# sjtuytc/betapose

Hardware: AMD Instinct MI355X
Metric: frames/sec (640x480, 50-kp KPD) (higher is better)
Workload: dtype f32 as an exact 3-way bf16 operand split (6 bf16 MFMA products), f32 accumulate and activations

## Files before the change

### betapose_amd/_lib.py

```python
from __future__ import annotations

import ctypes as C
import os
import threading

_HERE = os.path.dirname(os.path.abspath(__file__))
LIB_PATH = os.environ.get("BP_LIB") or os.path.join(_HERE, "libbetapose_hip.so")
_lock = threading.Lock()
_lib = None

c_float_p = C.POINTER(C.c_float)
c_double_p = C.POINTER(C.c_double)
c_int_p = C.POINTER(C.c_int)
vp = C.c_void_p

PROTOTYPES = {
    "bp_last_error": (C.c_char_p, []),
    "bp_version": (C.c_int, []),
    "bp_device_count": (C.c_int, []),
    "bp_device_name": (C.c_int, [C.c_int, C.c_char_p, C.c_int]),
    "bp_yolo_create": (C.c_int, [C.c_char_p, C.c_char_p, C.c_int, C.c_int, C.c_int, C.POINTER(vp)]),
    "bp_yolo_create_from_memory": (C.c_int, [C.c_char_p, vp, C.c_size_t, C.c_int, C.c_int, C.c_int, C.POINTER(vp)]),
    "bp_yolo_clone": (C.c_int, [vp, C.POINTER(vp)]),
    "bp_kpd_clone": (C.c_int, [vp, C.POINTER(vp)]),
    "bp_yolo_destroy": (None, [vp]),
    "bp_yolo_rows": (C.c_int, [vp]),
    "bp_yolo_attrs": (C.c_int, [vp]),
    "bp_yolo_forward": (C.c_int, [vp, vp, C.c_int, vp, vp]),
    "bp_yolo_forward_select": (C.c_int, [vp, vp, C.c_int, C.c_float, C.c_int, vp, vp, vp]),
    "bp_yolo_forward_select_classes": (C.c_int, [vp, vp, C.c_int, C.c_float, C.c_int, vp, C.c_int, vp, vp, vp]),
    "bp_yolo_select": (C.c_int, [vp, C.c_int, C.c_int, C.c_int, C.c_float, C.c_int, vp, vp]),
    "bp_yolo_tap_count": (C.c_int, [vp]),
    "bp_yolo_tap_info": (C.c_int, [vp, C.c_int, C.c_char_p, C.c_int, c_int_p, c_int_p, c_int_p]),
    "bp_yolo_tap_copy": (C.c_int, [vp, C.c_int, C.c_int, vp, vp]),
    "bp_kpd_create": (C.c_int, [vp, C.c_size_t, C.c_int, C.c_int, C.c_int, C.POINTER(vp)]),
    "bp_kpd_destroy": (None, [vp]),
    "bp_kpd_forward": (C.c_int, [vp, vp, C.c_int, vp, vp]),
    "bp_kpd_forward_argmax": (C.c_int, [vp, vp, C.c_int, vp, vp, vp]),
    "bp_kpd_launch_count": (C.c_int, [vp, C.c_int]),
    "bp_kpd_tap_count": (C.c_int, [vp]),
    "bp_kpd_tap_info": (C.c_int, [vp, C.c_int, C.c_char_p, C.c_int, c_int_p, c_int_p, c_int_p]),
    "bp_kpd_tap_copy": (C.c_int, [vp, C.c_int, C.c_int, vp, vp]),
    "bp_yolo_set_policy": (C.c_int, [vp, C.c_int, C.c_int, C.c_int, C.c_int]),
    "bp_kpd_set_policy": (C.c_int, [vp, C.c_int, C.c_int, C.c_int, C.c_int]),
    "bp_yolo_set_precision": (C.c_int, [vp, C.c_int]),
    "bp_kpd_set_precision": (C.c_int, [vp, C.c_int]),
    "bp_calibrate_ticks": (C.c_int, [C.c_longlong, c_float_p, vp]),
    "bp_yolo_set_prefetch": (C.c_int, [vp, C.c_int]),
    "bp_kpd_set_prefetch": (C.c_int, [vp, C.c_int]),
    "bp_yolo_set_fusion": (C.c_int, [vp, C.c_int]),
    "bp_kpd_set_fusion": (C.c_int, [vp, C.c_int]),
    "bp_yolo_fused_launches": (C.c_int, [vp, C.c_int, C.POINTER(C.c_int)]),
    "bp_kpd_fused_launches": (C.c_int, [vp, C.c_int, C.POINTER(C.c_int)]),
    "bp_yolo_xcd_errors": (C.c_int, [vp, C.POINTER(C.c_int), vp]),
    "bp_kpd_xcd_errors": (C.c_int, [vp, C.POINTER(C.c_int), vp]),
    "bp_yolo_set_stamps": (C.c_int, [vp, vp, C.c_int]),
    "bp_kpd_set_stamps": (C.c_int, [vp, vp, C.c_int]),
    "bp_yolo_op_name": (C.c_int, [vp, C.c_int, C.c_char_p, C.c_int]),
    "bp_kpd_op_name": (C.c_int, [vp, C.c_int, C.c_char_p, C.c_int]),
    "bp_yolo_op_stats": (C.c_int, [vp, c_double_p, c_double_p, C.c_int]),
    "bp_kpd_op_stats": (C.c_int, [vp, c_double_p, c_double_p, C.c_int]),
    "bp_yolo_device_bytes": (C.c_size_t, [vp]),
    "bp_kpd_device_bytes": (C.c_size_t, [vp]),
    "bp_crop": (C.c_int, [vp, C.c_int, C.c_int, C.c_int, vp, C.c_int, vp, vp, vp, vp, C.c_int, C.c_int, vp]),
    "bp_resize_bicubic": (C.c_int, [vp, C.c_int, C.c_int, C.c_int, C.c_int, C.c_int, C.c_int, vp, vp, vp]),
    "bp_conv2d": (C.c_int, [vp, C.c_int, C.c_int, C.c_int, C.c_int, vp, vp, C.c_int, C.c_int, C.c_int, C.c_int,
                            C.c_int, C.c_int, vp, C.c_int, C.c_int, C.c_int, vp, C.c_int, c_float_p, vp]),
    "bp_conv2d_planes": (C.c_int, [vp, C.c_int, C.c_int, C.c_int, C.c_int, vp, vp, C.c_int, C.c_int, C.c_int, C.c_int,
                                   C.c_int, C.c_int, vp, C.c_int, C.c_int, C.c_int, vp, vp, C.c_int, c_float_p, vp]),
    "bp_pipeline_create": (C.c_int, [vp, vp, C.c_int, C.c_int, C.c_int, C.c_float, C.c_int, vp, vp, vp, C.POINTER(vp)]),
    "bp_pipeline_kernel_count": (C.c_int, [vp]),
    "bp_yolo_profile": (C.c_int, [vp, C.c_int, C.c_int, c_float_p, c_int_p, C.c_int, vp]),
    "bp_kpd_profile": (C.c_int, [vp, C.c_int, C.c_int, c_float_p, c_int_p, C.c_int, vp]),
    "bp_pipeline_destroy": (None, [vp]),
    "bp_pipeline_frames": (vp, [vp]),
    "bp_pipeline_results": (vp, [vp]),
    "bp_pipeline_heatmaps": (vp, [vp]),
    "bp_pipeline_set_fixed_box": (C.c_int, [vp, vp]),
    "bp_pipeline_run": (C.c_int, [vp, C.c_int, vp]),
    "bp_pipeline_prepare": (C.c_int, [vp]),
    "bp_pipeline_latency_faults": (C.c_int, [vp]),
    "bp_scene_create": (C.c_int, [vp, vp, vp, C.c_int, C.c_int, C.c_int, C.c_float, C.c_int, vp, vp, C.POINTER(vp)]),
    "bp_scene_destroy": (None, [vp]),
    "bp_scene_results": (vp, [vp]),
    "bp_scene_poses": (vp, [vp]),
    "bp_scene_set_pose_solver": (C.c_int, [vp, C.c_int, vp, C.c_int, vp, C.c_int, vp]),
    "bp_scene_set_pose_ransac": (C.c_int, [vp, C.c_int, C.c_double, C.c_int, C.c_double]),
    "bp_scene_prepare": (C.c_int, [vp]),
    "bp_scene_run": (C.c_int, [vp, C.c_int, vp]),
    "bp_scene_kernel_count": (C.c_int, [vp]),
    "bp_yolo_select_nms": (C.c_int, [vp, C.c_int, C.c_int, C.c_int, C.c_float, C.c_int, C.c_int, C.c_float, C.c_int, vp, vp, vp]),
    "bp_yolo_forward_select_nms": (C.c_int, [vp, vp, C.c_int, C.c_float, C.c_int, C.c_int, C.c_float, C.c_int, vp, vp, vp, vp]),
    "bp_crop_candidates": (C.c_int, [vp, C.c_int, C.c_int, C.c_int, C.c_int, vp, C.c_int, vp, vp, vp, vp, C.c_int, C.c_int, vp]),
    "bp_cands_create": (C.c_int, [vp, vp, C.c_int, C.c_int, C.c_int, C.c_float, C.c_int, C.c_int, C.c_float, vp, vp, C.POINTER(vp)]),
    "bp_cands_destroy": (None, [vp]),
    "bp_cands_results": (vp, [vp]),
    "bp_cands_counts": (vp, [vp]),
    "bp_cands_prepare": (C.c_int, [vp]),
    "bp_cands_run": (C.c_int, [vp, C.c_int, vp]),
    "bp_cands_kernel_count": (C.c_int, [vp]),
    "bp_cands_set_pose_solver": (C.c_int, [vp, vp, C.c_int, vp, C.c_int, vp]),
    "bp_cands_pose": (vp, [vp]),
    "bp_cands_merged": (vp, [vp]),
    "bp_cands_info": (vp, [vp]),
    "bp_pose_from_candidate_records": (C.c_int, [vp, vp, C.c_int, C.c_int, vp, C.c_int, vp, C.c_int, vp, vp, vp, vp]),
    "bp_cands_set_instance_poses": (C.c_int, [vp, C.c_int, vp]),
    "bp_cands_instance_poses": (vp, [vp]),
    "bp_pose_instances_from_merged": (C.c_int, [vp, vp, vp, C.c_int, C.c_int, vp, C.c_int, vp, C.c_int, vp, vp]),
    "bp_heatmap_argmax": (C.c_int, [vp, C.c_int, C.c_int, C.c_int, C.c_int, vp, vp]),
    "bp_pose_errors": (C.c_int, [vp, C.c_int, vp, vp, C.c_int, vp, C.c_int, vp, vp]),
    "bp_pose_errors_sym": (C.c_int, [vp, C.c_int, vp, vp, C.c_int, vp, C.c_int, vp, C.c_int, vp, vp]),
    "bp_render_depth": (C.c_int, [vp, C.c_int, vp, C.c_int, vp, C.c_int, vp, C.c_int, C.c_int, C.c_double, C.c_double, vp, vp,
                                  vp]),
    "bp_render_depth_host": (C.c_int, [vp, C.c_int, vp, C.c_int, vp, C.c_int, vp, C.c_int, C.c_int, C.c_double, C.c_double, vp,
                                       vp]),
    "bp_vsd_errors": (C.c_int, [vp, C.c_int, vp, C.c_int, vp, vp, C.c_int, vp, vp, C.c_int, C.c_int, C.c_int, C.c_double, vp,
                                C.c_double, vp, C.c_int, C.c_double, C.c_double, C.c_double, C.c_int, vp, vp, vp]),
    "bp_icp_normal_equations": (C.c_int, [vp, C.c_int, vp, C.c_int, vp, C.c_int, vp, vp, C.c_int, C.c_int, C.c_int, C.c_double, vp,
                                          C.c_double, C.c_double, C.c_double, C.c_double, C.c_int, vp, vp]),
    "bp_icp_normal_equations_host": (C.c_int, [vp, C.c_int, vp, C.c_int, vp, C.c_int, vp, vp, C.c_int, C.c_int, C.c_int,
                                               C.c_double, vp, C.c_double, C.c_double, C.c_double, C.c_double, vp]),
    "bp_refine_depth": (C.c_int, [vp, C.c_int, vp, C.c_int, vp, C.c_int, vp, vp, C.c_int, C.c_int, C.c_int, C.c_double, vp,
                                  C.c_int, C.c_double, C.c_double, C.c_int, C.c_double, C.c_double, C.c_int, vp, vp, vp]),
    "bp_refine_depth_host": (C.c_int, [vp, C.c_int, vp, C.c_int, vp, C.c_int, vp, vp, C.c_int, C.c_int, C.c_int, C.c_double, vp,
                                       C.c_int, C.c_double, C.c_double, C.c_int, C.c_double, C.c_double, vp, vp]),
    "bp_pipeline_set_pose_solver": (C.c_int, [vp, vp, C.c_int, vp, C.c_int, vp]),
    "bp_pipeline_poses": (vp, [vp]),
    "bp_pose_from_records": (C.c_int, [vp, C.c_int, vp, C.c_int, vp, C.c_int, vp, vp]),
    "bp_solve_pnp_batch": (C.c_int, [vp, C.c_int, vp, C.c_int, C.c_int, vp, vp, vp, vp]),
    "bp_pnp_ransac_samples": (C.c_int, [C.c_int, C.c_int, vp]),
    "bp_pnp_ransac_trials_needed": (C.c_int, [C.c_int, C.c_double, vp]),
    "bp_pnp_ransac_workspace_bytes": (C.c_size_t, [C.c_int, C.c_int]),
    "bp_solve_pnp_ransac_batch": (C.c_int, [vp, C.c_int, vp, C.c_int, C.c_int, vp, C.c_double, C.c_int, C.c_double, vp, vp, vp,
                                            vp, C.c_size_t, vp]),
    "bp_pipeline_set_pose_ransac": (C.c_int, [vp, C.c_double, C.c_int, C.c_double]),
    "bp_pose_ransac_workspace_bytes": (C.c_size_t, [C.c_int, C.c_int]),
    "bp_pose_from_records_ransac": (C.c_int, [vp, C.c_int, vp, C.c_int, vp, C.c_int, C.c_double, C.c_int, C.c_double, vp, vp,
                                              C.c_size_t, vp]),
    "bp_solve_pnp": (C.c_int, [vp, vp, C.c_int, vp, vp, vp]),
    "bp_solve_pnp_status": (C.c_int, [vp, vp, C.c_int, vp, vp, vp, vp]),
    "bp_solve_pnp_refined": (C.c_int, [vp, vp, C.c_int, vp, vp, vp]),
    "bp_solve_pnp_ransac": (C.c_int, [vp, vp, C.c_int, vp, C.c_double, C.c_int, C.c_double, vp, vp, vp]),
    "bp_pose_nms": (C.c_int, [vp, vp, vp, vp, C.c_int, C.c_int, vp, vp, vp, vp]),
    "bp_darknet_last_error": (C.c_char_p, []),
    "bp_darknet_create": (C.c_int, [C.c_char_p, C.c_char_p, C.c_int, C.POINTER(vp)]),
    "bp_darknet_destroy": (None, [vp]),
    "bp_darknet_width": (C.c_int, [vp]),
    "bp_darknet_height": (C.c_int, [vp]),
    "bp_darknet_classes": (C.c_int, [vp]),
    "bp_darknet_detect_rgb": (C.c_int, [vp, vp, C.c_int, C.c_int, C.c_float, C.c_float, vp, C.c_int]),
    "bp_darknet_detect_png": (C.c_int, [vp, vp, C.c_size_t, C.c_float, C.c_float, vp, C.c_int]),
    "bp_darknet_detect_image": (C.c_int, [vp, vp, C.c_size_t, C.c_float, C.c_float, vp, C.c_int]),
    "bp_image_decode_rgb": (C.c_int, [vp, C.c_size_t, vp, C.c_size_t, C.POINTER(C.c_int), C.POINTER(C.c_int)]),
    "bp_darknet_detect_file": (C.c_int, [vp, C.c_char_p, C.c_float, C.c_float, vp, C.c_int]),
    "bp_yolo_create_darknet": (C.c_int, [C.c_char_p, C.c_char_p, C.c_int, C.c_int, C.c_int, C.POINTER(vp)]),
    "bp_stream_create_masked": (C.c_int, [vp, C.c_int, C.POINTER(vp)]),
    "bp_stream_destroy": (C.c_int, [vp]),
    "bp_probe_placement": (C.c_int, [C.c_int, vp, vp, vp]),
    "bp_png_info": (C.c_int, [vp, C.c_size_t, C.POINTER(C.c_int), C.POINTER(C.c_int), C.POINTER(C.c_int)]),
    "bp_png_decode_bgr": (C.c_int, [vp, C.c_size_t, vp, C.c_size_t, C.POINTER(C.c_int), C.POINTER(C.c_int)]),
    "bp_loader_create": (C.c_int, [C.POINTER(C.c_char_p), C.c_int, C.c_int, C.c_int, C.c_int, C.c_int, C.c_int,
                                   C.POINTER(vp)]),
    "bp_loader_destroy": (None, [vp]),
    "bp_loader_next": (C.c_int, [vp, C.POINTER(C.c_longlong), C.POINTER(vp)]),
    "bp_loader_release": (C.c_int, [vp, C.c_longlong]),
    "bp_upload": (C.c_int, [vp, vp, C.c_size_t, vp]),
}

RESULT_FLOATS = 316
POSE_DOUBLES = 166
PNP_MAX_POINTS = 64
MAX_SCENE_CLASSES = 16
MAX_CANDIDATES = 8
MERGED_FLOATS = 152


class BetaposeHipError(RuntimeError):
    pass


def lib():
    global _lib
    with _lock:
        if _lib is not None:
            return _lib
        import torch
        if not os.path.exists(LIB_PATH):
            from .build import build
            build(verbose=False)
        try:
            L = C.CDLL(LIB_PATH)
        except OSError as e:
            raise BetaposeHipError("cannot load %s: %s (run `python -m betapose_amd.build`)" % (LIB_PATH, e))
        for name, (res, args) in PROTOTYPES.items():
            fn = getattr(L, name)
            fn.restype = res
            fn.argtypes = args
        _lib = L
        return L


def check(rc: int) -> None:
    if rc != 0:
        msg = lib().bp_last_error()
        raise BetaposeHipError(msg.decode() if msg else "libbetapose_hip error %d" % rc)


def require_gpu() -> None:
    import torch
    if not torch.cuda.is_available():
        raise BetaposeHipError("betapose_amd needs an AMD GPU (gfx950): torch.cuda.is_available() is False; "
                               "there is no CPU fallback on the product path")
    if lib().bp_device_count() <= 0:
        raise BetaposeHipError("libbetapose_hip.so sees no HIP device")


def ptr(t) -> int:
    if t is None:
        return None
    if hasattr(t, "data_ptr"):
        if not t.is_contiguous():
            raise ValueError("tensor must be contiguous")
# ... 8 lines not shown
```

### betapose_amd/build.py

```python
from __future__ import annotations

import os
import shutil
import subprocess
import sys

HERE = os.path.dirname(os.path.abspath(__file__))
CSRC = os.path.join(HERE, "csrc")
LIB = os.path.join(HERE, "libbetapose_hip.so")
SOURCES = ["conv_igemm.hip", "conv_halo.hip", "conv_fused.hip", "conv_pl.hip", "conv_s1.hip", "conv_p3.hip", "aux_kernels.hip", "pose_metrics.hip", "pose_metrics_sym.hip", "raster.hip", "vsd.hip", "icp.hip", "pose_tail.hip", "pose_tail_cands.hip", "pose_tail_inst.hip", "pnp_ransac.hip", "engine.cpp", "host_post.cpp", "raster_host.cpp", "icp_host.cpp", "frame_io.cpp", "jpeg_bmp.cpp", "c_api.cpp", "darknet_compat.cpp"]
HEADERS = ["bp_common.h", "engine.h", "frame_chain.h", "frame_io.h", "conv_tail.inc", "pnp_wave.inc", "pnp_math.inc", "pose_decode.inc", "pose_tail.h", "raster.h", "raster_math.inc", "icp.h", "icp_math.inc", "conv_dev.h", os.path.join("..", "..", "include", "betapose_hip.h"),
           os.path.join("..", "..", "include", "yolo_v2_class_compat.h")]
EXP = "experimental"
EXP_SOURCES = [os.path.join(EXP, s_) for s_ in ("conv_w64.hip", "conv_kg.hip", "conv_rd.hip")]
EXP_HEADERS = [os.path.join(EXP, s_) for s_ in ("mega.inc", "kernels_unity.hip")]
ARCH = "gfx950"
LAST_ACTION = None
MIN_STUBS = {"conv_s1.hip": 1, "conv_p3.hip": 39, "conv_igemm.hip": 14, "conv_halo.hip": 13, "conv_fused.hip": 12, "conv_pl.hip": 12, "aux_kernels.hip": 21, "pose_metrics.hip": 2, "pose_metrics_sym.hip": 4, "raster.hip": 3, "vsd.hip": 2, "icp.hip": 4, "pose_tail.hip": 3, "pose_tail_cands.hip": 1, "pose_tail_inst.hip": 1, "pnp_ransac.hip": 2}
MIN_STUBS_EXP = {"conv_s1.hip": 1, "conv_p3.hip": 39, "experimental/kernels_unity.hip": 26, "conv_fused.hip": 12, "conv_pl.hip": 12, "experimental/conv_w64.hip": 8,
                 "experimental/conv_kg.hip": 3, "experimental/conv_rd.hip": 2, "aux_kernels.hip": 24, "pose_metrics.hip": 2, "pose_metrics_sym.hip": 4, "raster.hip": 3, "vsd.hip": 2, "icp.hip": 4, "pose_tail.hip": 3, "pose_tail_cands.hip": 1, "pose_tail_inst.hip": 1, "pnp_ransac.hip": 2}


def hipcc() -> str:
    for cand in (os.environ.get("HIPCC"), shutil.which("hipcc"), "/opt/rocm/bin/hipcc"):
        if cand and os.path.exists(cand):
            return cand
    raise RuntimeError("hipcc not found (need ROCm to build libbetapose_hip.so)")


def _stale() -> bool:
    if not os.path.exists(LIB):
        return True
    t = os.path.getmtime(LIB)
    deps = [os.path.join(CSRC, s) for s in SOURCES + HEADERS]
    return any(os.path.getmtime(d) > t for d in deps if os.path.exists(d))


def build(force: bool = False, verbose: bool = True, experimental: bool = False) -> str:
    if experimental:
        return _build(True, verbose, os.path.join(HERE, "libbetapose_hip_exp.so"), os.path.join(HERE, "build_exp"),
                      ["-DBP_EXPERIMENTAL"])
    global LAST_ACTION
    if not force and not _stale():
        LAST_ACTION = "reused"
        return LIB
    LAST_ACTION = "compiled"
    return _build(force, verbose, LIB, os.path.join(HERE, "build"), [])


def _build(force: bool, verbose: bool, LIB: str, objdir: str, extra) -> str:
    cc = hipcc()
    objs = []
    os.makedirs(objdir, exist_ok=True)
    procs = []
    sources = SOURCES + (EXP_SOURCES if extra else [])
    if extra:
        sources = [os.path.join(EXP, "kernels_unity.hip")] + [s_ for s_ in sources if s_ not in ("conv_igemm.hip", "conv_halo.hip")]
    hdr_t = max(os.path.getmtime(os.path.join(CSRC, h)) for h in HEADERS + (EXP_HEADERS if extra else []))
    flags_key = " ".join(list(extra) + os.environ.get("BP_CFLAGS", "").split())
    flags_file = os.path.join(objdir, ".flags")
    same_flags = os.path.exists(flags_file) and open(flags_file).read() == flags_key
    for src in sources:
        obj = os.path.join(objdir, os.path.splitext(os.path.basename(src))[0] + ".o")
        objs.append(obj)
        if not force and same_flags and os.path.exists(obj) and os.path.getmtime(obj) > max(hdr_t, os.path.getmtime(os.path.join(CSRC, src))):
            continue
        cmd = [cc, "--offload-arch=" + ARCH, "-O3", "-std=c++17", "-fPIC", "-x", "hip", "-c", "-I", CSRC,
               os.path.join(CSRC, src), "-o", obj] + list(extra) + os.environ.get("BP_CFLAGS", "").split()
        if verbose:
            print(" ".join(cmd), flush=True)
        procs.append((src, subprocess.Popen(cmd, stdout=subprocess.PIPE, stderr=subprocess.STDOUT, text=True)))
    for src, p in procs:
        out, _ = p.communicate()
        if p.returncode != 0:
            raise RuntimeError("hipcc failed on %s:\n%s" % (src, out))
        if verbose and out.strip():
            print(out)
    with open(flags_file, "w") as f:
        f.write(flags_key)
    nm = shutil.which("nm") or "/opt/rocm/lib/llvm/bin/llvm-nm"
    for src, want in (MIN_STUBS_EXP if extra else MIN_STUBS).items():
        obj = os.path.join(objdir, os.path.splitext(os.path.basename(src))[0] + ".o")
        syms = subprocess.run([nm, obj], stdout=subprocess.PIPE, text=True).stdout
        have = syms.count("__device_stub__")
        if have < want:
            raise RuntimeError("%s: %d kernel host stubs in the object, expected >= %d (hipcc dropped a kernel)" % (src, have, want))
    cmd = [cc, "--offload-arch=" + ARCH, "-shared", "-fPIC", "-o", LIB] + objs + ["-lz", "-lpthread"]
    if verbose:
        print(" ".join(cmd), flush=True)
    subprocess.check_call(cmd)
    return LIB


if __name__ == "__main__":
    print(build(force="--force" in sys.argv, experimental="--experimental" in sys.argv))
```

### betapose_amd/csrc/bp_common.h

```cpp
#pragma once
#include <hip/hip_runtime.h>
#include <cstdint>
#include <cstdio>
#include <mutex>
#include <set>
#include <stdexcept>
#include <string>
#include <utility>

namespace bp {

struct Error : std::runtime_error {
    using std::runtime_error::runtime_error;
};

#define BP_HIP(expr)                                                                      \
    do {                                                                                  \
        hipError_t _e = (expr);                                                           \
        if (_e != hipSuccess)                                                             \
            throw ::bp::Error(std::string(#expr) + ": " + hipGetErrorString(_e) + " @" +  \
                              __FILE__ + ":" + std::to_string(__LINE__));                 \
    } while (0)

#define BP_CHECK(cond, msg)                                                               \
    do {                                                                                  \
        if (!(cond)) throw ::bp::Error(std::string(msg) + " (" #cond ") @" + __FILE__ +   \
                                       ":" + std::to_string(__LINE__));                   \
    } while (0)

inline void allow_big_lds(const void* kernel) {
    static std::mutex mu;
    static std::set<std::pair<int, const void*>> done;
    int dev = 0;
    BP_HIP(hipGetDevice(&dev));
    std::lock_guard<std::mutex> lk(mu);
    if (done.count({dev, kernel})) return;
    BP_HIP(hipFuncSetAttribute(kernel, hipFuncAttributeMaxDynamicSharedMemorySize, 160 * 1024 - 64));
    done.insert({dev, kernel});
}

__device__ __forceinline__ unsigned long long bp_clock() { return __builtin_amdgcn_s_memrealtime(); }

enum Act : int { ACT_LINEAR = 0, ACT_LEAKY = 1, ACT_RELU = 2 };

enum StoreMode : int {
    ST_NHWC = 0,
    ST_UP2 = 1,
    ST_PIXSHUF = 2,
    ST_NCHW = 3
};

struct ConvParams {
    const float* in;
    int in_ld;
    int N, H, W, Cin;
    const float* w;
    int Kpad;
    int Ktrue;
    const float* bias;
    float* out;
    int out_ld;
    int OH, OW, Cout;
    int ksize, stride, pad;
    int act;
    const float* res;
    int res_ld;
    const float* res_scale;
    int res_after_act;
    int store_mode;
    int M;
    int nchunks;
    int splits;
    int chunks_per_split;
    float* partial;
    int* tickets;
    int CoutPad;
    int cin_pack;
    const unsigned short* w16;
    const unsigned short* w16s;
    int mfma_mode;
    unsigned long long* stamps;
    const unsigned short* in16;
    long long in16_plane;
    unsigned short* out16;
    long long out16_plane;
    int out_np;
    int skip_f32;
    const unsigned short* res16;
    int net_prec;
    int abl;
    const unsigned short* wbd;
    const unsigned short* wpl;
    float* pool_out;
    int hy_full, hy_splits, hy_cps;
    int xcd_home;
    int* xcc_of;
    int* err_word;
    int* tickets_local;
    int mtiles, n_tiles;
    int work_blocks;
    const void* pf_ptr;
    int pf_first;
    int pf_ntn, pf_splits, pf_cps, pf_nchunks;
    int pf_tile_stride, pf_chunk_bytes;
    int pf_cap;
};

enum Precision : int { PREC_F32 = 0, PREC_F16 = 1, PREC_BF16X3 = 2, PREC_F16_RES = 3 };

enum ConvTile : int { TILE_64x64 = 0, TILE_128x64 = 1, TILE_W64_1x1 = 2, TILE_W64_1x2 = 3, TILE_W64_2x1 = 5, TILE_W64_2x2 = 6,
                      TILE_KG1 = 7, TILE_KG2 = 8, TILE_KG4 = 9,
                      TILE_RD4 = 10, TILE_RD8 = 11,
                      TILE_64x64_BD = 12,
                      TILE_PL64 = 13,
                      TILE_PL128 = 14,
                      TILE_PL128x64 = 15,
                      TILE_PL256x128 = 16,
                      TILE_STEM3 = 20,
                      TILE_PL64BD = 19,
                      TILE_PL64K2 = 18,
                      TILE_PL128S = 17,
                      TILE_HALO64 = 21,
                      TILE_HALO128 = 22,
                      TILE_HALO64K2 = 23,
                      TILE_BD_K2 = 24,
                      TILE_PLH128 = 25,
                      TILE_S1 = 26,
                      TILE_P3 = 27,
                      TILE_STEM7 = 28,
                      TILE_LAST = 27,
                      TILE_FUSED = 40 };

struct ConvProfHook { hipEvent_t e0, e1; };
extern thread_local ConvProfHook* g_conv_prof;
bool conv_h16_eligible(const ConvParams& p);
int conv_vec_mode(const ConvParams& p);

void launch_conv(const ConvParams& p, int tile, hipStream_t s);
void launch_conv_w64(const ConvParams& p, int tile, hipStream_t s);
bool conv_tile_is_w64(int tile);
void launch_conv_kg(const ConvParams& p, int tile, hipStream_t s);
bool conv_tile_is_kg(int tile);
void launch_conv_rd(const ConvParams& p, int tile, hipStream_t s);
bool conv_tile_is_rd(int tile);
void launch_conv_pl(const ConvParams& p, int tile, hipStream_t s);
bool conv_tile_is_pl(int tile);
void launch_conv_halo(const ConvParams& p, int tile, hipStream_t s);
bool conv_tile_is_halo(int tile);
bool conv_halo_eligible(const ConvParams& p, int tile);
void conv_split_plan(const ConvParams& p, int tile, int want, int* splits, int* cps);
inline bool conv_tile_is_plh(int tile) { return tile == TILE_PLH128; }
bool conv_plh_eligible(const ConvParams& p);
bool conv_pl_eligible(const ConvParams& p);
bool conv_s1_eligible(const ConvParams& p, long long M);
void launch_conv_s1(const ConvParams& p, hipStream_t s);
bool conv_p3_eligible(const ConvParams& p, long long M);
void launch_conv_p3(const ConvParams& p, hipStream_t s);
void launch_pack_wpl(const float* in, unsigned short* out, int CoutPad, int Kpad, int Cin, int ksize, int np, hipStream_t s);
void launch_f32_to_planes(const float* in, int ld, long long pixels, int C, unsigned short* planes, long long plane_elems,
                          int np, hipStream_t s);
void launch_planes_to_f32(const unsigned short* planes, long long plane_elems, int np, float* out, int ld, long long pixels, int C,
                          hipStream_t s);
bool conv_fused_eligible(const ConvParams& pre, const ConvParams& c3, const ConvParams* post);
int conv_fused_blocks(const ConvParams& pre, const ConvParams& c3, const ConvParams* post);
void launch_conv_fused(const ConvParams& pre, const ConvParams& c3, const ConvParams* post, hipStream_t s);
int conv_tiles(const ConvParams& p, int tile);
bool conv_stem3_eligible(const ConvParams& p);
bool conv_stem7_eligible(const ConvParams& p);
void conv_grid_setup(ConvParams& q, int bm, int bn);
int conv_grid_blocks(const ConvParams& q);
int xcc_base();
bool conv_hybrid_plan(const ConvParams& p, int tile, size_t partial_floats, int* full, int* hs, int* hcps);
bool conv_home_layout(int tile, int splits);
void conv_prefetch_of(ConvParams& p, const ConvParams& next, int next_tile, int next_splits, int next_cps);
int conv_tile_bm(int tile);
int conv_tile_bn(int tile);

enum MegaOpType : int { MO_CONV_BD = 0, MO_CONV_K2 = 1, MO_CONV_F32V2 = 2, MO_STEM3 = 3 };

struct MegaOp {
    int type, items, npass, pad;
    ConvParams conv;
};
struct MegaArgs {
    const MegaOp* prog[8];
    int n_ops[8];
    unsigned* sync;
    int nb;
    unsigned long long* stamps;
};

size_t mega_lds_bytes(const MegaOp& o);
void mega_make_conv_op(const ConvParams& p, int tile, MegaOp* out);
void launch_mega(const MegaArgs& a, size_t lds_bytes, hipStream_t s);

void launch_nchw_to_nhwc(const float* in, float* out, int N, int C, int H, int W, hipStream_t s);
void launch_nhwc_to_nchw(const float* in, int in_ld, float* out, int N, int C, int H, int W, hipStream_t s);
void launch_maxpool3s2p1(const float* in, float* out, int N, int H, int W, int C, int OH, int OW, hipStream_t s,
                         unsigned short* planes = nullptr, long long plane_elems = 0, int np = 0);
void launch_add(const float* a, int a_ld, const float* b, int b_ld, float* out, int out_ld,
                long long pixels, int C, hipStream_t s);
void launch_upsample2(const float* in, int in_ld, float* out, int out_ld, int N, int H, int W, int C, hipStream_t s);
void launch_copy_channels(const float* in, int in_ld, float* out, int out_ld, long long pixels, int C, hipStream_t s);
void launch_pixel_shuffle2(const float* in, float* out, int N, int H, int W, int C, hipStream_t s,
                           unsigned short* planes = nullptr, long long plane_elems = 0, int np = 0);
int avgpool_parts(int HW);
void launch_avgpool(const float* in, int in_ld, float* out, int N, int HW, int C, hipStream_t s);
void launch_fc(const float* in, const float* w, const float* bias, float* out, int N, int Cin, int Cout,
               int act, int in_parts, float in_scale, hipStream_t s);

struct YoloHead {
    const float* t;
    int g;
    float aw[3], ah[3];
    int row_off;
};
void launch_yolo_decode(const YoloHead* heads, int nheads, int N, int reso, int attrs, int rows,
                        float* pred, hipStream_t s);
void launch_yolo_select(const float* pred, int N, int rows, int attrs, float conf, int num_classes,
                        float* sel, hipStream_t s, int sel_ld = 8);
void launch_yolo_decode_select(const YoloHead* heads, int nheads, int N, int reso, int attrs, int rows, float conf, int num_classes,
                               float* sel, hipStream_t s, int sel_ld = 8);
#define BP_MAX_SCENE_CLASSES 16
struct YoloClassList {
    int n;
    int id[BP_MAX_SCENE_CLASSES];
};
YoloClassList make_class_list(const int* class_ids, int K, int num_classes, int attrs);
void launch_yolo_select_classes(const float* pred, int N, int rows, int attrs, float conf, int num_classes, const YoloClassList& cl,
                                float* sel, hipStream_t s, int ld_image, int ld_slot);
void launch_yolo_decode_select_classes(const YoloHead* heads, int nheads, int N, int reso, int attrs, int rows, float conf,
                                       int num_classes, const YoloClassList& cl, float* sel, hipStream_t s, int ld_image, int ld_slot);
#define BP_MAX_CANDIDATES 8
void launch_yolo_select_nms(const float* pred, int N, int rows, int attrs, float conf, int num_classes, int class_id, float nms_conf,
                            int C, float* sel, int* count, hipStream_t s, int ld_image, int ld_slot);
void launch_yolo_decode_select_nms(const YoloHead* heads, int nheads, int N, int reso, int attrs, int rows, float conf, int num_classes,
                                   int class_id, float nms_conf, int C, float* sel, int* count, hipStream_t s, int ld_image,
                                   int ld_slot);
void launch_heatmap_argmax(const float* hm, int N, int C, int H, int W, float* out, hipStream_t s, int out_ld = 0);

void launch_f32_to_f16(const float* in, unsigned short* out, long long n, hipStream_t s);
void launch_f32_to_bf16x3(const float* in, unsigned short* out_planes, long long n, hipStream_t s);
void launch_f32_to_f16_staged(const float* in, unsigned short* out, int CoutPad, int Kpad, hipStream_t s);
void launch_f32_to_bf16x3_staged(const float* in, unsigned short* out, int CoutPad, int Kpad, hipStream_t s, int Cin_pl = 0);
void launch_probe_placement(int* d_out, int blocks, hipStream_t s);
void launch_spin_ticks(long long ticks, hipStream_t s);

void launch_crop(const uint8_t* frames, int batch, int H, int W, const float* sel, int reso, const float* boxes,
                 float* out_nhwc, float* out_nchw, float* pts, int oh, int ow, hipStream_t s, int sel_ld = 8, int pts_ld = 8,
                 int per_frame = 1);

struct ResizeTables {
    const int* hb;
    const int* hk;
    int ksize_h;
    const int* vb;
    const int* vk;
    int ksize_v;
};
void launch_resize_bicubic(const uint8_t* in, int batch, int H, int W, uint8_t* tmp, float* out_nhwc, uint8_t* out_u8,
                           int oh, int ow, const ResizeTables& t, int swap_rb, hipStream_t s);

}
```

### betapose_amd/csrc/c_api.cpp

```cpp
#include "../../include/betapose_hip.h"

#include <algorithm>
#include <cmath>
#include <cstdlib>
#include <cstring>
#include <fstream>
#include <memory>
#include <sstream>
#include <vector>

#include "engine.h"
#include "frame_chain.h"
#include "frame_io.h"
#include "icp.h"
#include "pose_tail.h"
#include "raster.h"

static thread_local std::string g_err;

#define BP_TRY try {
#define BP_CATCH                                   \
    }                                              \
    catch (const std::exception& e) {              \
        g_err = e.what();                          \
// ... 652 lines not shown
    void* ws = a.alloc_bytes(bp::raster_vertex_bytes(n, (int)(2 * c)));
    int* skipped = (int*)a.alloc_bytes(2 * c * sizeof(int));
    int* acc = (int*)a.alloc_bytes((size_t)P * bp::VSD_ACC * sizeof(int));
    BP_HIP(hipMemsetAsync(acc, 0, (size_t)P * bp::VSD_ACC * sizeof(int), s));
    BP_HIP(hipMemsetAsync(skipped, 0, 2 * c * sizeof(int), s));
    for (size_t p0 = 0; p0 < (size_t)P; p0 += c) {
        const int m = (int)std::min(c, (size_t)P - p0);
        BP_HIP(hipMemsetD32Async((hipDeviceptr_t)zbuf, 0x7f800000, 2 * (size_t)m * HW, s));
        bp::launch_raster(d_model, n, d_faces, F, d_gt + p0 * 12, m, d_est + p0 * 12, m, K, H, W, pixel_center, near_z, ws, zbuf,
                          skipped, s);
        bp::launch_vsd_reduce(zbuf, m, d_depth_test, T, d_test_index + p0, H, W, K, pixel_center, depth_scale, delta, tv, n_tau,
                              diameter, acc + p0 * bp::VSD_ACC, s);
    }
    bp::launch_vsd_finish(acc, d_test_index, T, P, n_tau, d_err, d_counts, s);
    BP_HIP(hipGetLastError());
    BP_HIP(hipStreamSynchronize(s));
    return 0;
    BP_CATCH
}

static bp::IcpParams icp_params(const double* K, int T, double depth_scale, int iterations, double max_dist, double min_cos,
                                int min_pixels, double pixel_center) {
    BP_CHECK(T > 0, "T must be positive");
    BP_CHECK(depth_scale > 0.0 && max_dist > 0.0, "depth_scale and max_dist must be positive");
    BP_CHECK(min_cos >= 0.0 && min_cos <= 1.0, "min_cos must lie in [0, 1]");
    BP_CHECK(iterations >= 0 && iterations <= 1000 && min_pixels >= 0, "iterations must lie in 0 .. 1000, min_pixels >= 0");
    return bp::IcpParams{K[0], K[4], K[2], K[5], pixel_center, depth_scale, max_dist, min_cos, min_pixels, iterations};
}

static size_t icp_chunk(int chunk, int n, int P, size_t HW) {
    size_t c = (size_t)chunk;
    if (c == 0) c = std::min(RASTER_WS_BYTES / (HW * sizeof(float)), RASTER_WS_BYTES / bp::raster_vertex_bytes(n, 1));
    return std::max<size_t>(1, std::min<size_t>(c, (size_t)P));
}

int bp_icp_normal_equations_host(const double* poses, int P, const double* vertices, int n, const int* faces, int F,
                                 const double* K, const uint16_t* depth_test, int T, int H, int W, double depth_scale,
                                 const int* test_index, double max_dist, double min_cos, double pixel_center, double near_z,
                                 double* out) {
    BP_TRY
    BP_CHECK(poses && vertices && faces && K && depth_test && test_index && out, "null argument");
    raster_check_sizes(n, F, P, H, W, near_z);
    const bp::IcpParams prm = icp_params(K, T, depth_scale, 0, max_dist, min_cos, 0, pixel_center);
    BP_CHECK(bp::icp_normal_equations_host(poses, P, vertices, n, faces, F, K, depth_test, T, test_index, H, W, prm, near_z,
                                           out) == 0,
             "a face index lies outside [0, n)");
    return 0;
    BP_CATCH
}

int bp_refine_depth_host(const double* poses, int P, const double* vertices, int n, const int* faces, int F, const double* K,
                         const uint16_t* depth_test, int T, int H, int W, double depth_scale, const int* test_index,
                         int iterations, double max_dist, double min_cos, int min_pixels, double pixel_center, double near_z,
                         double* poses_out, double* stats) {
    BP_TRY
    BP_CHECK(poses && vertices && faces && K && depth_test && test_index && poses_out && stats, "null argument");
    raster_check_sizes(n, F, P, H, W, near_z);
    const bp::IcpParams prm = icp_params(K, T, depth_scale, iterations, max_dist, min_cos, min_pixels, pixel_center);
    BP_CHECK(bp::refine_depth_host(poses, P, vertices, n, faces, F, K, depth_test, T, test_index, H, W, prm, near_z, poses_out,
                                   stats) == 0,
             "a face index lies outside [0, n)");
    return 0;
    BP_CATCH
}

int bp_icp_normal_equations(const double* d_model, int n, const int* d_faces, int F, const double* d_poses, int P,
                            const double* K, const uint16_t* d_depth_test, int T, int H, int W, double depth_scale,
                            const int* d_test_index, double max_dist, double min_cos, double pixel_center, double near_z,
                            int chunk, double* d_out, void* stream) {
    BP_TRY
    BP_CHECK(d_model && d_faces && d_poses && K && d_depth_test && d_test_index && d_out, "null argument");
    raster_check_sizes(n, F, P, H, W, near_z);
    BP_CHECK(chunk >= 0, "chunk must not be negative");
    const bp::IcpParams prm = icp_params(K, T, depth_scale, 0, max_dist, min_cos, 0, pixel_center);
    hipStream_t s = (hipStream_t)stream;
    const size_t HW = (size_t)H * W, c = icp_chunk(chunk, n, P, HW);
    const int slices = bp::icp_slices(H, W);
    bp::Arena a;
    uint32_t* zbuf = (uint32_t*)a.alloc_bytes(c * HW * sizeof(uint32_t));
    void* ws = a.alloc_bytes(bp::raster_vertex_bytes(n, (int)c));
    int* skipped = (int*)a.alloc_bytes(c * sizeof(int));
    double* partial = (double*)a.alloc_bytes(c * slices * bp::ICP_ACC * sizeof(double));
    BP_HIP(hipMemsetAsync(skipped, 0, c * sizeof(int), s));
    for (size_t p0 = 0; p0 < (size_t)P; p0 += c) {
        const int m = (int)std::min(c, (size_t)P - p0);
        BP_HIP(hipMemsetD32Async((hipDeviceptr_t)zbuf, 0x7f800000, (size_t)m * HW, s));
        bp::launch_raster(d_model, n, d_faces, F, d_poses + p0 * 12, m, nullptr, 0, K, H, W, pixel_center, near_z, ws, zbuf,
                          skipped, s);
        bp::launch_icp_accumulate(zbuf, d_poses + p0 * 12, m, d_depth_test, T, d_test_index + p0, H, W, prm, nullptr, partial, s);
        bp::launch_icp_sum(partial, d_test_index + p0, T, m, slices, d_out + p0 * bp::ICP_ACC, s);
    }
    BP_HIP(hipGetLastError());
    BP_HIP(hipStreamSynchronize(s));
    return 0;
    BP_CATCH
}

int bp_refine_depth(const double* d_model, int n, const int* d_faces, int F, const double* d_poses, int P, const double* K,
                    const uint16_t* d_depth_test, int T, int H, int W, double depth_scale, const int* d_test_index,
                    int iterations, double max_dist, double min_cos, int min_pixels, double pixel_center, double near_z,
                    int chunk, double* d_poses_out, double* d_stats, void* stream) {
    BP_TRY
    BP_CHECK(d_model && d_faces && d_poses && K && d_depth_test && d_test_index && d_poses_out && d_stats, "null argument");
    BP_CHECK(d_poses_out != d_poses, "d_poses_out must not be d_poses: a rejected pose gets its input back");
    raster_check_sizes(n, F, P, H, W, near_z);
    BP_CHECK(chunk >= 0, "chunk must not be negative");
    const bp::IcpParams prm = icp_params(K, T, depth_scale, iterations, max_dist, min_cos, min_pixels, pixel_center);
    hipStream_t s = (hipStream_t)stream;
    const size_t HW = (size_t)H * W, c = icp_chunk(chunk, n, P, HW);
    const int slices = bp::icp_slices(H, W);
    bp::Arena a;
    uint32_t* zbuf = (uint32_t*)a.alloc_bytes(c * HW * sizeof(uint32_t));
    void* ws = a.alloc_bytes(bp::raster_vertex_bytes(n, (int)c));
    int* skipped = (int*)a.alloc_bytes(c * sizeof(int));
    double* partial = (double*)a.alloc_bytes(c * slices * bp::ICP_ACC * sizeof(double));
    BP_HIP(hipMemsetAsync(skipped, 0, c * sizeof(int), s));
    bp::launch_icp_init(d_poses, d_test_index, T, P, d_poses_out, d_stats, s);
    for (size_t p0 = 0; p0 < (size_t)P; p0 += c) {
        const int m = (int)std::min(c, (size_t)P - p0);
        double* pose = d_poses_out + p0 * 12;
        double* stats = d_stats + p0 * bp::ICP_STATS;
        for (int k = 0; k <= iterations; ++k) {
            BP_HIP(hipMemsetD32Async((hipDeviceptr_t)zbuf, 0x7f800000, (size_t)m * HW, s));
            bp::launch_raster(d_model, n, d_faces, F, pose, m, nullptr, 0, K, H, W, pixel_center, near_z, ws, zbuf, skipped, s);
            bp::launch_icp_accumulate(zbuf, pose, m, d_depth_test, T, d_test_index + p0, H, W, prm, stats, partial, s);
            bp::launch_icp_step(partial, m, slices, k, prm, d_poses + p0 * 12, pose, stats, s);
        }
    }
    BP_HIP(hipGetLastError());
    BP_HIP(hipStreamSynchronize(s));
    return 0;
    BP_CATCH
}

int bp_heatmap_argmax(const float* d_hm, int batch, int C, int H, int W, float* d_kp, void* stream) {
    BP_TRY
    BP_CHECK(d_hm && d_kp && batch > 0 && C > 0 && H > 0 && W > 0, "bad argument");
    bp::launch_heatmap_argmax(d_hm, batch, C, H, W, d_kp, (hipStream_t)stream);
    BP_HIP(hipGetLastError());
    return 0;
    BP_CATCH
}

int bp_conv2d(const float* d_in, int N, int H, int W, int Cin, const float* h_w, const float* h_bias, int Cout, int k,
              int stride, int pad, int act, int store_mode, const float* d_res, int res_after_act, int tile, int splits,
              float* d_out, int iters, float* ms_per_iter, void* stream) {
    return bp_conv2d_planes(d_in, N, H, W, Cin, h_w, h_bias, Cout, k, stride, pad, act, store_mode, d_res, res_after_act, tile,
                            splits, d_out, nullptr, iters, ms_per_iter, stream);
}

int bp_conv2d_planes(const float* d_in, int N, int H, int W, int Cin, const float* h_w, const float* h_bias, int Cout, int k,
                     int stride, int pad, int act, int store_mode, const float* d_res, int res_after_act, int tile, int splits,
                     float* d_out, unsigned short* d_out_planes, int iters, float* ms_per_iter, void* stream) {
    BP_TRY
    BP_CHECK(d_in && h_w && d_out, "null argument");
    hipStream_t s = (hipStream_t)stream;
    struct OneConv : bp::Net {
        OneConv() : Net(1) {}
        using Net::add_conv;
        using Net::finalize;
        using Net::ops_;
        using Net::partial_;
        using Net::partial_floats_;
        using Net::arena_;
    } net;
    const int OH = (H + 2 * pad - k) / stride + 1, OW = (W + 2 * pad - k) / stride + 1;
    bp::Tensor in; in.p = const_cast<float*>(d_in); in.H = H; in.W = W; in.C = Cin; in.ld = Cin;
    bp::Tensor out; out.p = d_out; out.H = OH; out.W = OW; out.C = Cout;
    out.ld = store_mode == bp::ST_PIXSHUF ? Cout / 4 : Cout;
    bp::Tensor res; res.p = const_cast<float*>(d_res); res.ld = Cout; res.C = Cout; res.H = OH; res.W = OW;
    bp::ConvWeights cw; cw.w = h_w; cw.bias = h_bias;
    net.add_conv("conv", in, out, cw, Cout, k, stride, pad, act, store_mode, d_res ? &res : nullptr, nullptr,
                 res_after_act, 1e-5f, OH, OW);
    int t = tile;
    int prec = bp::PREC_F32;
    if (t >= 256) {
        prec = t >= 512 ? bp::PREC_BF16X3 : bp::PREC_F16;
        t -= t >= 512 ? 512 : 256;
        BP_CHECK(Cin % 32 == 0, "layer is not eligible for the 16-bit MFMA paths (needs Cin % 32 == 0)");
        net.set_precision(prec);
        net.ops_[0].conv.mfma_mode = prec;
#ifndef BP_EXPERIMENTAL
        BP_CHECK(bp::conv_tile_is_pl(t) || ((t == bp::TILE_64x64_BD || t == bp::TILE_BD_K2 || bp::conv_tile_is_halo(t)) && prec == bp::PREC_BF16X3),
                 "this kernel id exists only in the experimental library (python -m betapose_amd.build --experimental, BP_LIB)");
#endif
    } else {
        if (t < 0 && bp::conv_stem3_eligible(net.ops_[0].conv)) t = bp::TILE_STEM3;
        BP_CHECK(t <= bp::TILE_128x64 || (t == bp::TILE_STEM3 && bp::conv_stem3_eligible(net.ops_[0].conv)) || (t == bp::TILE_STEM7 && bp::conv_stem7_eligible(net.ops_[0].conv)),
                 "this tile needs a 16-bit precision mode (tile + 256 / + 512), or the layer is not a 3x3 / stride-1 / 4-channel-packed stem");
    }
    bp::ConvParams p = net.ops_[0].conv;
    p.N = N; p.M = N * OH * OW;
    if (t < 0) t = bp::TILE_64x64;
    const int np = prec == bp::PREC_F16 ? 1 : 3;
    if (bp::conv_tile_is_pl(t)) {
        const long long in_elems = (long long)N * H * W * Cin;
        BP_CHECK(Cin % 32 == 0 && k * k <= 32, "layer is not eligible for the operand-plane kernels (needs Cin % 32 == 0, k*k <= 32)");
        unsigned short* d_in16 = (unsigned short*)net.arena_.alloc_bytes((size_t)np * in_elems * 2);
        bp::launch_f32_to_planes(d_in, Cin, (long long)N * H * W, Cin, d_in16, in_elems, np, s);
        p.in16 = d_in16; p.in16_plane = in_elems;
        auto& packed = np == 1 ? net.weight_store()->wpl1 : net.weight_store()->wpl3;
        auto it = packed.find(p.w);
        if (it == packed.end()) {
            unsigned short* d = (unsigned short*)net.weight_store()->arena.alloc_bytes((size_t)np * p.CoutPad * p.Kpad * 2);
            bp::launch_pack_wpl(p.w, d, p.CoutPad, p.Kpad, p.Cin, p.ksize, np, s);
            it = packed.emplace(p.w, d).first;
        }
        p.wpl = it->second;
        if (t == bp::TILE_PL64BD) {
            auto& staged = net.weight_store()->wbd3;
            auto ib = staged.find(p.w);
            if (ib == staged.end()) {
                unsigned short* d = (unsigned short*)net.weight_store()->arena.alloc_bytes((size_t)3 * p.CoutPad * p.Kpad * 2);
                bp::launch_f32_to_bf16x3_staged(p.w, d, p.CoutPad, p.Kpad, s, p.Cin);
                ib = staged.emplace(p.w, d).first;
            }
            p.wbd = ib->second;
        }
    }
    if (const char* e = std::getenv("BP_PL_ABL")) p.abl = std::atoi(e);
    if (d_out_planes) {
        BP_CHECK(prec != bp::PREC_F32, "output planes need a 16-bit precision mode");
        long long out_elems = (long long)N * OH * OW * Cout;
        if (store_mode == bp::ST_UP2) out_elems *= 4;
        p.out16 = d_out_planes; p.out16_plane = out_elems; p.out_np = np;
    }
    if (prec == bp::PREC_F16 && std::getenv("BP_CONV_F16R")) {
        if (p.res) {
            const long long n_res = (long long)N * OH * OW;
            unsigned short* r16 = (unsigned short*)net.arena_.alloc_bytes((size_t)n_res * p.res_ld * 2);
            bp::launch_f32_to_planes(p.res, p.res_ld, n_res, Cout, r16, n_res * p.res_ld, 1, s);
            p.res16 = r16;
        }
        if (p.out16) p.skip_f32 = 1;
    }
    int sp = splits;
    if (sp <= 0) {
        const long long blocks = bp::conv_tiles(p, t);
        sp = 1;
        while (blocks * sp < 512 && p.nchunks / (sp + 1) >= 4 && sp < 64) ++sp;
    }
    if (t == bp::TILE_S1 || t == bp::TILE_P3) sp = 1;
    int per = 0;
    bp::conv_split_plan(p, t, sp, &sp, &per);
    p.splits = sp; p.chunks_per_split = per;
    if (sp > 1) {
        const int tiles = bp::conv_tiles(p, t);
        p.partial = net.arena_.alloc((size_t)sp * tiles * bp::conv_tile_bm(t) * bp::conv_tile_bn(t));
        p.tickets = (int*)net.arena_.alloc_bytes((size_t)(2 + 64) * tiles * sizeof(int));
        BP_HIP(hipMemset(p.tickets, 0, (size_t)(2 + 64) * tiles * sizeof(int)));
    }
    if (sp == 1 && !std::getenv("BP_CONV_SELF_PREFETCH")) {
        const size_t cap = (size_t)8 * 256 * bp::conv_tile_bm(t) * bp::conv_tile_bn(t);
        int full = 0, hs = 0, hcps = 0;
        if (bp::conv_hybrid_plan(p, t, cap, &full, &hs, &hcps)) {
            const int tail = bp::conv_tiles(p, t) - full;
            p.partial = net.arena_.alloc((size_t)hs * tail * bp::conv_tile_bm(t) * bp::conv_tile_bn(t));
            p.tickets = (int*)net.arena_.alloc_bytes((size_t)tail * sizeof(int));
            BP_HIP(hipMemset(p.tickets, 0, (size_t)tail * sizeof(int)));
            p.hy_full = full; p.hy_splits = hs; p.hy_cps = hcps;
        }
    }
    if (bp::conv_home_layout(t, sp)) {
        const int tiles = bp::conv_tiles(p, t);
        p.xcd_home = 1;
        p.tickets_local = p.tickets + tiles;
        p.xcc_of = p.tickets + 2 * tiles;
    }
    if (std::getenv("BP_CONV_SELF_PREFETCH")) bp::conv_prefetch_of(p, p, t, sp, per);
    bp::launch_conv(p, t, s);
    BP_HIP(hipStreamSynchronize(s));
    if (const char* e = std::getenv("BP_CONV_STAMPS")) {
        const int nb = bp::conv_tiles(p, t) * p.splits;
        unsigned long long* d = (unsigned long long*)net.arena_.alloc_bytes((size_t)nb * 8 * 8);
        BP_HIP(hipMemset(d, 0, (size_t)nb * 64));
        bp::ConvParams q = p; q.stamps = d;
        bp::launch_conv(q, t, s);
        BP_HIP(hipStreamSynchronize(s));
        std::vector<unsigned long long> h((size_t)nb * 8);
        BP_HIP(hipMemcpy(h.data(), d, h.size() * 8, hipMemcpyDeviceToHost));
        unsigned long long t0 = ~0ull;
        for (int b = 0; b < nb; ++b)
            if (h[(size_t)b * 8]) t0 = std::min(t0, h[(size_t)b * 8]);
        double acc[8] = {0, 0, 0, 0, 0, 0, 0, 0}, last = 0;
        int cnt[8] = {0, 0, 0, 0, 0, 0, 0, 0};
        for (int b = 0; b < nb; ++b)
            for (int k = 0; k < 8; ++k) {
                const unsigned long long v = h[(size_t)b * 8 + k];
                if (!v) continue;
                acc[k] += (double)(v - h[(size_t)b * 8]); ++cnt[k];
                last = std::max(last, (double)(v - t0));
            }
        auto mean = [&](int k) { return cnt[k] ? acc[k] / cnt[k] : 0.0; };
        if (std::getenv("BP_W64_ABLATE") && (std::atoi(std::getenv("BP_W64_ABLATE")) & 64)) {
            double sum[4] = {0, 0, 0, 0};
            for (int b = 0; b < nb; ++b) for (int k = 0; k < 4; ++k) sum[k] += (double)h[(size_t)b * 8 + 4 + k];
            const double stages = 2.0 * p.chunks_per_split * nb;
            std::fprintf(stderr, "[stage timing] cycles per stage: issue slots 0..UPW %.0f | slots ..SYNC %.0f | wait+barrier %.0f | SYNC..end %.0f\n",
                         sum[0] / stages, sum[1] / stages, sum[2] / stages, sum[3] / stages);
        }
        std::fprintf(stderr, "[stamps] blocks=%d  mean 10-ns ticks (s_memrealtime, 100 MHz) since the block's entry: index math done %.0f | chunk 0 in LDS %.0f | "
                     "K loop done %.0f | in-block sums (conv_kg) or cycles parked at the stage waits (conv_pl) %.0f | slab parked + ticket %.0f (%d blocks) | slices combined %.0f (%d) | stores done %.0f (%d) | "
                     "last mark of the grid %.0f after the first entry\n", nb, mean(1), mean(2), mean(3), mean(7), mean(5), cnt[5], mean(6),
                     cnt[6], mean(4), cnt[4], last);
    }
    if (iters > 0 && ms_per_iter) {
        hipEvent_t e0, e1;
        BP_HIP(hipEventCreate(&e0));
        BP_HIP(hipEventCreate(&e1));
        BP_HIP(hipEventRecord(e0, s));
        for (int i = 0; i < iters; ++i) bp::launch_conv(p, t, s);
        BP_HIP(hipEventRecord(e1, s));
        BP_HIP(hipEventSynchronize(e1));
        float ms = 0;
        BP_HIP(hipEventElapsedTime(&ms, e0, e1));
        *ms_per_iter = ms / iters;
        (void)hipEventDestroy(e0);
        (void)hipEventDestroy(e1);
    }
    return 0;
    BP_CATCH
}

static void pipeline_enqueue(bp_pipeline* p, hipStream_t s) {
    bp::YoloNet& yn = *p->y->net;
    bp::KpdNet& kn = *p->k->net;
    const int reso = yn.reso();
#ifdef BP_EXPERIMENTAL
    static const bool no_resize = std::getenv("BP_ABLATE_RESIZE") != nullptr;
    if (!no_resize) p->resize.enqueue(p->batch, p->H, p->W, yn.input_nhwc(), reso, s);
#else
    p->resize.enqueue(p->batch, p->H, p->W, yn.input_nhwc(), reso, s);
#endif
    const int R = BP_RESULT_FLOATS;
    yn.forward(yn.input_nhwc(), true, p->batch, nullptr, p->conf, p->num_classes, p->results, s, R);
    bp::launch_crop(p->resize.frames, p->batch, p->H, p->W, p->use_fixed ? nullptr : p->results, reso,
                    p->use_fixed ? p->fixed_box : nullptr, kn.input_nhwc(), nullptr, p->results + 8, kn.in_h(), kn.in_w(), s, R, R);
    kn.forward(kn.input_nhwc(), true, p->batch, p->hm, p->results + 16, s, R);
    p->pose.enqueue(p->results, p->batch, s);
    BP_HIP(hipGetLastError());
}

int bp_pipeline_create(bp_yolo* y, bp_kpd* k, int frame_h, int frame_w, int batch, float conf, int num_classes,
                       uint8_t* d_frames, float* d_results, float* d_hm, bp_pipeline** out) {
    BP_TRY
    BP_CHECK(y && k && out, "null argument");
    BP_CHECK(batch >= 1 && batch <= y->net->max_batch() && batch <= k->net->max_batch(), "pipeline batch > engine max_batch");
    BP_CHECK(k->net->out_c() == 50, "pipeline expects 50 key points");
    BP_HIP(hipSetDevice(y->device));
    std::unique_ptr<bp_pipeline> p(new bp_pipeline);
    p->y = y; p->k = k; p->H = frame_h; p->W = frame_w; p->batch = batch; p->conf = conf; p->num_classes = num_classes;
    p->engines = {{y->net.get()}, {k->net.get()}};
    p->resize.init(p->arena, d_frames, batch, frame_h, frame_w, y->net->reso());
    p->results = d_results ? d_results : p->arena.alloc((size_t)batch * BP_RESULT_FLOATS);
    p->hm = d_hm ? d_hm : p->arena.alloc((size_t)batch * 50 * k->net->out_h() * k->net->out_w());
    p->fixed_box = p->arena.alloc((size_t)batch * 4);
    BP_HIP(hipMemset(p->results, 0, (size_t)batch * BP_RESULT_FLOATS * sizeof(float)));
    *out = p.release();
    return 0;
    BP_CATCH
}
void bp_pipeline_destroy(bp_pipeline* p) { delete p; }
uint8_t* bp_pipeline_frames(bp_pipeline* p) { return p ? p->resize.frames : nullptr; }
float* bp_pipeline_results(bp_pipeline* p) { return p ? p->results : nullptr; }
float* bp_pipeline_heatmaps(bp_pipeline* p) { return p ? p->hm : nullptr; }
int bp_pipeline_kernel_count(bp_pipeline* p) { return p ? p->graph.nodes() : -1; }

int bp_pipeline_set_fixed_box(bp_pipeline* p, const float* box) {
    BP_TRY
    p->graph.drop();
    p->use_fixed = box != nullptr;
    if (box) {
        std::vector<float> h((size_t)p->batch * 4);
        for (int b = 0; b < p->batch; ++b) std::memcpy(&h[b * 4], box, 4 * sizeof(float));
        BP_HIP(hipMemcpy(p->fixed_box, h.data(), h.size() * sizeof(float), hipMemcpyHostToDevice));
    }
    return 0;
    BP_CATCH
}

int bp_pipeline_set_pose_solver(bp_pipeline* p, const double* kp3d, int n_kp, const double* K, int left_number,
                                double* d_poses) {
    BP_TRY
    BP_CHECK(p, "null argument");
    p->graph.drop();
    if (!kp3d) {
        p->pose.off();
        return 0;
    }
    const int dev = p->y->device;
    p->pose.set(p->arena, dev, kp3d, n_kp, K, left_number,
                d_poses ? d_poses : bp::own_pose_rows(p->arena, dev, p->own_poses, p->batch));
    return 0;
    BP_CATCH
}
// ... 574 lines not shown
```

### betapose_amd/csrc/conv_dev.h

```cpp
#pragma once
#include <hip/hip_ext.h>

#include <type_traits>
#include <utility>

#include "bp_common.h"

#if !defined(BP_EXPERIMENTAL) && (defined(BP_ABLATE_SPLIT) || defined(BP_ABLATE_MFMA) || defined(BP_ABLATE_KLOOP) || defined(BP_ABLATE_PREFETCH) || \
    defined(BP_ABLATE_TAIL) || defined(BP_ABLATE_SLABSTORE) || defined(BP_ABLATE_ACKWAIT) || defined(BP_ABLATE_REDUCE) || defined(BP_ABLATE_EPILOGUE) || \
    defined(BP_W64_DEBUG))
#error "BP_ABLATE_* / BP_W64_DEBUG are timing experiments with wrong results: build them with -DBP_EXPERIMENTAL only (build.py --experimental)"
#endif

namespace bp {

template <class F, int... I>
__device__ __forceinline__ void static_for_impl(F&& f, std::integer_sequence<int, I...>) {
    (f(std::integral_constant<int, I>{}), ...);
}
template <int N, class F>
__device__ __forceinline__ void static_for(F&& f) {
    static_for_impl(f, std::make_integer_sequence<int, N>{});
}

typedef float f32x16 __attribute__((ext_vector_type(16)));
typedef unsigned int u32x4 __attribute__((ext_vector_type(4)));
typedef float f32x4 __attribute__((ext_vector_type(4)));

typedef _Float16 f16x8 __attribute__((ext_vector_type(8)));
typedef _Float16 f16x4 __attribute__((ext_vector_type(4)));
typedef __bf16 bf16x8 __attribute__((ext_vector_type(8)));
typedef __bf16 bf16x4 __attribute__((ext_vector_type(4)));
typedef unsigned short u16x4 __attribute__((ext_vector_type(4)));
typedef float f32x2 __attribute__((ext_vector_type(2)));
typedef __bf16 bf16x2 __attribute__((ext_vector_type(2)));
typedef unsigned int u32x2 __attribute__((ext_vector_type(2)));

static constexpr int BK = 32;
static constexpr int LDS_LD = 36;
static constexpr unsigned OOB = 0x7fffff00u;

struct PlaneDesc {
    __amdgpu_buffer_rsrc_t r0, r1, r2;
    int np;
    bool f32;
};
template <class P>
__device__ __forceinline__ PlaneDesc make_plane_desc(const P& p) {
    PlaneDesc d;
    unsigned short* base = p.out16 ? p.out16 : reinterpret_cast<unsigned short*>(p.out);
    const int bytes = (int)min((long long)p.M * p.out_ld * ((p.store_mode == ST_PIXSHUF || p.store_mode == ST_UP2) ? 8 : 2), (long long)0x7fffff00);
    d.np = p.out16 ? p.out_np : 0;
    d.f32 = !(p.out16 && p.skip_f32);
    d.r0 = __builtin_amdgcn_make_buffer_rsrc(base, 0, bytes, 0x00020000);
    d.r1 = __builtin_amdgcn_make_buffer_rsrc(base + (d.np == 3 ? p.out16_plane : 0), 0, bytes, 0x00020000);
    d.r2 = __builtin_amdgcn_make_buffer_rsrc(base + (d.np == 3 ? 2 * p.out16_plane : 0), 0, bytes, 0x00020000);
    return d;
}
typedef __attribute__((address_space(3))) void lds_void_t;
__device__ __forceinline__ void dma16(__amdgpu_buffer_rsrc_t rsrc, char* lds, unsigned voff, int soff) {
    __builtin_amdgcn_raw_ptr_buffer_load_lds(rsrc, (lds_void_t*)lds, 16, (int)voff, soff, 0, 0);
}

__device__ __forceinline__ int xcc_id() {
    unsigned id;
    asm volatile("s_getreg_b32 %0, hwreg(HW_REG_XCC_ID)" : "=s"(id));
    return (int)(id & 15);
}
template <class P>
__device__ __forceinline__ void xcd_home_mark(const P& p, int tile_id, int split) {
    if (threadIdx.x == 0) __hip_atomic_store(&p.xcc_of[tile_id * 64 + split], xcc_id() ^ ((p.xcd_home >> 1) & (split == 0)), __ATOMIC_RELAXED, __HIP_MEMORY_SCOPE_AGENT);
}
template <class P>
__device__ __forceinline__ bool xcd_home_verify(const P& p, int tile_id, int* flag) {
    const bool bad = (int)threadIdx.x < p.splits &&
        __hip_atomic_load(&p.xcc_of[tile_id * 64 + (int)threadIdx.x], __ATOMIC_RELAXED, __HIP_MEMORY_SCOPE_AGENT) != xcc_id();
    if (bad) *flag = 3;
    __syncthreads();
    const bool any_bad = *flag != 1;
    if (any_bad && threadIdx.x == 0 && p.err_word) __hip_atomic_fetch_or(p.err_word, 1, __ATOMIC_RELAXED, __HIP_MEMORY_SCOPE_AGENT);
    return !any_bad;
}

template <int NT, class P>
__device__ __forceinline__ void prefetch_block(const P& p, char* lds, const int bp_bid) {
    const int e = bp_bid - p.pf_first;
    if (e < 0) return;
    const int x = bp_bid & 7, ql = e >> 3;
    const int g = p.pf_ntn < 8 ? p.pf_ntn : 8;
    if (ql >= (p.pf_ntn / g) * p.pf_splits) return;
    const int j = ql / p.pf_splits, split = ql - j * p.pf_splits;
    const int tile_n = (x & (g - 1)) + g * j;
    const int c0 = split * p.pf_cps, c1 = min(p.pf_nchunks, c0 + p.pf_cps);
    if (c1 <= c0) return;
    const long long beg = (long long)tile_n * p.pf_tile_stride + (long long)c0 * p.pf_chunk_bytes;
    const unsigned n = (unsigned)min((long long)(c1 - c0) * p.pf_chunk_bytes, (long long)p.pf_cap);
    const __amdgpu_buffer_rsrc_t r = __builtin_amdgcn_make_buffer_rsrc(
        const_cast<char*>(static_cast<const char*>(p.pf_ptr)) + beg, 0, (int)n, 0x00020000);
    char* const dst = lds + __builtin_amdgcn_readfirstlane((int)threadIdx.x >> 6) * 1024;
    for (unsigned off = threadIdx.x * 16u; off < n; off += NT * 16u) dma16(r, dst, off, 0);
}

__device__ __forceinline__ void store_b64_wt(u32x2 v, __amdgpu_buffer_rsrc_t r, unsigned off, bool) {
    __builtin_amdgcn_raw_buffer_store_b64(v, r, (int)off, 0, 0);
}
__device__ __forceinline__ void emit_planes4(const PlaneDesc& d, f32x4 v, unsigned off) {
    if (d.np == 1) {
        const f16x4 h = __builtin_convertvector(v, f16x4);
        store_b64_wt(__builtin_bit_cast(u32x2, h), d.r0, off, false);
    } else if (d.np == 3) {
        const bf16x4 h1 = __builtin_convertvector(v, bf16x4);
        const f32x4 r1 = v - __builtin_convertvector(h1, f32x4);
        const bf16x4 h2 = __builtin_convertvector(r1, bf16x4);
        const f32x4 r2 = r1 - __builtin_convertvector(h2, f32x4);
        const bf16x4 h3 = __builtin_convertvector(r2, bf16x4);
        store_b64_wt(__builtin_bit_cast(u32x2, h1), d.r0, off, false);
        store_b64_wt(__builtin_bit_cast(u32x2, h2), d.r1, off, false);
        store_b64_wt(__builtin_bit_cast(u32x2, h3), d.r2, off, false);
    }
}
template <class P>
__device__ __forceinline__ void emit_plane1(const P& p, long long idx, float v) {
    if (!p.out16) return;
    if (p.out_np == 1) {
        const _Float16 h = (_Float16)v;
        p.out16[idx] = __builtin_bit_cast(unsigned short, h);
    } else if (p.out_np == 3) {
        const __bf16 h1 = (__bf16)v;
        const float r1 = v - (float)h1;
        const __bf16 h2 = (__bf16)r1;
        const float r2 = r1 - (float)h2;
        const __bf16 h3 = (__bf16)r2;
        p.out16[idx] = __builtin_bit_cast(unsigned short, h1);
        p.out16[idx + p.out16_plane] = __builtin_bit_cast(unsigned short, h2);
        p.out16[idx + 2 * p.out16_plane] = __builtin_bit_cast(unsigned short, h3);
    }
}

__device__ __forceinline__ float apply_act(float v, int act) {
    if (act == ACT_LEAKY) return v > 0.f ? v : 0.1f * v;
    if (act == ACT_RELU) return v > 0.f ? v : 0.f;
    return v;
}

template <class P>
__device__ __forceinline__ void epilogue_store(const P& p, int m, int n, float v, float bias) {
    v += bias;
    int b = 0, pix = m;
    const int hw = p.OH * p.OW;
    const bool need_pix = p.store_mode != ST_NHWC || p.res_scale != nullptr;
    if (need_pix) {
        b = m / hw;
        pix = m - b * hw;
    }
    float r = 0.f;
    if (p.res) {
        if (p.res16) { const _Float16 h = __builtin_bit_cast(_Float16, p.res16[(long long)m * p.res_ld + n]); r = (float)h; }
        else r = p.res[(long long)m * p.res_ld + n];
        if (p.res_scale) r *= p.res_scale[b * p.Cout + n];
    }
    if (!p.res_after_act) v += r;
    v = apply_act(v, p.act);
    if (p.res_after_act) v += r;
    const bool keep32 = !(p.out16 && p.skip_f32);
    switch (p.store_mode) {
        case ST_NHWC:
            if (keep32) p.out[(long long)m * p.out_ld + n] = v;
            emit_plane1(p, (long long)m * p.out_ld + n, v);
            break;
        case ST_UP2: {
            const int oy = pix / p.OW, ox = pix - oy * p.OW;
            const int W2 = 2 * p.OW;
            const long long i0 = ((long long)(b * 2 * p.OH + 2 * oy) * W2 + 2 * ox) * p.out_ld + n;
            float* o = p.out + i0;
            if (keep32) {
                o[0] = v;
                o[p.out_ld] = v;
                o[(long long)W2 * p.out_ld] = v;
                o[(long long)(W2 + 1) * p.out_ld] = v;
            }
            emit_plane1(p, i0, v);
            emit_plane1(p, i0 + p.out_ld, v);
            emit_plane1(p, i0 + (long long)W2 * p.out_ld, v);
            emit_plane1(p, i0 + (long long)(W2 + 1) * p.out_ld, v);
        } break;
        case ST_PIXSHUF: {
            const int oy = pix / p.OW, ox = pix - oy * p.OW;
            const int cq = p.Cout >> 2;
            const int ij = n / cq, c = n - ij * cq;
            const int y = 2 * oy + (ij >> 1), x = 2 * ox + (ij & 1);
            const long long i0 = ((long long)(b * 2 * p.OH + y) * (2 * p.OW) + x) * p.out_ld + c;
            if (keep32) p.out[i0] = v;
            emit_plane1(p, i0, v);
        } break;
        case ST_NCHW:
            p.out[((long long)b * p.Cout + n) * hw + pix] = v;
            break;
    }
}

template <class P>
__device__ __forceinline__ void epilogue_tile(const P& p, const f32x16& v, int m_base, int n) {
    if (n >= p.Cout) return;
    const float bias = p.bias[n];
    static_for<16>([&](auto ec) __attribute__((always_inline)) {
        constexpr int e = decltype(ec)::value;
        const int m = m_base + (e & 3) + 8 * (e >> 2);
        if (m < p.M) epilogue_store(p, m, n, v[e], bias);
    });
}

__device__ __forceinline__ f32x4 buf_load4(__amdgpu_buffer_rsrc_t rsrc, unsigned voff, int soff) {
    const u32x4 t = __builtin_amdgcn_raw_buffer_load_b128(rsrc, (int)voff, soff, 0);
    return f32x4{__uint_as_float(t.x), __uint_as_float(t.y), __uint_as_float(t.z), __uint_as_float(t.w)};
}
// ... 151 lines not shown
```

### betapose_amd/csrc/conv_igemm.hip

```cpp
#include <cstdlib>

#include "conv_dev.h"

namespace bp {

template <int TM, int TN, int VEC, class P>
__device__ __forceinline__ void conv_igemm_body(const P& p, const int bp_bid, float* const smem, int* const s_last_p) {
    constexpr int BM = 64 * TM, BN = 64 * TN;
    constexpr int RA = BM / 32, RB = BN / 32;
    float (*As)[BM * LDS_LD] = reinterpret_cast<float (*)[BM * LDS_LD]>(smem);
    float (*Bs)[BN * LDS_LD] = reinterpret_cast<float (*)[BN * LDS_LD]>(smem + 2 * BM * LDS_LD);
    constexpr int LDT = BN + 4;
    static_assert(BM * LDT <= 2 * (BM + BN) * LDS_LD, "LDS too small for the staged epilogue");

    const unsigned long long t_entry = p.stamps ? bp_clock() : 0ull;
    const int tid = threadIdx.x;
    const int lane = tid & 63;
    const int wave = tid >> 6;
    const int wm = wave >> 1, wn = wave & 1;
    const int n_tiles_n = p.CoutPad / BN;
    const int split = bp_bid % p.splits;
    const int tile_id = bp_bid / p.splits;
    const int tile_n = tile_id % n_tiles_n;
    const int tile_m = tile_id / n_tiles_n;
// ... 749 lines not shown
        const int oy = fast_div(rem, p.OW, rcp_ow), ox = rem - oy * p.OW;
        const int base = (b * p.H + 2 * oy - 3) * p.W + 2 * ox - 3;
#pragma unroll
        for (int i = 0; i < NT; ++i) {
            const int t = 4 * i + tq;
            const int ky = (t * 37) >> 8, kx = t - 7 * ky;
            const int iy = 2 * oy - 3 + ky, ix = 2 * ox - 3 + kx;
            const bool ok = (t < 49) & ((unsigned)iy < (unsigned)p.H) & ((unsigned)ix < (unsigned)p.W);
            const unsigned off = (unsigned)((base + ky * p.W + kx) * p.in_ld * 4);
            x[i] = buf_load4(rsrcA, ok ? off : OOB, 0);
        }
    };
    const int groups = (p.M + GP - 1) / GP, G = (groups + (int)gridDim.x - 1) / (int)gridDim.x;
    const int g0 = (int)blockIdx.x * G;
    f32x4 xn[NT];
    load_taps(g0 * GP, xn);
    for (int g = 0; g < G; ++g) {
        const int m0 = (g0 + g) * GP;
        if (m0 >= p.M) break;
        f32x4 x[NT];
#pragma unroll
        for (int i = 0; i < NT; ++i) x[i] = xn[i];
        if (g + 1 < G && m0 + GP < p.M) load_taps(m0 + GP, xn);
        {
            char* const row = rows + pix * RB;
#pragma unroll
            for (int i = 0; i < NT; ++i) {
                const int t = 4 * i + tq;
                f32x4 v = x[i];
                if (p.Cin < 4) v.w = 0.f;
                if (t < 49) *reinterpret_cast<f16x4*>(row + 8 * t) = __builtin_convertvector(v, f16x4);
            }
        }
        __syncthreads();
        f32x16 acc;
#pragma unroll
        for (int r = 0; r < 16; ++r) acc[r] = 0.f;
        {
            const char* const arow = rows + (32 * wp + (lane & 31)) * RB + (lane >> 5) * 16;
#pragma unroll
            for (int ks = 0; ks < 14; ++ks)
                acc = __builtin_amdgcn_mfma_f32_32x32x16_f16(*reinterpret_cast<const f16x8*>(arow + 32 * ks), fb[ks], acc, 0, 0, 0);
        }
#pragma unroll
        for (int r = 0; r < 16; ++r)
            S[(32 * wp + (r & 3) + 8 * (r >> 2) + 4 * (lane >> 5)) * LDT + 32 * wc + (lane & 31)] = acc[r];
        __syncthreads();
        const int m = m0 + pix;
        if (m < p.M && c0 < p.Cout) {
            const float* srow = S + pix * LDT + c0;
            f32x4 v[4] = {*reinterpret_cast<const f32x4*>(srow) + b4a, *reinterpret_cast<const f32x4*>(srow + 4) + b4b,
                          *reinterpret_cast<const f32x4*>(srow + 8) + b4c, *reinterpret_cast<const f32x4*>(srow + 12) + b4d};
#pragma unroll
            for (int q = 0; q < 4; ++q) {
                if (p.act == ACT_LEAKY) {
                    v[q].x = v[q].x > 0.f ? v[q].x : 0.1f * v[q].x; v[q].y = v[q].y > 0.f ? v[q].y : 0.1f * v[q].y;
                    v[q].z = v[q].z > 0.f ? v[q].z : 0.1f * v[q].z; v[q].w = v[q].w > 0.f ? v[q].w : 0.1f * v[q].w;
                } else if (p.act == ACT_RELU) {
                    v[q].x = v[q].x > 0.f ? v[q].x : 0.f; v[q].y = v[q].y > 0.f ? v[q].y : 0.f;
                    v[q].z = v[q].z > 0.f ? v[q].z : 0.f; v[q].w = v[q].w > 0.f ? v[q].w : 0.f;
                }
            }
            const long long e = (long long)m * p.out_ld + c0;
            if (!(p.out16 && p.skip_f32)) {
#pragma unroll
                for (int q = 0; q < 4; ++q) *reinterpret_cast<f32x4*>(p.out + e + 4 * q) = v[q];
            }
            if (p.out16 && p.out_np == 1) {
                const f16x4 h0 = __builtin_convertvector(v[0], f16x4), h1 = __builtin_convertvector(v[1], f16x4),
                            h2 = __builtin_convertvector(v[2], f16x4), h3 = __builtin_convertvector(v[3], f16x4);
                *reinterpret_cast<f16x8*>(p.out16 + e) = __builtin_shufflevector(h0, h1, 0, 1, 2, 3, 4, 5, 6, 7);
                *reinterpret_cast<f16x8*>(p.out16 + e + 8) = __builtin_shufflevector(h2, h3, 0, 1, 2, 3, 4, 5, 6, 7);
            }
        }
    }
}

bool conv_stem7_eligible(const ConvParams& p) {
    return p.cin_pack == 4 && p.Cin <= 4 && (p.in_ld == 4 || (p.in_ld == 3 && p.Cin == 3)) && p.ksize == 7 && p.stride == 2 && p.pad == 3 && p.Cout == 64 && p.CoutPad == 64 &&
           p.Kpad == 224 && p.store_mode == ST_NHWC && p.res == nullptr && p.res_scale == nullptr && p.pool_out == nullptr && (p.out_ld & 7) == 0 &&
           (p.out16 == nullptr || p.out_np == 1) && (reinterpret_cast<uintptr_t>(p.out) & 15) == 0 && (reinterpret_cast<uintptr_t>(p.out16) & 15) == 0 &&
           (long long)p.M * p.out_ld * 4 < (long long)OOB && (long long)p.N * p.H * p.W * 16 < (long long)OOB && p.M < (1 << 24);
}

static void launch_stem7(const ConvParams& p, hipStream_t s) {
    BP_CHECK(conv_stem7_eligible(p) && p.splits == 1, "not the 7x7 / stride-2 / packed-RGB stem");
    static const int g_env = std::getenv("BP_STEM7_G") ? std::atoi(std::getenv("BP_STEM7_G")) : 0;
    const int groups = (p.M + 63) / 64;
    int per = g_env > 0 ? g_env : 8;
    while (per > 1 && groups / per < 512) --per;
    const dim3 g((groups + per - 1) / per);
    if (g_conv_prof) hipExtLaunchKernelGGL(stem7x7_f16_kernel, g, dim3(256), 0, s, g_conv_prof->e0, g_conv_prof->e1, 0, p);
    else hipLaunchKernelGGL(stem7x7_f16_kernel, g, dim3(256), 0, s, p);
}

static bool stem3_f16_wanted(const ConvParams& p) {
    static const bool off = std::getenv("BP_NO_STEM_F16") != nullptr;
    return !off && p.out16 != nullptr && p.out_np == 1 && p.Cout == 32 && p.Kpad >= 48 && p.out_ld % 8 == 0 &&
           (reinterpret_cast<uintptr_t>(p.out16) & 15) == 0 && (reinterpret_cast<uintptr_t>(p.out) & 15) == 0;
}

bool conv_stem3_eligible(const ConvParams& p) {
    return p.cin_pack == 4 && p.Cin <= 4 && p.in_ld >= p.Cin && p.in_ld <= 4 && p.ksize == 3 && p.stride == 1 && p.pad == 1 && p.OH == p.H && p.OW == p.W &&
           p.Cout % 4 == 0 && p.Cout <= 64 && p.CoutPad >= ((p.Cout + 7) / 8) * 8 && p.Kpad >= 36 && p.store_mode == ST_NHWC &&
           p.res == nullptr && p.res_scale == nullptr && (p.out_ld & 3) == 0 && p.pool_out == nullptr &&
           (long long)p.M * p.out_ld * 4 < (long long)OOB;
}

static void launch_stem3(const ConvParams& p, hipStream_t s) {
    BP_CHECK(conv_stem3_eligible(p) && p.splits == 1, "not a 3x3 / stride-1 / packed-RGB stem");
    if (stem3_f16_wanted(p)) {
        static const int g_env = std::getenv("BP_STEM_G") ? std::atoi(std::getenv("BP_STEM_G")) : 0;
        const int groups = (p.M + 127) / 128;
        int per = g_env > 0 ? g_env : 8;
        while (per > 1 && groups / per < 512) --per;
        const dim3 g((groups + per - 1) / per);
        if (g_conv_prof) hipExtLaunchKernelGGL(stem3x3_f16_kernel, g, dim3(256), 0, s, g_conv_prof->e0, g_conv_prof->e1, 0, p);
        else hipLaunchKernelGGL(stem3x3_f16_kernel, g, dim3(256), 0, s, p);
        return;
    }
    const int cg = (p.Cout + 7) / 8;
    const dim3 grid((p.M + 63) / 64);
#define BP_STEM(CG_)                                                                                                       \
    if (g_conv_prof) hipExtLaunchKernelGGL((stem3x3_kernel<CG_>), grid, dim3(64 * CG_), 0, s, g_conv_prof->e0, g_conv_prof->e1, 0, p); \
    else hipLaunchKernelGGL((stem3x3_kernel<CG_>), grid, dim3(64 * CG_), 0, s, p)
    switch (cg) {
        case 1: BP_STEM(1); break;
        case 2: BP_STEM(2); break;
        case 4: BP_STEM(4); break;
        case 8: BP_STEM(8); break;
        default: throw Error("stem kernel: 8, 16, 32 or 64 output channels");
    }
#undef BP_STEM
}

void conv_grid_setup(ConvParams& q, int bm, int bn) {
    q.mtiles = (q.M + bm - 1) / bm;
    const int ntn = (q.CoutPad + bn - 1) / bn;
    q.n_tiles = q.mtiles * ntn;
    q.work_blocks = q.hy_splits > 0 ? q.hy_full + (q.n_tiles - q.hy_full) * q.hy_splits
                   : q.xcd_home ? ((q.n_tiles + 7) / 8) * 8 * q.splits : q.n_tiles * q.splits;
    q.pf_first = (q.work_blocks + 7) & ~7;
}
int conv_grid_blocks(const ConvParams& q) {
    if (!q.pf_ptr) return q.work_blocks;
    const int g = q.pf_ntn < 8 ? q.pf_ntn : 8;
    return q.pf_first + 8 * (q.pf_ntn / g) * q.pf_splits;
}

int conv_tile_bm(int tile) {
    switch (tile) {
        case TILE_128x64: case TILE_W64_2x1: case TILE_W64_2x2: case TILE_PL128: case TILE_PL128x64: case TILE_PL128S: case TILE_PLH128: case TILE_P3: return 128;
        case TILE_PL256x128: return 256;
        case TILE_S1: return 32;
        default: return 64;
    }
}
int conv_tile_bn(int tile) {
    switch (tile) {
        case TILE_W64_1x2: case TILE_W64_2x2: case TILE_PL128: case TILE_PL256x128: case TILE_PL128S: case TILE_HALO128: case TILE_PLH128: case TILE_S1: case TILE_P3: return 128;
        default: return 64;
    }
}

template <int TM, int TN>
static void launch_t(const ConvParams& p, hipStream_t s) {
    constexpr int BM = 64 * TM, BN = 64 * TN;
    dim3 grid(((p.M + BM - 1) / BM) * (p.CoutPad / BN) * p.splits);
    const int vec = conv_vec_mode(p);
    if (g_conv_prof) {
        if (vec == 1)
            hipExtLaunchKernelGGL((conv_igemm_kernel<TM, TN, 1>), grid, dim3(256), 0, s, g_conv_prof->e0, g_conv_prof->e1, 0, p);
        else if (vec == 2)
            hipExtLaunchKernelGGL((conv_igemm_kernel<TM, TN, 2>), grid, dim3(256), 0, s, g_conv_prof->e0, g_conv_prof->e1, 0, p);
        else
            hipExtLaunchKernelGGL((conv_igemm_kernel<TM, TN, 0>), grid, dim3(256), 0, s, g_conv_prof->e0, g_conv_prof->e1, 0, p);
    } else if (vec == 1) {
        hipLaunchKernelGGL((conv_igemm_kernel<TM, TN, 1>), grid, dim3(256), 0, s, p);
    } else if (vec == 2) {
        hipLaunchKernelGGL((conv_igemm_kernel<TM, TN, 2>), grid, dim3(256), 0, s, p);
    } else {
        hipLaunchKernelGGL((conv_igemm_kernel<TM, TN, 0>), grid, dim3(256), 0, s, p);
    }
}

template <int TM, int TN, int NP, bool BD = false>
static void launch_h_t(const ConvParams& p, hipStream_t s) {
    constexpr int BM = 64 * TM, BN = 64 * TN;
    ConvParams q = p;
    conv_grid_setup(q, BM, BN);
    dim3 grid(conv_grid_blocks(q));
    if (g_conv_prof)
        hipExtLaunchKernelGGL((conv_igemm_h_kernel<TM, TN, NP, BD>), grid, dim3(256), 0, s, g_conv_prof->e0, g_conv_prof->e1, 0, q);
    else
        hipLaunchKernelGGL((conv_igemm_h_kernel<TM, TN, NP, BD>), grid, dim3(256), 0, s, q);
}

int conv_vec_mode(const ConvParams& p) {
    if ((p.Cin % 32 == 0) && (p.in_ld % 4 == 0) && p.ksize <= 8) return 1;
    if (p.cin_pack == 4 && p.Cin <= 4 && p.ksize <= 8) return 2;
    return 0;
}

bool conv_h16_eligible(const ConvParams& p) {
    return (p.w16 != nullptr || p.w16s != nullptr) && (p.Cin % 32 == 0) && (p.in_ld % 4 == 0) && p.ksize <= 8;
}

void conv_split_plan(const ConvParams& p, int tile, int want, int* splits, int* cps) {
    const int unit = ((conv_tile_is_halo(tile) || conv_tile_is_plh(tile)) && p.nchunks % 9 == 0 && p.nchunks >= 9) ? 9 : 1;
    const int units = p.nchunks / unit;
    int s = want < 1 ? 1 : (want > units ? units : want);
    const int per = (units + s - 1) / s;
    s = (units + per - 1) / per;
    *splits = s; *cps = per * unit;
}

int conv_tiles(const ConvParams& p, int tile) {
    const int bm = conv_tile_bm(tile), bn = conv_tile_bn(tile);
    return ((p.M + bm - 1) / bm) * ((p.CoutPad + bn - 1) / bn);
}

void launch_conv(const ConvParams& p, int tile, hipStream_t s) {
    BP_CHECK(p.CoutPad % 64 == 0, "CoutPad must be a multiple of 64");
    BP_CHECK(p.Kpad % BK == 0 && p.nchunks == p.Kpad / BK, "Kpad");
    BP_CHECK(p.splits >= 1 && (p.splits == 1 || (p.partial != nullptr && p.tickets != nullptr)), "split-K workspace");
    BP_CHECK((long long)p.N * p.H * p.W * p.in_ld * 4 < (long long)OOB, "activation tensor too large for 32-bit offsets");
    BP_CHECK((long long)p.M * p.out_ld * 4 < (long long)OOB && (p.res == nullptr || (long long)p.M * p.res_ld * 4 < (long long)OOB),
             "output / residual tensor too large for 32-bit offsets");
    if (tile == TILE_STEM3) {
        launch_stem3(p, s);
    } else if (tile == TILE_STEM7) {
        launch_stem7(p, s);
    } else if (conv_tile_is_pl(tile)) {
        launch_conv_pl(p, tile, s);
    } else if (conv_tile_is_halo(tile)) {
        launch_conv_halo(p, tile, s);
    } else if (tile == TILE_64x64_BD && p.mfma_mode == PREC_BF16X3) {
        BP_CHECK(conv_h16_eligible(p) && p.w16s != nullptr, "filters-direct tile needs the stage-packed filter copy and Cin % 32 == 0");
        BP_CHECK((long long)3 * p.CoutPad * p.Kpad * 2 < (long long)OOB, "filter planes too large for 32-bit offsets");
        launch_h_t<1, 1, 3, true>(p, s);
    } else if (tile == TILE_BD_K2) {
        BP_CHECK(p.mfma_mode == PREC_BF16X3 && conv_h16_eligible(p) && p.w16s != nullptr, "filters-direct K2 tile: bf16x3 mode, stage-packed filter copy, Cin % 32 == 0");
        BP_CHECK((long long)3 * p.CoutPad * p.Kpad * 2 < (long long)OOB, "filter planes too large for 32-bit offsets");
        BP_CHECK(!p.xcd_home && !p.pf_ptr, "filters-direct K2 tile: no latency-mode layouts");
        ConvParams q = p;
        conv_grid_setup(q, 64, 64);
        if (g_conv_prof) hipExtLaunchKernelGGL(conv_igemm_bdk2_kernel, dim3(conv_grid_blocks(q)), dim3(512), 0, s, g_conv_prof->e0, g_conv_prof->e1, 0, q);
        else hipLaunchKernelGGL(conv_igemm_bdk2_kernel, dim3(conv_grid_blocks(q)), dim3(512), 0, s, q);
#ifdef BP_EXPERIMENTAL
    } else if (conv_tile_is_w64(tile)) {
        launch_conv_w64(p, tile, s);
    } else if (conv_tile_is_kg(tile)) {
        launch_conv_kg(p, tile, s);
    } else if (conv_tile_is_rd(tile)) {
        launch_conv_rd(p, tile, s);
    } else if (p.mfma_mode == PREC_F16 && conv_h16_eligible(p)) {
        switch (tile) {
            case TILE_64x64_BD:
                BP_CHECK(p.w16s != nullptr, "filters-direct tile needs the stage-packed filter copy");
                launch_h_t<1, 1, 1, true>(p, s);
                break;
            case TILE_128x64: launch_h_t<2, 1, 1>(p, s); break;
            default: launch_h_t<1, 1, 1>(p, s); break;
        }
    } else if (p.mfma_mode == PREC_BF16X3 && conv_h16_eligible(p)) {
        BP_CHECK(tile == TILE_64x64 && p.w16 != nullptr, "the LDS-staged bf16x3 kernel is built for the 64x64 tile");
        launch_h_t<1, 1, 3>(p, s);
#endif
    } else {
        BP_CHECK(tile == TILE_64x64 || tile == TILE_128x64,
                 "this kernel id exists only in the experimental library (python -m betapose_amd.build --experimental, BP_LIB)");
        switch (tile) {
            case TILE_128x64: launch_t<2, 1>(p, s); break;
            default: launch_t<1, 1>(p, s); break;
        }
    }
    BP_HIP(hipGetLastError());
}

}
```

### betapose_amd/csrc/conv_s1.hip

```cpp
#include <algorithm>
#include <cstdlib>

#include "conv_dev.h"

namespace bp {

struct S1Args {
    int MT;
    int NG;
    int MS;
    int NL;
    int res_bytes;
    int rq;
    int rbuf;
    int off_stg, off_res, off_bias;
    int hw;
};

static constexpr int S1_BM = 32, S1_BN = 128;
static constexpr int S1_STG_FLOATS = 16 * 36;

#define S1_W(n) case n: asm volatile("s_waitcnt vmcnt(" #n ")" ::: "memory"); break;
__device__ __forceinline__ void s1_vm_wait(int allowed) {
    const int a = __builtin_amdgcn_readfirstlane(allowed);
    switch (a < 0 ? 0 : (a > 60 ? 60 : a)) {
        S1_W(0) S1_W(1) S1_W(2) S1_W(3) S1_W(4) S1_W(5) S1_W(6) S1_W(7) S1_W(8) S1_W(9) S1_W(10) S1_W(11) S1_W(12) S1_W(13) S1_W(14) S1_W(15)
        S1_W(16) S1_W(17) S1_W(18) S1_W(19) S1_W(20) S1_W(21) S1_W(22) S1_W(23) S1_W(24) S1_W(25) S1_W(26) S1_W(27) S1_W(28) S1_W(29) S1_W(30)
        S1_W(31) S1_W(32) S1_W(33) S1_W(34) S1_W(35) S1_W(36) S1_W(37) S1_W(38) S1_W(39) S1_W(40) S1_W(41) S1_W(42) S1_W(43) S1_W(44) S1_W(45)
        S1_W(46) S1_W(47) S1_W(48) S1_W(49) S1_W(50) S1_W(51) S1_W(52) S1_W(53) S1_W(54) S1_W(55) S1_W(56) S1_W(57) S1_W(58) S1_W(59)
        default: asm volatile("s_waitcnt vmcnt(60)" ::: "memory"); break;
    }
}
#undef S1_W

template <int NCH, int KH>
__global__ __launch_bounds__(384) void conv_s1_kernel(const ConvParams p, const S1Args a) {
    constexpr int GW = S1_BN / KH;
    constexpr int NCW = NCH / KH;
    extern __shared__ __attribute__((aligned(16))) char lds[];
    const int tid = threadIdx.x, lane = tid & 63;
    const int w = __builtin_amdgcn_readfirstlane(tid >> 6);
    const int nlw = (int)(blockDim.x >> 6) - 4;
    const int oR = a.off_res;
    float* const ldsBias = reinterpret_cast<float*>(lds + a.off_bias);
    const int rrow = GW * a.res_bytes;
    const int rtile = 32 * rrow;
    const int xcd = (int)blockIdx.x & 7, bq = (int)blockIdx.x >> 3;
    const int ng = bq % a.NG, ms = bq / a.NG;
    const int MT8 = (a.MT + 7) >> 3;
    int nit = ms < MT8 ? (MT8 - 1 - ms) / a.MS + 1 : 0;
    if (nit > 0 && (ms + (nit - 1) * a.MS) * 8 + xcd >= a.MT) --nit;
    const int n0 = ng * GW;

    if (tid < GW) ldsBias[tid] = n0 + tid < p.CoutPad ? p.bias[n0 + tid] : 0.f;
    const bool has_res = a.res_bytes != 0, r16 = a.res_bytes == 2, has_scale = p.res_scale != nullptr;
    const float rcp_hw = 1.0f / (float)a.hw, rcp_ow = 1.0f / (float)p.OW;

    if (w >= 4) {
        const int li = w - 4;
        asm volatile("s_waitcnt vmcnt(0) lgkmcnt(0)" ::: "memory");
        __syncthreads();
        if (nit == 0) return;
        const __amdgpu_buffer_rsrc_t rsrcA = __builtin_amdgcn_make_buffer_rsrc(
            const_cast<unsigned short*>(p.in16), 0, (int)min((long long)p.N * p.H * p.W * p.in_ld * 2, (long long)OOB), 0x00020000);
        const __amdgpu_buffer_rsrc_t rsrcR = __builtin_amdgcn_make_buffer_rsrc(
            r16 ? (void*)const_cast<unsigned short*>(p.res16) : (void*)const_cast<float*>(p.res ? p.res : p.out), 0,
            (int)min((long long)p.M * (p.res ? p.res_ld : p.out_ld) * (r16 ? 2 : 4), (long long)OOB), 0x00020000);
        const __amdgpu_buffer_rsrc_t rsrcS = __builtin_amdgcn_make_buffer_rsrc(
            const_cast<float*>(has_scale ? p.res_scale : p.bias), 0, has_scale ? p.N * p.Cout * 4 : 0, 0x00020000);
        int vm = 0;
        int seqa = 0, seqr = 0;
        auto a_issue = [&](int k) __attribute__((always_inline)) {
            if (k >= nit) return;
            const int mt = (ms + k * a.MS) * 8 + xcd, j = k % a.NL;
            const int gsw = (lane & 3) ^ ((lane >> 4) & 3);
            unsigned vo[2];
#pragma unroll
            for (int rg = 0; rg < 2; ++rg) {
                const int m = mt * S1_BM + 16 * rg + (lane >> 2);
                long long pix = m;
                if (p.stride != 1) {
                    const int mm = m < p.M ? m : 0;
                    const int b = fast_div(mm, a.hw, rcp_hw);
                    const int rem = mm - b * a.hw;
                    const int oy = fast_div(rem, p.OW, rcp_ow), ox = rem - oy * p.OW;
                    pix = ((long long)b * p.H + oy * p.stride) * p.W + ox * p.stride;
                }
                vo[rg] = m < p.M ? (unsigned)((pix * p.in_ld + gsw * 8) * 2) : OOB;
            }
            char* const dst = lds + j * (NCH * 2048);
            int cnt = 0;
#pragma unroll
            for (int c = 0; c < NCH; ++c) {
                if (nlw == 2 && (c & 1) != li) continue;
                dma16(rsrcA, dst + c * 2048, vo[0], c * 64);
                dma16(rsrcA, dst + c * 2048 + 1024, vo[1], c * 64);
                cnt += 2;
            }
            vm += cnt;
            seqa = lane == j ? vm : seqa;
        };
        auto r_issue = [&](int k) __attribute__((always_inline)) {
            if (!has_res || li != 0 || k >= nit) return;
            const int mt = (ms + k * a.MS) * 8 + xcd, j = k % a.rq;
            const int m0 = mt * S1_BM;
            char* const dst = lds + oR + j * a.rbuf;
            if (r16) {
                constexpr int LPR = GW / 8, RPP = 64 / LPR, NP_ = 32 / RPP;
#pragma unroll
                for (int i = 0; i < NP_; ++i) {
                    const int m = m0 + RPP * i + lane / LPR, n = n0 + 8 * (lane % LPR);
                    dma16(rsrcR, dst + i * 1024, (m < p.M && n < p.Cout) ? (unsigned)((m * p.res_ld + n) * 2) : OOB, 0);
                }
                vm += NP_;
            } else {
                constexpr int LPR = GW / 4, RPP = 64 / LPR, NP_ = 32 / RPP;
#pragma unroll
                for (int i = 0; i < NP_; ++i) {
                    const int m = m0 + RPP * i + lane / LPR, n = n0 + 4 * (lane % LPR);
                    dma16(rsrcR, dst + i * 1024, (m < p.M && n < p.Cout) ? (unsigned)((m * p.res_ld + n) * 4) : OOB, 0);
                }
                vm += NP_;
            }
            if (has_scale) {
                constexpr int LPI = GW / 4;
                const int b0 = fast_div(min(m0, p.M - 1), a.hw, rcp_hw);
                const int b = min(b0 + lane / LPI, p.N - 1), n = n0 + 4 * (lane % LPI);
                dma16(rsrcS, dst + rtile, (lane < 2 * LPI && n < p.Cout) ? (unsigned)((b * p.Cout + n) * 4) : OOB, 0);
                ++vm;
            }
            seqr = lane == j ? vm : seqr;
        };
        for (int k = 0; k < a.NL; ++k) { a_issue(k); if (k < a.rq) r_issue(k); }
        for (int k = 0; k < nit; ++k) {
            int need = __builtin_amdgcn_readlane(seqa, k % a.NL);
            if (has_res && li == 0) need = max(need, __builtin_amdgcn_readlane(seqr, k % a.rq));
            s1_vm_wait(vm - need);
            asm volatile("s_barrier" ::: "memory");
            if (k > 0) { a_issue(k - 1 + a.NL); r_issue(k - 1 + a.rq); }
            if constexpr (KH == 2) asm volatile("s_barrier" ::: "memory");
        }
        return;
    }

    const __amdgpu_buffer_rsrc_t rsrcB = __builtin_amdgcn_make_buffer_rsrc(
        const_cast<unsigned short*>(p.wpl), 0, (int)((long long)p.CoutPad * p.Kpad * 2), 0x00020000);
    const __amdgpu_buffer_rsrc_t rsrcO =
        __builtin_amdgcn_make_buffer_rsrc(p.out, 0, (int)min((long long)p.M * p.out_ld * 4, (long long)OOB), 0x00020000);
    const PlaneDesc pd = make_plane_desc(p);
    float* const stg = reinterpret_cast<float*>(lds + a.off_stg) + w * S1_STG_FLOATS;
    const int kh = KH == 2 ? (w >> 1) : 0;
    const int wq = KH == 2 ? (w & 1) : w;
    const int fsw = ((lane & 31) >> 2) & 3;
    const int fr0 = (lane & 31) * 64 + ((((lane >> 5)) ^ fsw) << 4), fr1 = fr0 ^ 32;
    f16x8 fb[NCW][2];
    {
        const int col0 = n0 + 32 * wq;
        const int t64 = col0 >> 6;
        const int row_off = ((col0 >> 5) & 1) * 2048;
        auto load_from = [&](auto startc) __attribute__((always_inline)) {
            constexpr int start = decltype(startc)::value;
            static_for<NCW>([&](auto ic) __attribute__((always_inline)) {
                constexpr int c = (decltype(ic)::value + start) % NCW;
                const int so = (t64 * NCH + kh * NCW + c) * 4096 + row_off;
                fb[c][0] = __builtin_bit_cast(f16x8, __builtin_amdgcn_raw_buffer_load_b128(rsrcB, fr0, so, 0));
                fb[c][1] = __builtin_bit_cast(f16x8, __builtin_amdgcn_raw_buffer_load_b128(rsrcB, fr1, so, 0));
            });
        };
        switch (NCW >= 4 ? (ms & 3) : 0) {
            case 1: load_from(std::integral_constant<int, NCW / 4>{}); break;
            case 2: load_from(std::integral_constant<int, NCW / 2>{}); break;
            case 3: load_from(std::integral_constant<int, (3 * NCW) / 4>{}); break;
            default: load_from(std::integral_constant<int, 0>{}); break;
        }
    }
    asm volatile("s_waitcnt vmcnt(0) lgkmcnt(0)" ::: "memory");
    __syncthreads();
    const int e_row = lane >> 3, e_q = lane & 7;
    const int nl = 32 * wq + 4 * e_q, n = n0 + nl;
    const f32x4 bias4 = *reinterpret_cast<const f32x4*>(ldsBias + nl);
    const bool n_ok = n < p.Cout;

    for (int k = 0; k < nit; ++k) {
        const int mt = (ms + k * a.MS) * 8 + xcd;
        const int m0 = mt * S1_BM;
        asm volatile("s_barrier" ::: "memory");
// ... 153 lines not shown
```

### betapose_amd/csrc/engine.cpp

```cpp
#include "engine.h"

#include <algorithm>
#include <cmath>
#include <cstdlib>
#include <cstring>
#include <sstream>

namespace bp {

Arena::~Arena() {
    for (void* p : ptrs_) (void)hipFree(p);
}
void* Arena::alloc_bytes(size_t bytes) {
    void* p = nullptr;
    bytes = (bytes + 255) & ~size_t(255);
    BP_HIP(hipMalloc(&p, bytes));
    ptrs_.push_back(p);
    total_ += bytes;
    return p;
}
float* Arena::alloc(size_t n) { return static_cast<float*>(alloc_bytes(n * sizeof(float))); }

Tensor Net::new_tensor(int H, int W, int C) {
    Tensor t;
// ... 266 lines not shown
    {  1280,   512,    4, TILE_PL64,  1},
    {  1280,   512,    8, TILE_PL64,  1},
    {  1280,   512,   72, TILE_PL64,  3},
    {  2704,    64,    8, TILE_PL64,  1},
    {  2704,   128,    8, TILE_PL64,  1},
    {  2704,   128,   12, TILE_PL64,  1},
    {  2704,   256,   36, TILE_PL64,  1},
    {  5120,    64,    2, TILE_PL64,  1},
    {  5120,    64,    8, TILE_PL64,  1},
    {  5120,    64,   18, TILE_PL64,  1},
    {  5120,    64,   36, TILE_PL64,  2},
    {  5120,   128,    8, TILE_PL64,  1},
    {  5120,   256,    2, TILE_PL64,  1},
    { 10816,    64,    4, TILE_PL64,  1},
    { 10816,   128,   18, TILE_PL64,  1},
    { 43264,    64,    2, TILE_PL64,  1},
    { 43264,    64,    9, TILE_PL64,  1},
    {0, 0, 0, 0, 0},
};
static const PlanEntry kPlanPL1[] = {
    {    80,   512,   64, TILE_PL64,  4},
    {    80,   512,  144, TILE_PL64,  6},
    {    80,  2048,   16, TILE_PL64,  1},
    {    80,  2048,   32, TILE_PL64,  1},
    {   169,    64,   32, TILE_PL64,  4},
    {   169,   256,   16, TILE_PL64,  3},
    {   169,   512,   32, TILE_PL64,  4},
    {   169,  1024,  144, TILE_PL64,  4},
    {   320,   256,   32, TILE_PL64,  4},
    {   320,   256,   72, TILE_PL64,  4},
    {   320,   512,   32, TILE_PL64,  3},
    {   320,  1024,    8, TILE_PL64,  1},
    {   320,  1024,   16, TILE_PL64,  1},
    {   320,  1024,  144, TILE_PL64,  3},
    {   676,    64,   16, TILE_PL64,  1},
    {   676,   128,    8, TILE_PL64,  1},
    {   676,   256,   16, TILE_PL64,  1},
    {   676,   256,   24, TILE_PL64,  1},
    {   676,   512,   72, TILE_PL64,  2},
    {  1280,   128,   16, TILE_PL64,  1},
    {  1280,   128,   36, TILE_PL64,  3},
    {  1280,   256,   16, TILE_PL64,  1},
    {  1280,   512,    4, TILE_PL64,  1},
    {  1280,   512,    8, TILE_PL64,  1},
    {  1280,   512,   72, TILE_PL64,  3},
    {  2704,    64,    8, TILE_PL64,  1},
    {  2704,   128,    8, TILE_PL64,  1},
    {  2704,   128,   12, TILE_PL64,  1},
    {  2704,   256,   36, TILE_PL64,  1},
    {  5120,    64,    2, TILE_PL64,  1},
    {  5120,    64,    8, TILE_PL64,  1},
    {  5120,    64,   18, TILE_PL64,  1},
    {  5120,    64,   36, TILE_PL64,  1},
    {  5120,   128,    8, TILE_PL64,  1},
    {  5120,   256,    2, TILE_PL64,  1},
    { 10816,    64,    4, TILE_PL64,  1},
    { 10816,   128,   18, TILE_PL64,  1},
    { 43264,    64,    2, TILE_PL64,  1},
    { 43264,    64,    9, TILE_PL64,  1},
    {   4732,  1024,  144, TILE_PLH128,  1},
    {   8960,  1024,  144, TILE_PLH128,  1},
    {  35840,   512,   72, TILE_PLH128,  1},
    {   8960,   256,   72, TILE_PLH128,  1},
    {  18928,   512,   72, TILE_PLH128,  1},
    {  35840,   128,   36, TILE_PLH128,  1},
    {  75712,   256,   36, TILE_PLH128,  1},
    { 302848,   128,   18, TILE_PLH128,  1},
    {   2240,   512,   64, TILE_PL64,  1},
    {   2240,   512,  144, TILE_PL64,  1},
    {   2240,  2048,   16, TILE_PL64,  1},
    {   2240,  2048,   32, TILE_PL128,  1},
    {   4732,    64,   32, TILE_PL64,  1},
    {   4732,   256,   16, TILE_PL128x64,  1},
    {   4732,   512,   32, TILE_PL64,  1},
    {   4732,  1024,  144, TILE_PL128,  1},
    {   8960,   256,   32, TILE_PL64,  1},
    {   8960,   256,   72, TILE_PL64,  1},
    {   8960,   512,   32, TILE_PL64,  1},
    {   8960,  1024,    8, TILE_PL64,  1},
    {   8960,  1024,   16, TILE_PL64,  1},
    {   8960,  1024,  144, TILE_PL256x128,  1},
    {  18928,    64,   16, TILE_PL64,  1},
    {  18928,   128,    8, TILE_PL64,  1},
    {  18928,   256,   16, TILE_PL64,  1},
    {  18928,   256,   24, TILE_PL64,  1},
    {  18928,   512,   72, TILE_PL256x128,  1},
    {  35840,   128,   16, TILE_PL64,  1},
    {  35840,   128,   36, TILE_PL64,  1},
    {  35840,   256,   16, TILE_PL64,  1},
    {  35840,   512,    4, TILE_PL64,  1},
    {  35840,   512,    8, TILE_PL64,  1},
    {  35840,   512,   72, TILE_PL256x128,  1},
    {  75712,    64,    8, TILE_PL64,  1},
    {  75712,   128,    8, TILE_PL64,  1},
    {  75712,   128,   12, TILE_PL256x128,  1},
    {  75712,   256,   36, TILE_PL128,  1},
    { 143360,    64,    2, TILE_PL64,  1},
    { 143360,    64,    8, TILE_PL64,  1},
    { 143360,    64,   18, TILE_PL64,  1},
    { 143360,    64,   36, TILE_PL64,  1},
    { 143360,   128,    8, TILE_PL64,  1},
    { 143360,   256,    2, TILE_PL64,  1},
    { 302848,    64,    4, TILE_PL64,  1},
    { 302848,   128,   18, TILE_PL256x128,  1},
    {1211392,    64,    2, TILE_PL64,  1},
    {1211392,    64,    9, TILE_PL64,  1},
    {0, 0, 0, 0, 0},
};

static bool plh_ok(const ConvParams& c) {
    static const bool w63 = std::getenv("BP_PLH_W63") != nullptr;
    return conv_plh_eligible(c) && (c.W <= 63 || !w63);
}

static void choose_pl(const ConvParams& c, long long M, int mode, int sk_max, int* tile, int* splits) {
    for (const PlanEntry& e : plan_file_entries())
        if (e.M == (int)M && e.CoutPad == c.CoutPad && e.nchunks == c.nchunks && conv_tile_is_pl(e.tile) &&
            (!conv_tile_is_plh(e.tile) || plh_ok(c)) &&
            (e.tile != TILE_S1 || (e.splits == 1 && conv_s1_eligible(c, M))) &&
            (e.tile != TILE_P3 || (e.splits == 1 && conv_p3_eligible(c, M)))) { *tile = e.tile; *splits = e.splits; return; }
    for (const PlanEntry* e = (mode == PREC_F16 ? kPlanPL1 : kPlanPL3); e->M != 0; ++e)
        if (e->M == (int)M && e->CoutPad == c.CoutPad && e->nchunks == c.nchunks &&
            (!conv_tile_is_plh(e->tile) || plh_ok(c))) { *tile = e->tile; *splits = e->splits; return; }
    const long long tiles128 = ((M + 127) / 128) * ((c.CoutPad + 127) / 128);
    int t = (c.CoutPad >= 128 && tiles128 >= 192 && c.nchunks >= 32) ? TILE_PL128 : TILE_PL64;
    if (t == TILE_PL128 && mode == PREC_F16 && plh_ok(c)) t = TILE_PLH128;
    int s = 1;
    if (t == TILE_PL64) {
        const long long blocks = ((M + 63) / 64) * (c.CoutPad / 64);
        const int min_chunks = mode == PREC_F16 ? 8 : 4;
        while (blocks * s < 256 && c.nchunks / (s + 1) >= min_chunks && s < sk_max) ++s;
    }
    *tile = t; *splits = s;
}
#ifdef BP_EXPERIMENTAL
static void pl64_form(const ConvParams& c, int mode, int* tile) {
    static const bool bd = std::getenv("BP_B3_PL64BD") != nullptr;
    if (*tile == TILE_PL64 && mode == PREC_BF16X3 && c.wbd && bd) *tile = TILE_PL64BD;
}
#else
static void pl64_form(const ConvParams&, int, int*) {}
#endif

static void choose_h16(const ConvParams& c, long long M, int mode, int sk_max, int* tile, int* splits, bool lone = false) {
#ifdef BP_EXPERIMENTAL
    static const bool legacy = std::getenv("BP_LEGACY") != nullptr;
#else
    constexpr bool legacy = false;
#endif
    if (conv_pl_eligible(c) && !legacy) { choose_pl(c, M, mode, sk_max, tile, splits); pl64_form(c, mode, tile); return; }
    if (mode == PREC_BF16X3)
        for (const PlanEntry& e : plan_file_entries())
            if (e.M == (int)M && e.CoutPad == c.CoutPad && e.nchunks == c.nchunks && !conv_tile_is_pl(e.tile) &&
                (!conv_tile_is_halo(e.tile) || conv_halo_eligible(c, e.tile))) { *tile = e.tile; *splits = e.splits; return; }
    static const bool halo_off = std::getenv("BP_NO_HALO") != nullptr;
#ifdef BP_EXPERIMENTAL
    for (const PlanEntry* e = (mode == PREC_F16 ? kPlanF16 : kPlanB3); e->M != 0; ++e)
#else
    for (const PlanEntry* e = kPlanB3; e->M != 0; ++e)
#endif
        if (e->M == (int)M && e->CoutPad == c.CoutPad && e->nchunks == c.nchunks &&
            (!conv_tile_is_halo(e->tile) || (!halo_off && mode == PREC_BF16X3 && conv_halo_eligible(c, e->tile)))) {
            *tile = e->tile; *splits = e->splits;
            if (lone && e->tile == TILE_BD_K2)
                for (const PlanEntry* l = kPlanB3Lone; l->M != 0; ++l)
                    if (l->M == e->M && l->CoutPad == e->CoutPad && l->nchunks == e->nchunks) { *tile = l->tile; *splits = l->splits; break; }
            return;
        }
    int t = TILE_64x64_BD;
    static const int halo_min_tiles = std::getenv("BP_HALO_BATCH_MIN_TILES") ? std::atoi(std::getenv("BP_HALO_BATCH_MIN_TILES")) : 64;
    if (mode == PREC_BF16X3 && !halo_off && c.in16 == nullptr) {
        const int ht = conv_halo_eligible(c, TILE_HALO128) ? TILE_HALO128 : (conv_halo_eligible(c, TILE_HALO64K2) ? TILE_HALO64K2 : -1);
        if (ht >= 0 && ((M + 63) / 64) * (c.CoutPad / conv_tile_bn(ht)) >= halo_min_tiles) { *tile = ht; *splits = 1; return; }
    }
#ifdef BP_EXPERIMENTAL
    const long long tiles128 = ((M + 127) / 128) * ((c.CoutPad + 127) / 128);
    if (!(mode == PREC_BF16X3 && c.w16s)) t = (c.CoutPad >= 128 && tiles128 >= 128) ? TILE_W64_2x2 : TILE_64x64;
#endif
    const int bm = conv_tile_bm(t), bn = conv_tile_bn(t);
    const long long blocks = ((M + bm - 1) / bm) * ((c.CoutPad + bn - 1) / bn);
    const int target = t == TILE_W64_2x2 ? 256 : (mode == PREC_F16 ? 128 : 512);
    const int min_chunks = mode == PREC_F16 ? 8 : 4;
    int s = 1;
    while (blocks * s < target && c.nchunks / (s + 1) >= min_chunks && s < sk_max) ++s;
    *tile = t; *splits = s;
}

static bool tile_runs(int tile, const ConvParams& c, long long M = 0) {
    const bool on_planes = c.in16 != nullptr && c.wpl != nullptr;
    if (tile == TILE_64x64 || tile == TILE_128x64) return !on_planes;
    if (tile == TILE_S1) return conv_s1_eligible(c, M);
    if (tile == TILE_P3) return conv_p3_eligible(c, M);
    if (conv_tile_is_pl(tile)) return c.mfma_mode != PREC_F32 && conv_pl_eligible(c) && (!conv_tile_is_plh(tile) || conv_plh_eligible(c));
    if (tile == TILE_64x64_BD || tile == TILE_BD_K2) return c.mfma_mode == PREC_BF16X3 && conv_h16_eligible(c) && c.w16s != nullptr && !on_planes;
    if (conv_tile_is_halo(tile)) return c.mfma_mode == PREC_BF16X3 && c.in16 == nullptr && conv_halo_eligible(c, tile);
#ifdef BP_EXPERIMENTAL
    if (tile >= 0 && tile <= TILE_LAST) return c.mfma_mode != PREC_F32 && conv_h16_eligible(c);
#endif
    return false;
}

static bool stem3_wanted(const ConvParams& c, int force_tile) {
    static const bool off = std::getenv("BP_NO_STEM3") != nullptr;
    return !off && (force_tile < 0 || force_tile == TILE_STEM3) && conv_stem3_eligible(c);
}

static bool stem7_wanted(const ConvParams& c, int force_tile) {
    static const bool off = std::getenv("BP_NO_STEM7") != nullptr;
    return !off && force_tile < 0 && c.net_prec == PREC_F16 && conv_stem7_eligible(c);
}

static void choose_launch(const Op& op, int batch, int force_tile, int sk_target, int sk_min_chunks, int sk_max,
                          int* tile, int* splits, int* cps, bool lone = false) {
    const int mode = op.conv.mfma_mode;
    const ConvParams& c = op.conv;
    const long long M = (long long)batch * c.OH * c.OW;
    int t = TILE_64x64;
    int s = 1;
    if (mode != PREC_F32) {
        choose_h16(c, M, mode, sk_max, &t, &s, lone);
        if (t == TILE_S1 && op.pool_out) t = TILE_PL64;
        static const bool s1_off = std::getenv("BP_NO_S1") != nullptr;
        if (!s1_off && mode == PREC_F16 && s == 1 && conv_tile_is_pl(t) && !op.pool_out && conv_s1_eligible(c, M)) t = TILE_S1;
        static const bool p3_off = std::getenv("BP_NO_P3") != nullptr;
        if (!p3_off && mode == PREC_F16 && s == 1 && t == TILE_PLH128 && !op.pool_out && conv_p3_eligible(c, M)) t = TILE_P3;
        static const int p3_k1 = std::getenv("BP_P3_K1") ? std::atoi(std::getenv("BP_P3_K1")) : 1;
        if (!p3_off && p3_k1 && mode == PREC_F16 && s == 1 && c.ksize == 1 && conv_tile_is_pl(t) && !op.pool_out && conv_p3_eligible(c, M) &&
            (p3_k1 == 2 || c.Cin >= 512)) t = TILE_P3;
        if (force_tile >= 0 && !((force_tile == TILE_S1 || force_tile == TILE_P3) && op.pool_out) && tile_runs(force_tile, c, M)) t = force_tile;
        if (!(sk_target == 512 && sk_min_chunks == 4 && sk_max == 8)) {
            const long long blocks = ((M + conv_tile_bm(t) - 1) / conv_tile_bm(t)) *
                                     ((c.CoutPad + conv_tile_bn(t) - 1) / conv_tile_bn(t));
            s = 1;
            while (blocks * s < sk_target && c.nchunks / (s + 1) >= sk_min_chunks && s < sk_max) ++s;
        }
        if (t == TILE_S1 || t == TILE_P3) s = 1;
    } else if (stem3_wanted(c, force_tile)) {
        t = TILE_STEM3;
    } else if (stem7_wanted(c, force_tile)) {
        t = TILE_STEM7;
    } else {
        if ((force_tile == TILE_64x64 || force_tile == TILE_128x64) && tile_runs(force_tile, c)) t = force_tile;
        const int bm = conv_tile_bm(t);
        const long long blocks = ((M + bm - 1) / bm) * (c.CoutPad / 64);
        while (blocks * s < sk_target && c.nchunks / (s + 1) >= sk_min_chunks && s < sk_max) ++s;
        if (t == TILE_64x64 && sk_target == 512 && sk_min_chunks == 4 && sk_max == 8)
            for (const SplitEntry& e : kSplitTable)
                if (e.M == (int)M && e.CoutPad == c.CoutPad && e.nchunks == c.nchunks) { s = e.splits; break; }
    }
    {
        static const int pct = std::getenv("BP_SPLIT_PCT") ? std::atoi(std::getenv("BP_SPLIT_PCT")) : 100;
        if (pct != 100 && s > 1) s = std::max(1, (s * pct + 50) / 100);
    }
    int per = 0;
    conv_split_plan(c, t, s, &s, &per);
    *tile = t; *splits = s; *cps = per;
}

int Net::add_conv(const std::string& name, const Tensor& in, const Tensor& out_view, const ConvWeights& cw, int Cout,
                  int k, int stride, int pad, int act, int store_mode, const Tensor* res, const float* res_scale,
                  int res_after_act, float bn_eps, int OH, int OW) {
    const int Cin = in.C;
    const int cpk = Cin <= 4 ? 4 : Cin;
    const int K = k * k * cpk;
    const int Kpad = round_up(K, 32);
    const int CoutPad = round_up(Cout, 64);
    float *dW, *dB;
    if (reuse_) {
        dW = upload_weights(nullptr, 0);
        dB = upload_weights(nullptr, 0);
    } else {
        std::vector<float> W((size_t)CoutPad * Kpad, 0.f), B(CoutPad, 0.f);
        for (int co = 0; co < Cout; ++co) {
            double s = 1.0, b = 0.0;
            if (cw.bn_scale) {
                s = darknet_bn_ ? (double)cw.bn_scale[co] / (std::sqrt((double)cw.bn_var[co]) + 1e-6)
                                : (double)cw.bn_scale[co] / std::sqrt((double)cw.bn_var[co] + (double)bn_eps);
                b = (double)cw.bn_bias[co] - (double)cw.bn_mean[co] * s;
            } else if (cw.bias) {
                b = cw.bias[co];
            }
            int n = co;
            if (store_mode == ST_PIXSHUF) n = (co & 3) * (Cout / 4) + (co >> 2);
            B[n] = (float)b;
            float* dst = W.data() + (size_t)n * Kpad;
            const float* src = cw.w + (size_t)co * Cin * k * k;
            for (int ci = 0; ci < Cin; ++ci)
                for (int t = 0; t < k * k; ++t) dst[(size_t)t * cpk + ci] = (float)((double)src[(size_t)ci * k * k + t] * s);
        }
        dW = upload_weights(W.data(), W.size());
        dB = upload_weights(B.data(), B.size());
    }

    Op op;
    op.type = OP_CONV;
    op.name = name;
    ConvParams& c = op.conv;
    c.in = in.p; c.in_ld = in.ld; c.N = 1; c.H = in.H; c.W = in.W; c.Cin = Cin;
    c.w = dW; c.Kpad = Kpad; c.Ktrue = K; c.bias = dB; c.cin_pack = cpk;
    c.out = out_view.p; c.out_ld = out_view.ld; c.OH = OH; c.OW = OW; c.Cout = Cout;
    c.ksize = k; c.stride = stride; c.pad = pad; c.act = act;
    c.res = res ? res->p : nullptr; c.res_ld = res ? res->ld : 0; c.res_scale = res_scale;
    c.res_after_act = res_after_act; c.store_mode = store_mode;
    c.M = OH * OW; c.nchunks = Kpad / 32; c.splits = 1; c.chunks_per_split = c.nchunks; c.partial = nullptr;
    c.tickets = nullptr;
    c.stamps = nullptr;
    c.w16 = nullptr; c.w16s = nullptr;
    c.in16 = nullptr; c.out16 = nullptr; c.wpl = nullptr; c.wbd = nullptr; c.in16_plane = c.out16_plane = 0; c.out_np = 0; c.abl = 0; c.skip_f32 = 0; c.res16 = nullptr; c.net_prec = PREC_F32;
    c.pool_out = nullptr; c.hy_full = c.hy_splits = c.hy_cps = 0;
    c.pf_ptr = nullptr; c.xcd_home = 0; c.xcc_of = nullptr; c.err_word = nullptr; c.tickets_local = nullptr; c.mtiles = c.n_tiles = c.work_blocks = c.pf_first = 0;
    c.pf_ntn = c.pf_splits = c.pf_cps = c.pf_nchunks = c.pf_tile_stride = c.pf_chunk_bytes = c.pf_cap = 0;
    c.CoutPad = CoutPad;
    const double Kalg = (double)k * k * Cin;
    op.flops = 2.0 * OH * OW * (double)Cout * Kalg;
    op.bytes = 4.0 * ((double)Cout * Kalg + (double)in.H * in.W * Cin + (double)OH * OW * Cout + (res ? (double)OH * OW * Cout : 0.0));
    ops_.push_back(op);
    return (int)ops_.size() - 1;
}

size_t Net::workspace_need() const {
    size_t need = 0;
    for (const Op& op : ops_) {
        if (op.type != OP_CONV) continue;
        for (int lone = 0; lone < 2; ++lone)
            for (int b = 1; b <= max_batch_; ++b) {
                int tile, splits, cps;
                choose_launch(op, b, force_tile_, sk_target_, sk_min_chunks_, 64, &tile, &splits, &cps, lone != 0);
                ConvParams q = op.conv; q.N = b; q.M = b * q.OH * q.OW; q.splits = splits;
                if (splits > 1) {
                    need = std::max(need, (size_t)splits * conv_tiles(q, tile) * conv_tile_bm(tile) * conv_tile_bn(tile));
                } else {
                    int full = 0, hs = 0, hcps = 0;
                    if (conv_hybrid_plan(q, tile, (size_t)-1, &full, &hs, &hcps))
                        need = std::max(need, (size_t)hs * (conv_tiles(q, tile) - full) * conv_tile_bm(tile) * conv_tile_bn(tile));
                }
            }
    }
    return std::max(need, (size_t)4 << 20);
}

void Net::find_fuse_groups() {
    fuse_groups_.clear();
    auto readers = [&](const float* t) {
        int n = 0;
        for (const Op& o : ops_) {
            if (o.type == OP_CONV) n += (o.conv.in == t) + (o.conv.res == t);
            else n += (o.a == t) + (o.b == t);
        }
        return n;
    };
    auto producer = [&](const float* t, int ld) {
        int idx = -1, n = 0;
        for (int i = 0; i < (int)ops_.size(); ++i) {
            const Op& o = ops_[i];
            if (o.type == OP_CONV ? (o.conv.out == t && o.conv.out_ld == ld) : o.out == t) { idx = i; ++n; }
        }
        return n == 1 ? idx : -1;
    };
    auto private_out = [&](const ConvParams& c) {
        for (const float* q : f32_readers_) if (q == c.out) return false;
        const ActAlloc* a = find_act(c.out);
        return a == nullptr || (a->base == c.out && c.out_ld == c.Cout);
    };
    for (int j = 0; j < (int)ops_.size(); ++j) {
        const Op& c3 = ops_[j];
        if (c3.type != OP_CONV || c3.conv.ksize != 3 || c3.conv.stride != 1 || c3.conv.pad != 1) continue;
        const int i = producer(c3.conv.in, c3.conv.in_ld);
        if (i < 0 || i >= j || ops_[i].type != OP_CONV) continue;
        const ConvParams& pre = ops_[i].conv;
        if (!(pre.ksize == 1 && pre.stride == 1 && pre.res == nullptr && pre.res_scale == nullptr && pre.store_mode == ST_NHWC && pre.Cout == c3.conv.Cin)) continue;
        if (readers(pre.out) != 1 || !private_out(pre) || ops_[i].pool_out) continue;
        if (i != j - 1) continue;
        FuseGroup g{i, j, -1};
        if (j + 1 < (int)ops_.size() && ops_[j + 1].type == OP_CONV) {
            const ConvParams& post = ops_[j + 1].conv;
            if (post.in == c3.conv.out && post.in_ld == c3.conv.out_ld && post.ksize == 1 && post.stride == 1 && c3.conv.res == nullptr &&
                c3.conv.store_mode == ST_NHWC && readers(c3.conv.out) == 1 && private_out(c3.conv) && !ops_[j].pool_out)
                g.post = j + 1;
        }
        fuse_groups_.push_back(g);
    }
}

void Net::plan_roles(int batch) {
    if (roles_batch_ == batch && roles_version_ == plan_version_) return;
    roles_.assign(ops_.size(), FR_NONE);
    role_group_.assign(ops_.size(), -1);
    roles_batch_ = batch; roles_version_ = plan_version_;
    static const bool env_off = std::getenv("BP_NO_FUSION") != nullptr;
// ... 1015 lines not shown
```

### betapose_amd/ops.py

```python
from __future__ import annotations

import ctypes as C
from typing import Optional

import numpy as np

from . import _lib

ACT = {"linear": 0, "leaky": 1, "relu": 2}
STORE = {"nhwc": 0, "up2": 1, "pixshuf": 2, "nchw": 3}
_F16, _B3 = 256, 512
TILE = {"auto": -1, "64x64": 0, "128x64": 1, "stem3": 20, "stem7": 28, "64x64_f16": _F16, "128x64_f16": _F16 + 1, "64x64_b3": _B3, "bd_b3": _B3 + 12,
        "bd_f16": _F16 + 12, "halo64_b3": _B3 + 21, "halo128_b3": _B3 + 22, "halo64k2_b3": _B3 + 23, "bdk2_b3": _B3 + 24}
for _n, _i in (("w1x1", 2), ("w1x2", 3), ("w2x1", 5), ("w2x2", 6), ("pl64", 13), ("pl128", 14), ("pl128x64", 15), ("pl256x128", 16), ("pl128s", 17), ("pl64k2", 18), ("pl64bd", 19), ("plh128", 25), ("s1", 26), ("p3", 27)):
    TILE[_n + "_f16"] = _F16 + _i
    TILE[_n + "_b3"] = _B3 + _i
for _n, _i in (("kg1", 7), ("kg2", 8), ("kg4", 9), ("rd4", 10), ("rd8", 11)):
    TILE[_n + "_b3"] = _B3 + _i


def conv2d_nhwc(x, weight, bias=None, stride: int = 1, pad: int = 0, act: str = "linear", store: str = "nhwc",
                res=None, res_after_act: bool = False, tile: str = "auto", splits: int = 0, iters: int = 0,
                planes: bool = False):
    import torch
    _lib.require_gpu()
    w = np.ascontiguousarray(weight.detach().cpu().numpy() if hasattr(weight, "detach") else weight, dtype=np.float32)
    b = None
    if bias is not None:
        b = np.ascontiguousarray(bias.detach().cpu().numpy() if hasattr(bias, "detach") else bias, dtype=np.float32)
    N, H, W, Cin = x.shape
    Cout, _, k, _ = w.shape
    OH, OW = (H + 2 * pad - k) // stride + 1, (W + 2 * pad - k) // stride + 1
    x = x.contiguous()
    if store == "nhwc":
        out = torch.empty((N, OH, OW, Cout), device=x.device, dtype=torch.float32)
    elif store == "up2":
        out = torch.empty((N, 2 * OH, 2 * OW, Cout), device=x.device, dtype=torch.float32)
    elif store == "pixshuf":
        out = torch.empty((N, 2 * OH, 2 * OW, Cout // 4), device=x.device, dtype=torch.float32)
    else:
        out = torch.empty((N, Cout, OH, OW), device=x.device, dtype=torch.float32)
    ms = C.c_float(0)
    pl = None
    if planes:
        assert store != "nchw", "NCHW outputs (the heat-maps) have no operand planes"
        pl = torch.zeros((1 if TILE[tile] < _B3 else 3,) + tuple(out.shape), device=x.device, dtype=torch.int16)
    _lib.check(_lib.lib().bp_conv2d_planes(x.data_ptr(), N, H, W, Cin, w.ctypes.data, b.ctypes.data if b is not None else None,
                                           Cout, k, stride, pad, ACT[act], STORE[store],
                                           res.contiguous().data_ptr() if res is not None else None, int(res_after_act),
                                           TILE[tile], int(splits), out.data_ptr(), pl.data_ptr() if planes else None,
                                           int(iters), C.byref(ms), _lib.current_stream()))
    ret = (out,) + ((pl,) if planes else ()) + ((ms.value,) if iters > 0 else ())
    return ret if len(ret) > 1 else out


def crop(frames_bgr_u8, sel=None, boxes=None, reso: int = 416, oh: int = 320, ow: int = 256, nchw: bool = True):
    import torch
    _lib.require_gpu()
    f = frames_bgr_u8.contiguous()
    B, H, W, _ = f.shape
    out = torch.empty((B, 3, oh, ow) if nchw else (B, oh, ow, 3), device=f.device, dtype=torch.float32)
    pts = torch.empty((B, 8), device=f.device, dtype=torch.float32)
    _lib.check(_lib.lib().bp_crop(f.data_ptr(), B, H, W, sel.contiguous().data_ptr() if sel is not None else None, reso,
                                  boxes.contiguous().data_ptr() if boxes is not None else None,
                                  out.data_ptr() if nchw else None, None if nchw else out.data_ptr(), pts.data_ptr(),
                                  oh, ow, _lib.current_stream()))
    return out, pts


def crop_candidates(frames_bgr_u8, candidates: int, sel=None, boxes=None, reso: int = 416, oh: int = 320, ow: int = 256,
                    nchw: bool = True):
    import torch
    _lib.require_gpu()
    f = frames_bgr_u8.contiguous()
    F, H, W, _ = f.shape
    Cn = int(candidates)
    B = F * Cn
    src = sel if sel is not None else boxes
    src = src.contiguous().reshape(B, -1)
    assert src.shape[1] == (8 if sel is not None else 4)
    out = torch.empty((B, 3, oh, ow) if nchw else (B, oh, ow, 3), device=f.device, dtype=torch.float32)
    pts = torch.empty((B, 8), device=f.device, dtype=torch.float32)
    _lib.check(_lib.lib().bp_crop_candidates(f.data_ptr(), F, Cn, H, W, src.data_ptr() if sel is not None else None, reso,
                                             src.data_ptr() if sel is None else None,
                                             out.data_ptr() if nchw else None, None if nchw else out.data_ptr(), pts.data_ptr(),
                                             oh, ow, _lib.current_stream()))
    return out, pts


def select_nms(pred, max_candidates: int, nms_conf: float, class_id: int = 0, confidence: float = 0.01, num_classes: int = 80):
    import torch
    _lib.require_gpu()
    p = pred.contiguous()
    assert p.dtype == torch.float32 and p.dim() == 3
    B, rows, attrs = p.shape
    Cn = int(max_candidates)
    sel = torch.empty((B, Cn, 8), device=p.device, dtype=torch.float32)
    counts = torch.empty((B,), device=p.device, dtype=torch.int32)
    _lib.check(_lib.lib().bp_yolo_select_nms(p.data_ptr(), B, rows, attrs, float(confidence), int(num_classes), int(class_id),
                                             float(nms_conf), Cn, sel.data_ptr(), counts.data_ptr(), _lib.current_stream()))
    return sel, counts


def pose_from_candidate_records(records, counts, kp3d, K, left_number: int = 50):
    import torch
    _lib.require_gpu()
    rec = records.contiguous()
    assert rec.dtype == torch.float32 and rec.dim() == 3 and rec.shape[2] == _lib.RESULT_FLOATS
    F, Cn = rec.shape[0], rec.shape[1]
    cnt = counts.to(device=rec.device, dtype=torch.int32).contiguous()
    assert cnt.shape == (F,)
    k3 = torch.as_tensor(np.asarray(kp3d, dtype=np.float64).reshape(-1, 3), device=rec.device).contiguous()
    Kc = np.ascontiguousarray(K, dtype=np.float64)
    poses = torch.empty((F, _lib.POSE_DOUBLES), dtype=torch.float64, device=rec.device)
    merged = torch.zeros((F, Cn, _lib.MERGED_FLOATS), dtype=torch.float32, device=rec.device)
    info = torch.zeros((F, 4), dtype=torch.int32, device=rec.device)
    _lib.check(_lib.lib().bp_pose_from_candidate_records(rec.data_ptr(), cnt.data_ptr(), F, Cn, k3.data_ptr(), k3.shape[0],
                                                         Kc.ctypes.data, int(left_number), poses.data_ptr(), merged.data_ptr(),
                                                         info.data_ptr(), _lib.current_stream()))
    return poses, merged, info


def pose_instances(merged, info, poses, kp3d, K, left_number: int = 50):
    import torch
    _lib.require_gpu()
    mg = merged.contiguous()
    assert mg.dtype == torch.float32 and mg.dim() == 3 and mg.shape[2] == _lib.MERGED_FLOATS
    F, Cn = mg.shape[0], mg.shape[1]
    inf = info.to(device=mg.device, dtype=torch.int32).contiguous()
    ps = poses.to(device=mg.device, dtype=torch.float64).contiguous()
    assert inf.shape == (F, 4) and ps.shape == (F, _lib.POSE_DOUBLES)
    k3 = torch.as_tensor(np.asarray(kp3d, dtype=np.float64).reshape(-1, 3), device=mg.device).contiguous()
    Kc = np.ascontiguousarray(K, dtype=np.float64)
    inst = torch.empty((F, Cn, _lib.POSE_DOUBLES), dtype=torch.float64, device=mg.device)
    _lib.check(_lib.lib().bp_pose_instances_from_merged(mg.data_ptr(), inf.data_ptr(), ps.data_ptr(), F, Cn, k3.data_ptr(),
                                                        k3.shape[0], Kc.ctypes.data, int(left_number), inst.data_ptr(),
                                                        _lib.current_stream()))
    return inst


def resize_bicubic(frames_u8, oh: int = 416, ow: int = 416, swap_rb: bool = True, want: str = "f32"):
    import torch
    _lib.require_gpu()
    f = frames_u8.contiguous()
    B, H, W, _ = f.shape
    if want == "u8":
        out = torch.empty((B, oh, ow, 3), device=f.device, dtype=torch.uint8)
        _lib.check(_lib.lib().bp_resize_bicubic(f.data_ptr(), B, H, W, oh, ow, int(swap_rb), out.data_ptr(), None,
                                                _lib.current_stream()))
    else:
        out = torch.empty((B, oh, ow, 3), device=f.device, dtype=torch.float32)
        _lib.check(_lib.lib().bp_resize_bicubic(f.data_ptr(), B, H, W, oh, ow, int(swap_rb), None, out.data_ptr(),
                                                _lib.current_stream()))
    return out


def solve_pnp(points_3d, points_2d, K, method: str = "iterative"):
    p3 = np.ascontiguousarray(points_3d, dtype=np.float64)
    p2 = np.ascontiguousarray(np.asarray(points_2d)[:, :2], dtype=np.float64)
    assert p3.shape[0] == p2.shape[0], "points 3D and points 2D must have same number of vertices"
    Kc = np.ascontiguousarray(K, dtype=np.float64)
    R = np.empty((3, 3), np.float64)
    t = np.empty(3, np.float64)
    fn = {"iterative": _lib.lib().bp_solve_pnp, "refined": _lib.lib().bp_solve_pnp_refined}[method]
    _lib.check(fn(p3.ctypes.data, p2.ctypes.data, p3.shape[0], Kc.ctypes.data, R.ctypes.data, t.ctypes.data))
    return R, t.reshape(3, 1)


def solve_pnp_status(points_3d, points_2d, K):
    p3 = np.ascontiguousarray(points_3d, dtype=np.float64)
    p2 = np.ascontiguousarray(np.asarray(points_2d)[:, :2], dtype=np.float64)
    assert p3.shape[0] == p2.shape[0], "points 3D and points 2D must have same number of vertices"
    Kc = np.ascontiguousarray(K, dtype=np.float64)
    R = np.empty((3, 3), np.float64)
    t = np.empty(3, np.float64)
    st = C.c_int(0)
    _lib.check(_lib.lib().bp_solve_pnp_status(p3.ctypes.data, p2.ctypes.data, p3.shape[0], Kc.ctypes.data, R.ctypes.data,
                                              t.ctypes.data, C.addressof(st)))
    if st.value != 0:
        return [], [], int(st.value)
    return R, t.reshape(3, 1), 0


def solve_pnp_batch(points_3d, points_2d, K):
    import torch
    _lib.require_gpu()
    p2 = torch.as_tensor(points_2d, dtype=torch.float64).cuda().contiguous()
    assert p2.dim() == 3 and p2.shape[2] >= 2, "points_2d must be [P, n, 2]"
    p2 = p2[:, :, :2].contiguous()
    P, n = p2.shape[0], p2.shape[1]
    p3 = torch.as_tensor(points_3d, dtype=torch.float64).to(p2.device).contiguous()
    shared = p3.dim() == 2
    assert p3.shape[-2:] == (n, 3) and (shared or p3.shape[0] == P), "points 3D and points 2D must have same number of vertices"
    Kc = np.ascontiguousarray(K, dtype=np.float64)
    Rt = torch.empty((P, 3, 4), dtype=torch.float64, device=p2.device)
    st = torch.empty(P, dtype=torch.int32, device=p2.device)
    _lib.check(_lib.lib().bp_solve_pnp_batch(p3.data_ptr(), int(shared), p2.data_ptr(), n, P, Kc.ctypes.data,
                                             Rt.data_ptr(), st.data_ptr(), _lib.current_stream()))
    return Rt[:, :, :3].contiguous(), Rt[:, :, 3:].contiguous(), st


def pose_from_records(records, kp3d, K, left_number: int = 50):
# ... 91 lines not shown
```

### include/betapose_hip.h

```cpp
#ifndef BETAPOSE_HIP_H
#define BETAPOSE_HIP_H

#include <stddef.h>
#include <stdint.h>

#ifdef __cplusplus
extern "C" {
#endif

typedef struct bp_yolo bp_yolo;
typedef struct bp_kpd bp_kpd;
typedef struct bp_pipeline bp_pipeline;
typedef struct bp_scene bp_scene;
typedef struct bp_cands bp_cands;

#define BP_RESULT_FLOATS 316
#define BP_KP_FLOATS 6
#define BP_SEL_FLOATS 8
#define BP_MAX_SCENE_CLASSES 16
#define BP_MAX_CANDIDATES 8
#define BP_MERGED_FLOATS 152

#define BP_POSE_DOUBLES 166
#define BP_PNP_MAX_POINTS 64

const char* bp_last_error(void);
int bp_version(void);
int bp_device_count(void);
int bp_device_name(int device, char* out, int cap);

int bp_yolo_create(const char* cfg_path, const char* weights_path, int reso, int max_batch, int device, bp_yolo** out);
int bp_yolo_create_from_memory(const char* cfg_text, const float* stream, size_t n_floats, int reso, int max_batch,
                               int device, bp_yolo** out);
int bp_yolo_clone(const bp_yolo* y, bp_yolo** out);
void bp_yolo_destroy(bp_yolo* y);
int bp_yolo_rows(const bp_yolo* y);
int bp_yolo_attrs(const bp_yolo* y);
int bp_yolo_forward(bp_yolo* y, const float* d_img_nchw, int batch, float* d_pred, void* stream);
int bp_yolo_forward_select(bp_yolo* y, const float* d_img_nchw, int batch, float conf, int num_classes, float* d_pred,
                           float* d_sel, void* stream);
int bp_yolo_forward_select_classes(bp_yolo* y, const float* d_img_nchw, int batch, float conf, int num_classes,
                                   const int* class_ids, int K, float* d_pred, float* d_sel, void* stream);
int bp_yolo_select(const float* d_pred, int batch, int rows, int attrs, float conf, int num_classes, float* d_sel,
                   void* stream);
int bp_yolo_select_nms(const float* d_pred, int batch, int rows, int attrs, float conf, int num_classes, int class_id,
                       float nms_conf, int max_candidates, float* d_sel, int* d_counts, void* stream);
int bp_yolo_forward_select_nms(bp_yolo* y, const float* d_img_nchw, int batch, float conf, int num_classes, int class_id,
                               float nms_conf, int max_candidates, float* d_pred, float* d_sel, int* d_counts, void* stream);
int bp_yolo_tap_count(const bp_yolo* y);
int bp_yolo_tap_info(const bp_yolo* y, int i, char* name, int cap, int* C, int* H, int* W);
int bp_yolo_tap_copy(bp_yolo* y, int i, int batch, float* d_out_nchw, void* stream);

int bp_kpd_create(const float* stream, size_t n_floats, int n_classes, int max_batch, int device, bp_kpd** out);
int bp_kpd_clone(const bp_kpd* k, bp_kpd** out);
void bp_kpd_destroy(bp_kpd* k);
int bp_kpd_forward(bp_kpd* k, const float* d_inps_nchw, int batch, float* d_hm, void* stream);
int bp_kpd_forward_argmax(bp_kpd* k, const float* d_inps_nchw, int batch, float* d_hm, float* d_kp, void* stream);
int bp_kpd_launch_count(bp_kpd* k, int batch);
int bp_kpd_tap_count(const bp_kpd* k);
int bp_kpd_tap_info(const bp_kpd* k, int i, char* name, int cap, int* C, int* H, int* W);
int bp_kpd_tap_copy(bp_kpd* k, int i, int batch, float* d_out_nchw, void* stream);

int bp_yolo_set_policy(bp_yolo* y, int sk_target_blocks, int sk_min_chunks, int sk_max_splits, int force_tile);
int bp_kpd_set_policy(bp_kpd* k, int sk_target_blocks, int sk_min_chunks, int sk_max_splits, int force_tile);
int bp_yolo_set_precision(bp_yolo* y, int precision);
int bp_kpd_set_precision(bp_kpd* k, int precision);
int bp_yolo_op_stats(const bp_yolo* y, double* flops, double* bytes, int cap);
int bp_kpd_op_stats(const bp_kpd* k, double* flops, double* bytes, int cap);
int bp_yolo_profile(bp_yolo* y, int batch, int iters, float* ms, int* info, int cap, void* stream);
int bp_calibrate_ticks(long long ticks, float* ms, void* stream);
int bp_yolo_set_prefetch(bp_yolo* y, int on);
int bp_kpd_set_prefetch(bp_kpd* k, int on);
int bp_yolo_set_fusion(bp_yolo* y, int on);
int bp_kpd_set_fusion(bp_kpd* k, int on);
int bp_yolo_fused_launches(bp_yolo* y, int batch, int* launches);
int bp_kpd_fused_launches(bp_kpd* k, int batch, int* launches);
int bp_yolo_xcd_errors(bp_yolo* y, int* count, void* stream);
int bp_kpd_xcd_errors(bp_kpd* k, int* count, void* stream);
int bp_yolo_set_stamps(bp_yolo* y, unsigned long long* d_buf, int slots);
int bp_kpd_set_stamps(bp_kpd* k, unsigned long long* d_buf, int slots);
int bp_yolo_op_name(const bp_yolo* y, int i, char* out, int cap);
int bp_kpd_op_name(const bp_kpd* k, int i, char* out, int cap);
int bp_kpd_profile(bp_kpd* k, int batch, int iters, float* ms, int* info, int cap, void* stream);
size_t bp_yolo_device_bytes(const bp_yolo* y);
size_t bp_kpd_device_bytes(const bp_kpd* k);

int bp_crop(const uint8_t* d_frames, int batch, int H, int W, const float* d_sel, int reso, const float* d_boxes,
            float* d_out_nchw, float* d_out_nhwc, float* d_pts, int oh, int ow, void* stream);
int bp_crop_candidates(const uint8_t* d_frames, int frames, int C, int H, int W, const float* d_sel, int reso,
                       const float* d_boxes, float* d_out_nchw, float* d_out_nhwc, float* d_pts, int oh, int ow, void* stream);
int bp_resize_bicubic(const uint8_t* d_in, int batch, int H, int W, int oh, int ow, int swap_rb, uint8_t* d_out_u8,
                      float* d_out_nhwc, void* stream);
int bp_heatmap_argmax(const float* d_hm, int batch, int C, int H, int W, float* d_kp, void* stream);
int bp_pose_errors(const double* d_model, int n, const double* d_gt, const double* d_est, int P,
                   const double* K, int want, double* d_out, void* stream);
int bp_pose_errors_sym(const double* d_model, int n, const double* d_gt, const double* d_est, int P, const double* d_sym,
                       int S, const double* K, int want, double* d_out, void* stream);
int bp_render_depth(const double* d_model, int n, const int* d_faces, int F, const double* d_poses, int P, const double* K,
                    int H, int W, double pixel_center, double near_z, float* d_depth, int* d_skipped, void* stream);
int bp_render_depth_host(const double* poses, int P, const double* vertices, int n, const int* faces, int F, const double* K,
                         int H, int W, double pixel_center, double near_z, float* depth, int* skipped);
int bp_vsd_errors(const double* d_model, int n, const int* d_faces, int F, const double* d_gt, const double* d_est, int P,
                  const double* K, const uint16_t* d_depth_test, int T, int H, int W, double depth_scale,
                  const int* d_test_index, double delta, const double* taus, int n_tau, double diameter, double pixel_center,
                  double near_z, int chunk, double* d_err, int* d_counts, void* stream);
int bp_refine_depth(const double* d_model, int n, const int* d_faces, int F, const double* d_poses, int P, const double* K,
                    const uint16_t* d_depth_test, int T, int H, int W, double depth_scale, const int* d_test_index,
                    int iterations, double max_dist, double min_cos, int min_pixels, double pixel_center, double near_z,
                    int chunk, double* d_poses_out, double* d_stats, void* stream);
int bp_refine_depth_host(const double* poses, int P, const double* vertices, int n, const int* faces, int F, const double* K,
                         const uint16_t* depth_test, int T, int H, int W, double depth_scale, const int* test_index,
                         int iterations, double max_dist, double min_cos, int min_pixels, double pixel_center, double near_z,
                         double* poses_out, double* stats);
int bp_icp_normal_equations(const double* d_model, int n, const int* d_faces, int F, const double* d_poses, int P,
                            const double* K, const uint16_t* d_depth_test, int T, int H, int W, double depth_scale,
                            const int* d_test_index, double max_dist, double min_cos, double pixel_center, double near_z,
                            int chunk, double* d_out, void* stream);
int bp_icp_normal_equations_host(const double* poses, int P, const double* vertices, int n, const int* faces, int F,
                                 const double* K, const uint16_t* depth_test, int T, int H, int W, double depth_scale,
                                 const int* test_index, double max_dist, double min_cos, double pixel_center, double near_z,
                                 double* out);
int bp_conv2d(const float* d_in, int N, int H, int W, int Cin, const float* h_w, const float* h_bias, int Cout, int k,
              int stride, int pad, int act, int store_mode, const float* d_res, int res_after_act, int tile, int splits,
              float* d_out, int iters, float* ms_per_iter, void* stream);
int bp_conv2d_planes(const float* d_in, int N, int H, int W, int Cin, const float* h_w, const float* h_bias, int Cout, int k,
                     int stride, int pad, int act, int store_mode, const float* d_res, int res_after_act, int tile, int splits,
                     float* d_out, unsigned short* d_out_planes, int iters, float* ms_per_iter, void* stream);

int bp_pipeline_create(bp_yolo* y, bp_kpd* k, int frame_h, int frame_w, int batch, float conf, int num_classes,
                       uint8_t* d_frames, float* d_results, float* d_hm, bp_pipeline** out);
void bp_pipeline_destroy(bp_pipeline* p);
uint8_t* bp_pipeline_frames(bp_pipeline* p);
int bp_pipeline_kernel_count(bp_pipeline* p);
float* bp_pipeline_results(bp_pipeline* p);
float* bp_pipeline_heatmaps(bp_pipeline* p);
int bp_pipeline_set_fixed_box(bp_pipeline* p, const float* box_xyxy_or_null);
int bp_pipeline_run(bp_pipeline* p, int use_graph, void* stream);
int bp_pipeline_latency_faults(const bp_pipeline* p);
int bp_pipeline_prepare(bp_pipeline* p);

int bp_pipeline_set_pose_solver(bp_pipeline* p, const double* kp3d, int n_kp, const double* K, int left_number,
                                double* d_poses);
double* bp_pipeline_poses(bp_pipeline* p);
int bp_pose_from_records(const float* d_records, int batch, const double* d_kp3d, int n_kp, const double* K, int left_number,
                         double* d_poses, void* stream);
int bp_solve_pnp_batch(const double* d_pts3d, int shared_3d, const double* d_pts2d, int n, int P, const double* K,
                       double* d_Rt, int* d_status, void* stream);

int bp_pnp_ransac_samples(int n, int max_trials, int* idx);
int bp_pnp_ransac_trials_needed(int n, double confidence, int* need);
size_t bp_pnp_ransac_workspace_bytes(int P, int max_trials);
int bp_solve_pnp_ransac_batch(const double* d_pts3d, int shared_3d, const double* d_pts2d, int n, int P, const double* K,
                              double reproj_err, int max_trials, double confidence, double* d_Rt, int* d_status,
                              unsigned char* d_inliers, void* d_workspace, size_t workspace_bytes, void* stream);
int bp_pipeline_set_pose_ransac(bp_pipeline* p, double reproj_err, int max_trials, double confidence);
size_t bp_pose_ransac_workspace_bytes(int batch, int max_trials);
int bp_pose_from_records_ransac(const float* d_records, int batch, const double* d_kp3d, int n_kp, const double* K,
                                int left_number, double reproj_err, int max_trials, double confidence, double* d_poses,
                                void* d_workspace, size_t workspace_bytes, void* stream);

int bp_scene_create(bp_yolo* y, bp_kpd* const* kpds, const int* class_ids, int K, int frame_h, int frame_w, float conf,
                    int num_classes, uint8_t* d_frames, float* d_results, bp_scene** out);
void bp_scene_destroy(bp_scene* s);
float* bp_scene_results(bp_scene* s);
int bp_scene_set_pose_solver(bp_scene* s, int k, const double* kp3d, int n_kp, const double* K, int left_number,
                             double* d_poses_row);
int bp_scene_set_pose_ransac(bp_scene* s, int k, double reproj_err, int max_trials, double confidence);
double* bp_scene_poses(bp_scene* s);
int bp_scene_prepare(bp_scene* s);
int bp_scene_run(bp_scene* s, int use_graph, void* stream);
int bp_scene_kernel_count(bp_scene* s);

int bp_cands_create(bp_yolo* y, bp_kpd* k, int max_candidates, int frame_h, int frame_w, float conf, int num_classes,
                    int class_id, float nms_conf, uint8_t* d_frame, float* d_results, bp_cands** out);
void bp_cands_destroy(bp_cands* s);
float* bp_cands_results(bp_cands* s);
int* bp_cands_counts(bp_cands* s);
int bp_cands_prepare(bp_cands* s);
int bp_cands_run(bp_cands* s, int use_graph, void* stream);
int bp_cands_kernel_count(bp_cands* s);
int bp_cands_set_pose_solver(bp_cands* s, const double* kp3d, int n_kp, const double* K, int left_number, double* d_pose);
double* bp_cands_pose(bp_cands* s);
float* bp_cands_merged(bp_cands* s);
int* bp_cands_info(bp_cands* s);
int bp_pose_from_candidate_records(const float* d_records, const int* d_counts, int frames, int C, const double* d_kp3d,
                                   int n_kp, const double* K, int left_number, double* d_poses, float* d_merged, int* d_info,
                                   void* stream);
int bp_cands_set_instance_poses(bp_cands* s, int on, double* d_inst_poses);
double* bp_cands_instance_poses(bp_cands* s);
int bp_pose_instances_from_merged(const float* d_merged, const int* d_info, const double* d_poses, int frames, int C,
                                  const double* d_kp3d, int n_kp, const double* K, int left_number, double* d_inst_poses,
                                  void* stream);

int bp_solve_pnp(const double* pts3d, const double* pts2d, int n, const double* K, double* R, double* t);
int bp_solve_pnp_status(const double* pts3d, const double* pts2d, int n, const double* K, double* R, double* t, int* status);
int bp_solve_pnp_refined(const double* pts3d, const double* pts2d, int n, const double* K, double* R, double* t);
int bp_solve_pnp_ransac(const double* pts3d, const double* pts2d, int n, const double* K, double reproj_err,
                        int max_trials, double confidence, double* R, double* t, unsigned char* inliers);
int bp_pose_nms(const float* bboxes, const float* bbox_scores, const float* preds, const float* scores, int n, int K,
                int* out_pick, float* out_pose, float* out_score, float* out_prop);

typedef struct bp_darknet bp_darknet;
typedef struct bp_bbox {
    unsigned int x, y, w, h;
    float prob;
    unsigned int obj_id, track_id, frames_counter;
} bp_bbox;
const char* bp_darknet_last_error(void);
int bp_darknet_create(const char* cfg_path, const char* weights_path, int device, bp_darknet** out);
void bp_darknet_destroy(bp_darknet* d);
int bp_darknet_width(const bp_darknet* d);
int bp_darknet_height(const bp_darknet* d);
int bp_darknet_classes(const bp_darknet* d);
int bp_darknet_detect_rgb(bp_darknet* d, const float* planar_rgb, int w, int h, float thresh, float nms, bp_bbox* out,
                          int cap);
int bp_darknet_detect_image(bp_darknet* d, const unsigned char* data, size_t n, float thresh, float nms, bp_bbox* out,
                            int cap);
int bp_image_decode_rgb(const unsigned char* data, size_t n, unsigned char* out_rgb, size_t cap, int* h, int* w);
int bp_darknet_detect_png(bp_darknet* d, const unsigned char* png, size_t n, float thresh, float nms, bp_bbox* out,
                          int cap);
int bp_darknet_detect_file(bp_darknet* d, const char* png_path, float thresh, float nms, bp_bbox* out, int cap);
int bp_yolo_create_darknet(const char* cfg_path, const char* weights_path, int reso, int max_batch, int device,
                           bp_yolo** out);

int bp_stream_create_masked(const uint32_t* cu_mask, int words, void** out_stream);
int bp_stream_destroy(void* stream);
int bp_probe_placement(int blocks, int* h_xcc, int* h_hw_id, void* stream);

int bp_png_info(const unsigned char* data, size_t n, int* h, int* w, int* channels);
int bp_png_decode_bgr(const unsigned char* data, size_t n, unsigned char* out_bgr, size_t cap, int* h, int* w);
typedef struct bp_loader bp_loader;
int bp_loader_create(const char* const* paths, int n, int H, int W, int threads, int depth, int pinned, bp_loader** out);
void bp_loader_destroy(bp_loader* l);
int bp_loader_next(bp_loader* l, long long* index, const unsigned char** bgr);
int bp_loader_release(bp_loader* l, long long index);
int bp_upload(void* d_dst, const void* h_src, size_t bytes, void* stream);

#ifdef __cplusplus
}
#endif
#endif
```

Baseline: 1021.

## Add streaming warp-specialized bf16x3 1x1 conv tile for stride-1 layers

Adds a new bf16x3 kernel for 1x1 stride-1 convolutions. It splits each block into producer waves that stream activations and residuals into LDS via buffer-to-LDS DMA, and consumer waves that run the MFMA products, with fine-grained vmcnt waits. The engine now picks this tile automatically wherever the filters-direct tile was chosen and the layer qualifies, so those 1x1 layers should see less load latency and better overlap. The cost is a large new kernel, more LDS use, and a new dispatch path for a subset of layers. It can be disabled with an environment variable.

```diff
diff --git a/betapose_amd/_lib.py b/betapose_amd/_lib.py
--- a/betapose_amd/_lib.py
+++ b/betapose_amd/_lib.py
@@ -68,6 +68,9 @@
                             C.c_int, C.c_int, vp, C.c_int, C.c_int, C.c_int, vp, C.c_int, c_float_p, vp]),
     "bp_conv2d_planes": (C.c_int, [vp, C.c_int, C.c_int, C.c_int, C.c_int, vp, vp, C.c_int, C.c_int, C.c_int, C.c_int,
                                    C.c_int, C.c_int, vp, C.c_int, C.c_int, C.c_int, vp, vp, C.c_int, c_float_p, vp]),
+    "bp_conv2d_scaled": (C.c_int, [vp, C.c_int, C.c_int, C.c_int, C.c_int, vp, vp, C.c_int, C.c_int, C.c_int, C.c_int,
+                                   C.c_int, C.c_int, vp, vp, C.c_int, C.c_int, C.c_int, vp, vp, C.c_int, c_float_p, vp]),
+    "bp_conv_tile_eligible": (C.c_int, [C.c_int] * 12),
     "bp_pipeline_create": (C.c_int, [vp, vp, C.c_int, C.c_int, C.c_int, C.c_float, C.c_int, vp, vp, vp, C.POINTER(vp)]),
     "bp_pipeline_kernel_count": (C.c_int, [vp]),
     "bp_yolo_profile": (C.c_int, [vp, C.c_int, C.c_int, c_float_p, c_int_p, C.c_int, vp]),
diff --git a/betapose_amd/build.py b/betapose_amd/build.py
--- a/betapose_amd/build.py
+++ b/betapose_amd/build.py
@@ -8,7 +8,7 @@
 HERE = os.path.dirname(os.path.abspath(__file__))
 CSRC = os.path.join(HERE, "csrc")
 LIB = os.path.join(HERE, "libbetapose_hip.so")
-SOURCES = ["conv_igemm.hip", "conv_halo.hip", "conv_fused.hip", "conv_pl.hip", "conv_s1.hip", "conv_p3.hip", "aux_kernels.hip", "pose_metrics.hip", "pose_metrics_sym.hip", "raster.hip", "vsd.hip", "icp.hip", "pose_tail.hip", "pose_tail_cands.hip", "pose_tail_inst.hip", "pnp_ransac.hip", "engine.cpp", "host_post.cpp", "raster_host.cpp", "icp_host.cpp", "frame_io.cpp", "jpeg_bmp.cpp", "c_api.cpp", "darknet_compat.cpp"]
+SOURCES = ["conv_igemm.hip", "conv_halo.hip", "conv_fused.hip", "conv_pl.hip", "conv_s1.hip", "conv_s1b3.hip", "conv_p3.hip", "aux_kernels.hip", "pose_metrics.hip", "pose_metrics_sym.hip", "raster.hip", "vsd.hip", "icp.hip", "pose_tail.hip", "pose_tail_cands.hip", "pose_tail_inst.hip", "pnp_ransac.hip", "engine.cpp", "host_post.cpp", "raster_host.cpp", "icp_host.cpp", "frame_io.cpp", "jpeg_bmp.cpp", "c_api.cpp", "darknet_compat.cpp"]
 HEADERS = ["bp_common.h", "engine.h", "frame_chain.h", "frame_io.h", "conv_tail.inc", "pnp_wave.inc", "pnp_math.inc", "pose_decode.inc", "pose_tail.h", "raster.h", "raster_math.inc", "icp.h", "icp_math.inc", "conv_dev.h", os.path.join("..", "..", "include", "betapose_hip.h"),
            os.path.join("..", "..", "include", "yolo_v2_class_compat.h")]
 EXP = "experimental"
@@ -16,8 +16,8 @@
 EXP_HEADERS = [os.path.join(EXP, s_) for s_ in ("mega.inc", "kernels_unity.hip")]
 ARCH = "gfx950"
 LAST_ACTION = None
-MIN_STUBS = {"conv_s1.hip": 1, "conv_p3.hip": 39, "conv_igemm.hip": 14, "conv_halo.hip": 13, "conv_fused.hip": 12, "conv_pl.hip": 12, "aux_kernels.hip": 21, "pose_metrics.hip": 2, "pose_metrics_sym.hip": 4, "raster.hip": 3, "vsd.hip": 2, "icp.hip": 4, "pose_tail.hip": 3, "pose_tail_cands.hip": 1, "pose_tail_inst.hip": 1, "pnp_ransac.hip": 2}
-MIN_STUBS_EXP = {"conv_s1.hip": 1, "conv_p3.hip": 39, "experimental/kernels_unity.hip": 26, "conv_fused.hip": 12, "conv_pl.hip": 12, "experimental/conv_w64.hip": 8,
+MIN_STUBS = {"conv_s1.hip": 1, "conv_s1b3.hip": 3, "conv_p3.hip": 39, "conv_igemm.hip": 14, "conv_halo.hip": 13, "conv_fused.hip": 12, "conv_pl.hip": 12, "aux_kernels.hip": 21, "pose_metrics.hip": 2, "pose_metrics_sym.hip": 4, "raster.hip": 3, "vsd.hip": 2, "icp.hip": 4, "pose_tail.hip": 3, "pose_tail_cands.hip": 1, "pose_tail_inst.hip": 1, "pnp_ransac.hip": 2}
+MIN_STUBS_EXP = {"conv_s1.hip": 1, "conv_s1b3.hip": 3, "conv_p3.hip": 39, "experimental/kernels_unity.hip": 26, "conv_fused.hip": 12, "conv_pl.hip": 12, "experimental/conv_w64.hip": 8,
                  "experimental/conv_kg.hip": 3, "experimental/conv_rd.hip": 2, "aux_kernels.hip": 24, "pose_metrics.hip": 2, "pose_metrics_sym.hip": 4, "raster.hip": 3, "vsd.hip": 2, "icp.hip": 4, "pose_tail.hip": 3, "pose_tail_cands.hip": 1, "pose_tail_inst.hip": 1, "pnp_ransac.hip": 2}
 
 
diff --git a/betapose_amd/csrc/bp_common.h b/betapose_amd/csrc/bp_common.h
--- a/betapose_amd/csrc/bp_common.h
+++ b/betapose_amd/csrc/bp_common.h
@@ -128,7 +128,8 @@
                       TILE_S1 = 26,
                       TILE_P3 = 27,
                       TILE_STEM7 = 28,
-                      TILE_LAST = 27,
+                      TILE_S1B3 = 29,
+                      TILE_LAST = 29,
                       TILE_FUSED = 40 };
 
 struct ConvProfHook { hipEvent_t e0, e1; };
@@ -154,6 +155,8 @@
 bool conv_pl_eligible(const ConvParams& p);
 bool conv_s1_eligible(const ConvParams& p, long long M);
 void launch_conv_s1(const ConvParams& p, hipStream_t s);
+bool conv_s1b3_eligible(const ConvParams& p, long long M);
+void launch_conv_s1b3(const ConvParams& p, hipStream_t s);
 bool conv_p3_eligible(const ConvParams& p, long long M);
 void launch_conv_p3(const ConvParams& p, hipStream_t s);
 void launch_pack_wpl(const float* in, unsigned short* out, int CoutPad, int Kpad, int Cin, int ksize, int np, hipStream_t s);
diff --git a/betapose_amd/csrc/c_api.cpp b/betapose_amd/csrc/c_api.cpp
--- a/betapose_amd/csrc/c_api.cpp
+++ b/betapose_amd/csrc/c_api.cpp
@@ -828,7 +828,38 @@
 int bp_conv2d_planes(const float* d_in, int N, int H, int W, int Cin, const float* h_w, const float* h_bias, int Cout, int k,
                      int stride, int pad, int act, int store_mode, const float* d_res, int res_after_act, int tile, int splits,
                      float* d_out, unsigned short* d_out_planes, int iters, float* ms_per_iter, void* stream) {
-    BP_TRY
+    return bp_conv2d_scaled(d_in, N, H, W, Cin, h_w, h_bias, Cout, k, stride, pad, act, store_mode, d_res, nullptr, res_after_act, tile,
+                            splits, d_out, d_out_planes, iters, ms_per_iter, stream);
+}
+
+int bp_conv_tile_eligible(int tile, int precision, int N, int H, int W, int Cin, int Cout, int k, int stride, int pad, int store_mode,
+                          int pooled) {
+    BP_TRY
+    BP_CHECK(tile == bp::TILE_S1B3, "eligibility is answered for the streaming bf16x3 1x1 tile (29) only");
+    BP_CHECK(N > 0 && H > 0 && W > 0 && Cin > 0 && Cout > 0 && k > 0 && stride > 0 && pad >= 0, "bad argument");
+    static float present;
+    bp::ConvParams p{};
+    const int cpk = Cin <= 4 ? 4 : Cin;
+    p.in = &present; p.in_ld = Cin; p.N = N; p.H = H; p.W = W; p.Cin = Cin;
+    p.w = &present; p.Ktrue = k * k * cpk; p.Kpad = (p.Ktrue + 31) / 32 * 32; p.nchunks = p.Kpad / 32; p.cin_pack = cpk;
+    p.bias = &present; p.out = &present; p.out_ld = store_mode == bp::ST_PIXSHUF ? Cout / 4 : Cout;
+    p.OH = (H + 2 * pad - k) / stride + 1; p.OW = (W + 2 * pad - k) / stride + 1; p.Cout = Cout; p.CoutPad = (Cout + 63) / 64 * 64;
+    p.ksize = k; p.stride = stride; p.pad = pad; p.store_mode = store_mode; p.splits = 1; p.chunks_per_split = p.nchunks;
+    p.M = N * p.OH * p.OW;
+    const bool h16 = precision != bp::PREC_F32 && Cin % 32 == 0;
+    p.mfma_mode = h16 ? (precision == bp::PREC_F16_RES ? (int)bp::PREC_F16 : precision) : (int)bp::PREC_F32;
+    p.net_prec = precision;
+    if (h16) p.w16s = reinterpret_cast<const unsigned short*>(&present);
+    if (pooled) p.pool_out = &present;
+    return bp::conv_s1b3_eligible(p, p.M) ? 1 : 0;
+    BP_CATCH
+}
+
+int bp_conv2d_scaled(const float* d_in, int N, int H, int W, int Cin, const float* h_w, const float* h_bias, int Cout, int k,
+                     int stride, int pad, int act, int store_mode, const float* d_res, const float* d_res_scale, int res_after_act,
+                     int tile, int splits, float* d_out, unsigned short* d_out_planes, int iters, float* ms_per_iter, void* stream) {
+    BP_TRY
+    BP_CHECK(!d_res_scale || d_res, "a residual scale needs a residual");
     BP_CHECK(d_in && h_w && d_out, "null argument");
     hipStream_t s = (hipStream_t)stream;
     struct OneConv : bp::Net {
@@ -846,7 +877,7 @@
     out.ld = store_mode == bp::ST_PIXSHUF ? Cout / 4 : Cout;
     bp::Tensor res; res.p = const_cast<float*>(d_res); res.ld = Cout; res.C = Cout; res.H = OH; res.W = OW;
     bp::ConvWeights cw; cw.w = h_w; cw.bias = h_bias;
-    net.add_conv("conv", in, out, cw, Cout, k, stride, pad, act, store_mode, d_res ? &res : nullptr, nullptr,
+    net.add_conv("conv", in, out, cw, Cout, k, stride, pad, act, store_mode, d_res ? &res : nullptr, d_res_scale,
                  res_after_act, 1e-5f, OH, OW);
     int t = tile;
     int prec = bp::PREC_F32;
@@ -857,7 +888,7 @@
         net.set_precision(prec);
         net.ops_[0].conv.mfma_mode = prec;
 #ifndef BP_EXPERIMENTAL
-        BP_CHECK(bp::conv_tile_is_pl(t) || ((t == bp::TILE_64x64_BD || t == bp::TILE_BD_K2 || bp::conv_tile_is_halo(t)) && prec == bp::PREC_BF16X3),
+        BP_CHECK(bp::conv_tile_is_pl(t) || ((t == bp::TILE_64x64_BD || t == bp::TILE_BD_K2 || t == bp::TILE_S1B3 || bp::conv_tile_is_halo(t)) && prec == bp::PREC_BF16X3),
                  "this kernel id exists only in the experimental library (python -m betapose_amd.build --experimental, BP_LIB)");
 #endif
     } else {
@@ -916,7 +947,7 @@
         sp = 1;
         while (blocks * sp < 512 && p.nchunks / (sp + 1) >= 4 && sp < 64) ++sp;
     }
-    if (t == bp::TILE_S1 || t == bp::TILE_P3) sp = 1;
+    if (t == bp::TILE_S1 || t == bp::TILE_P3 || t == bp::TILE_S1B3) sp = 1;
     int per = 0;
     bp::conv_split_plan(p, t, sp, &sp, &per);
     p.splits = sp; p.chunks_per_split = per;
diff --git a/betapose_amd/csrc/conv_dev.h b/betapose_amd/csrc/conv_dev.h
--- a/betapose_amd/csrc/conv_dev.h
+++ b/betapose_amd/csrc/conv_dev.h
@@ -61,6 +61,19 @@
 __device__ __forceinline__ void dma16(__amdgpu_buffer_rsrc_t rsrc, char* lds, unsigned voff, int soff) {
     __builtin_amdgcn_raw_ptr_buffer_load_lds(rsrc, (lds_void_t*)lds, 16, (int)voff, soff, 0, 0);
 }
+
+#define S1_W(n) case n: asm volatile("s_waitcnt vmcnt(" #n ")" ::: "memory"); break;
+__device__ __forceinline__ void s1_vm_wait(int allowed) {
+    const int a = __builtin_amdgcn_readfirstlane(allowed);
+    switch (a < 0 ? 0 : (a > 60 ? 60 : a)) {
+        S1_W(0) S1_W(1) S1_W(2) S1_W(3) S1_W(4) S1_W(5) S1_W(6) S1_W(7) S1_W(8) S1_W(9) S1_W(10) S1_W(11) S1_W(12) S1_W(13) S1_W(14) S1_W(15)
+        S1_W(16) S1_W(17) S1_W(18) S1_W(19) S1_W(20) S1_W(21) S1_W(22) S1_W(23) S1_W(24) S1_W(25) S1_W(26) S1_W(27) S1_W(28) S1_W(29) S1_W(30)
+        S1_W(31) S1_W(32) S1_W(33) S1_W(34) S1_W(35) S1_W(36) S1_W(37) S1_W(38) S1_W(39) S1_W(40) S1_W(41) S1_W(42) S1_W(43) S1_W(44) S1_W(45)
+        S1_W(46) S1_W(47) S1_W(48) S1_W(49) S1_W(50) S1_W(51) S1_W(52) S1_W(53) S1_W(54) S1_W(55) S1_W(56) S1_W(57) S1_W(58) S1_W(59)
+        default: asm volatile("s_waitcnt vmcnt(60)" ::: "memory"); break;
+    }
+}
+#undef S1_W
 
 __device__ __forceinline__ int xcc_id() {
     unsigned id;
diff --git a/betapose_amd/csrc/conv_igemm.hip b/betapose_amd/csrc/conv_igemm.hip
--- a/betapose_amd/csrc/conv_igemm.hip
+++ b/betapose_amd/csrc/conv_igemm.hip
@@ -925,13 +925,13 @@
     switch (tile) {
         case TILE_128x64: case TILE_W64_2x1: case TILE_W64_2x2: case TILE_PL128: case TILE_PL128x64: case TILE_PL128S: case TILE_PLH128: case TILE_P3: return 128;
         case TILE_PL256x128: return 256;
-        case TILE_S1: return 32;
+        case TILE_S1: case TILE_S1B3: return 32;
         default: return 64;
     }
 }
 int conv_tile_bn(int tile) {
     switch (tile) {
-        case TILE_W64_1x2: case TILE_W64_2x2: case TILE_PL128: case TILE_PL256x128: case TILE_PL128S: case TILE_HALO128: case TILE_PLH128: case TILE_S1: case TILE_P3: return 128;
+        case TILE_W64_1x2: case TILE_W64_2x2: case TILE_PL128: case TILE_PL256x128: case TILE_PL128S: case TILE_HALO128: case TILE_PLH128: case TILE_S1: case TILE_S1B3: case TILE_P3: return 128;
         default: return 64;
     }
 }
@@ -1008,6 +1008,8 @@
         launch_conv_pl(p, tile, s);
     } else if (conv_tile_is_halo(tile)) {
         launch_conv_halo(p, tile, s);
+    } else if (tile == TILE_S1B3) {
+        launch_conv_s1b3(p, s);
     } else if (tile == TILE_64x64_BD && p.mfma_mode == PREC_BF16X3) {
         BP_CHECK(conv_h16_eligible(p) && p.w16s != nullptr, "filters-direct tile needs the stage-packed filter copy and Cin % 32 == 0");
         BP_CHECK((long long)3 * p.CoutPad * p.Kpad * 2 < (long long)OOB, "filter planes too large for 32-bit offsets");
diff --git a/betapose_amd/csrc/conv_s1.hip b/betapose_amd/csrc/conv_s1.hip
--- a/betapose_amd/csrc/conv_s1.hip
+++ b/betapose_amd/csrc/conv_s1.hip
@@ -19,19 +19,6 @@
 
 static constexpr int S1_BM = 32, S1_BN = 128;
 static constexpr int S1_STG_FLOATS = 16 * 36;
-
-#define S1_W(n) case n: asm volatile("s_waitcnt vmcnt(" #n ")" ::: "memory"); break;
-__device__ __forceinline__ void s1_vm_wait(int allowed) {
-    const int a = __builtin_amdgcn_readfirstlane(allowed);
-    switch (a < 0 ? 0 : (a > 60 ? 60 : a)) {
-        S1_W(0) S1_W(1) S1_W(2) S1_W(3) S1_W(4) S1_W(5) S1_W(6) S1_W(7) S1_W(8) S1_W(9) S1_W(10) S1_W(11) S1_W(12) S1_W(13) S1_W(14) S1_W(15)
-        S1_W(16) S1_W(17) S1_W(18) S1_W(19) S1_W(20) S1_W(21) S1_W(22) S1_W(23) S1_W(24) S1_W(25) S1_W(26) S1_W(27) S1_W(28) S1_W(29) S1_W(30)
-        S1_W(31) S1_W(32) S1_W(33) S1_W(34) S1_W(35) S1_W(36) S1_W(37) S1_W(38) S1_W(39) S1_W(40) S1_W(41) S1_W(42) S1_W(43) S1_W(44) S1_W(45)
-        S1_W(46) S1_W(47) S1_W(48) S1_W(49) S1_W(50) S1_W(51) S1_W(52) S1_W(53) S1_W(54) S1_W(55) S1_W(56) S1_W(57) S1_W(58) S1_W(59)
-        default: asm volatile("s_waitcnt vmcnt(60)" ::: "memory"); break;
-    }
-}
-#undef S1_W
 
 template <int NCH, int KH>
 __global__ __launch_bounds__(384) void conv_s1_kernel(const ConvParams p, const S1Args a) {
diff --git a/betapose_amd/csrc/conv_s1b3.hip b/betapose_amd/csrc/conv_s1b3.hip
--- /dev/null
+++ b/betapose_amd/csrc/conv_s1b3.hip
@@ -0,0 +1,305 @@
+#include <algorithm>
+#include <cstdlib>
+
+#include "conv_dev.h"
+
+namespace bp {
+
+struct S1B3Args {
+    int MT;
+    int NG;
+    int MS;
+    int has_res;
+    int rbuf;
+    int off_pl, off_stg, off_res, off_bias;
+    int hw;
+    int stamp_blocks;
+};
+
+static constexpr int S1B3_BM = 32, S1B3_BN = 128;
+static constexpr int S1B3_STG_FLOATS = 16 * 36;
+
+template <int NCH>
+__global__ __launch_bounds__(384) void conv_s1b3_kernel(const ConvParams p, const S1B3Args a) {
+    constexpr int RAW = NCH * 4096;
+    constexpr int PLS = NCH * 2048;
+    extern __shared__ __attribute__((aligned(16))) char lds[];
+    const int tid = threadIdx.x, lane = tid & 63;
+    unsigned long long* const st = (p.stamps && tid == 0 && (int)blockIdx.x < a.stamp_blocks) ? p.stamps + (long long)blockIdx.x * 8 : nullptr;
+    if (st) st[0] = bp_clock();
+    const int w = __builtin_amdgcn_readfirstlane(tid >> 6);
+    const int nlw = (int)(blockDim.x >> 6) - 4;
+    const int oR = a.off_res;
+    float* const ldsBias = reinterpret_cast<float*>(lds + a.off_bias);
+    constexpr int rrow = S1B3_BN * 4;
+    constexpr int rtile = 32 * rrow;
+    const int xcd = (int)blockIdx.x & 7, bq = (int)blockIdx.x >> 3;
+    const int ng = bq % a.NG, ms = bq / a.NG;
+    const int MT8 = (a.MT + 7) >> 3;
+    int nit = ms < MT8 ? (MT8 - 1 - ms) / a.MS + 1 : 0;
+    if (nit > 0 && (ms + (nit - 1) * a.MS) * 8 + xcd >= a.MT) --nit;
+    const int n0 = ng * S1B3_BN;
+
+    if (tid < S1B3_BN) ldsBias[tid] = n0 + tid < p.CoutPad ? p.bias[n0 + tid] : 0.f;
+    const bool has_res = a.has_res != 0, has_scale = p.res_scale != nullptr;
+    const float rcp_hw = 1.0f / (float)a.hw;
+
+    if (w >= 4) {
+        const int li = w - 4;
+        asm volatile("s_waitcnt vmcnt(0) lgkmcnt(0)" ::: "memory");
+        __syncthreads();
+        if (nit == 0) return;
+        const __amdgpu_buffer_rsrc_t rsrcA = __builtin_amdgcn_make_buffer_rsrc(
+            const_cast<float*>(p.in), 0, (int)min((long long)p.N * p.H * p.W * p.in_ld * 4, (long long)OOB), 0x00020000);
+        const __amdgpu_buffer_rsrc_t rsrcR = __builtin_amdgcn_make_buffer_rsrc(
+            const_cast<float*>(p.res ? p.res : p.out), 0, (int)min((long long)p.M * (p.res ? p.res_ld : p.out_ld) * 4, (long long)OOB), 0x00020000);
+        const __amdgpu_buffer_rsrc_t rsrcS = __builtin_amdgcn_make_buffer_rsrc(
+            const_cast<float*>(has_scale ? p.res_scale : p.bias), 0, has_scale ? p.N * p.Cout * 4 : 0, 0x00020000);
+        int vm = 0;
+        int seqa = 0, seqr = 0;
+        auto a_issue = [&](int k) __attribute__((always_inline)) {
+            if (k >= nit) return;
+            const int mt = (ms + k * a.MS) * 8 + xcd, j = k & 1;
+            const int q = (lane & 7) ^ ((lane >> 4) & 1);
+            unsigned vo[4];
+#pragma unroll
+            for (int i = 0; i < 4; ++i) {
+                const int m = mt * S1B3_BM + 8 * i + (lane >> 3);
+                vo[i] = m < p.M ? (unsigned)((m * p.in_ld + q * 4) * 4) : OOB;
+            }
+            char* const dst = lds + j * RAW;
+            int cnt = 0;
+#pragma unroll
+            for (int c = 0; c < NCH; ++c) {
+                if (nlw == 2 && (c & 1) != li) continue;
+#pragma unroll
+                for (int i = 0; i < 4; ++i) dma16(rsrcA, dst + c * 4096 + i * 1024, vo[i], c * 128);
+                cnt += 4;
+            }
+            vm += cnt;
+            seqa = lane == j ? vm : seqa;
+        };
+        auto r_issue = [&](int k) __attribute__((always_inline)) {
+            if (!has_res || li != 0 || k >= nit) return;
+            const int mt = (ms + k * a.MS) * 8 + xcd, j = k & 1;
+            const int m0 = mt * S1B3_BM;
+            char* const dst = lds + oR + j * a.rbuf;
+            constexpr int LPR = S1B3_BN / 4, RPP = 64 / LPR, NP_ = 32 / RPP;
+#pragma unroll
+            for (int i = 0; i < NP_; ++i) {
+                const int m = m0 + RPP * i + lane / LPR, n = n0 + 4 * (lane % LPR);
+                dma16(rsrcR, dst + i * 1024, (m < p.M && n < p.Cout) ? (unsigned)((m * p.res_ld + n) * 4) : OOB, 0);
+            }
+            vm += NP_;
+            if (has_scale) {
+                const int b0 = fast_div(min(m0, p.M - 1), a.hw, rcp_hw);
+                const int b = min(b0 + lane / LPR, p.N - 1), n = n0 + 4 * (lane % LPR);
+                dma16(rsrcS, dst + rtile, n < p.Cout ? (unsigned)((b * p.Cout + n) * 4) : OOB, 0);
+                ++vm;
+            }
+            seqr = lane == j ? vm : seqr;
+        };
+        a_issue(0); r_issue(0); a_issue(1); r_issue(1);
+        for (int k = 0; k < nit; ++k) {
+            int need = __builtin_amdgcn_readlane(seqa, k & 1);
+            if (has_res && li == 0) need = max(need, __builtin_amdgcn_readlane(seqr, k & 1));
+            s1_vm_wait(vm - need);
+            asm volatile("s_barrier" ::: "memory");
+            if (k > 0) r_issue(k + 1);
+            asm volatile("s_barrier" ::: "memory");
+            a_issue(k + 2);
+        }
+        return;
+    }
+
+    const __amdgpu_buffer_rsrc_t rsrcB = __builtin_amdgcn_make_buffer_rsrc(
+        const_cast<unsigned short*>(p.w16s), 0, (int)((long long)3 * p.CoutPad * p.Kpad * 2), 0x00020000);
+    const __amdgpu_buffer_rsrc_t rsrcO =
+        __builtin_amdgcn_make_buffer_rsrc(p.out, 0, (int)min((long long)p.M * p.out_ld * 4, (long long)OOB), 0x00020000);
+    const PlaneDesc pd = make_plane_desc(p);
+    float* const stg = reinterpret_cast<float*>(lds + a.off_stg) + w * S1B3_STG_FLOATS;
+    char* const planes = lds + a.off_pl;
+    const int fsw = ((lane & 31) >> 2) & 3;
+    const int fr0 = (lane & 31) * 64 + ((((lane >> 5)) ^ fsw) << 4), fr1 = fr0 ^ 32;
+    u32x4 fb[NCH][3][2];
+    {
+        const int col0 = n0 + 32 * w;
+        const int so_tile = (col0 >> 6) * (p.Kpad >> 4) * (3 * 64 * 32);
+        const int voff = (32 * ((col0 >> 5) & 1) + (lane & 31)) * 32 + (((lane >> 5) ^ ((lane >> 3) & 1)) << 4);
+        static_for<NCH>([&](auto ic) __attribute__((always_inline)) {
+            constexpr int c = decltype(ic)::value;
+#pragma unroll
+            for (int ks = 0; ks < 2; ++ks)
+#pragma unroll
+                for (int pl = 0; pl < 3; ++pl)
+                    fb[c][pl][ks] = __builtin_amdgcn_raw_buffer_load_b128(rsrcB, voff, so_tile + (2 * c + ks) * (3 * 64 * 32) + pl * 2048, 0);
+        });
+    }
+    asm volatile("s_waitcnt vmcnt(0) lgkmcnt(0)" ::: "memory");
+    __syncthreads();
+    if (st) st[1] = bp_clock();
+    const int s_row = 16 * (w & 1) + (lane >> 2), s_g = lane & 3;
+    const int s_sw = (s_row >> 1) & 1;
+    const int s_in = (w >> 1) * 4096 + s_row * 128, s_lo = ((2 * s_g) ^ s_sw) << 4, s_hi = ((2 * s_g + 1) ^ s_sw) << 4;
+    const int s_out = (w >> 1) * 2048 + s_row * 64 + ((s_g ^ ((s_row >> 2) & 3)) << 4);
+    const int e_row = lane >> 3, e_q = lane & 7;
+    const int nl = 32 * w + 4 * e_q, n = n0 + nl;
+    const f32x4 bias4 = *reinterpret_cast<const f32x4*>(ldsBias + nl);
+    const bool n_ok = n < p.Cout;
+    constexpr int PA[6] = {2, 1, 0, 1, 0, 0};
+    constexpr int PB[6] = {0, 1, 2, 0, 1, 0};
+
+    for (int k = 0; k < nit; ++k) {
+        const int mt = (ms + k * a.MS) * 8 + xcd;
+        const int m0 = mt * S1B3_BM;
+        asm volatile("s_barrier" ::: "memory");
+        if (st && k < 4) st[k == 0 ? 2 : 4 + k] = bp_clock();
+        {
+            const char* const raw = lds + (k & 1) * RAW + s_in;
+            char* const dst = planes + s_out;
+#pragma unroll
+            for (int s = 0; s < NCH / 2; ++s) {
+                const f32x4 lo = *reinterpret_cast<const f32x4*>(raw + s * 8192 + s_lo), hi = *reinterpret_cast<const f32x4*>(raw + s * 8192 + s_hi);
+                const bf16x4 l1 = __builtin_convertvector(lo, bf16x4), h1 = __builtin_convertvector(hi, bf16x4);
+                const f32x4 rl1 = lo - __builtin_convertvector(l1, f32x4), rh1 = hi - __builtin_convertvector(h1, f32x4);
+                const bf16x4 l2 = __builtin_convertvector(rl1, bf16x4), h2 = __builtin_convertvector(rh1, bf16x4);
+                const f32x4 rl2 = rl1 - __builtin_convertvector(l2, f32x4), rh2 = rh1 - __builtin_convertvector(h2, f32x4);
+                const bf16x4 l3 = __builtin_convertvector(rl2, bf16x4), h3 = __builtin_convertvector(rh2, bf16x4);
+                *reinterpret_cast<bf16x8*>(dst + s * 4096) = __builtin_shufflevector(l1, h1, 0, 1, 2, 3, 4, 5, 6, 7);
+                *reinterpret_cast<bf16x8*>(dst + s * 4096 + PLS) = __builtin_shufflevector(l2, h2, 0, 1, 2, 3, 4, 5, 6, 7);
+                *reinterpret_cast<bf16x8*>(dst + s * 4096 + 2 * PLS) = __builtin_shufflevector(l3, h3, 0, 1, 2, 3, 4, 5, 6, 7);
+            }
+        }
+        asm volatile("s_waitcnt lgkmcnt(0)\n\ts_barrier" ::: "memory");
+        f32x16 acc;
+#pragma unroll
+        for (int r = 0; r < 16; ++r) acc[r] = 0.f;
+        static_for<NCH>([&](auto cc) __attribute__((always_inline)) {
+            constexpr int c = decltype(cc)::value;
+#pragma unroll
+            for (int ks = 0; ks < 2; ++ks) {
+                bf16x8 fa[3];
+#pragma unroll
+                for (int pl = 0; pl < 3; ++pl) fa[pl] = *reinterpret_cast<const bf16x8*>(planes + pl * PLS + c * 2048 + (ks ? fr1 : fr0));
+#pragma unroll
+                for (int q = 0; q < 6; ++q)
+                    acc = __builtin_amdgcn_mfma_f32_32x32x16_bf16(fa[PA[q]], __builtin_bit_cast(bf16x8, fb[c][PB[q]][ks]), acc, 0, 0, 0);
+            }
+        });
+        if (st && k == 0) { asm volatile("" :: "v"(acc[0])); st[3] = bp_clock(); }
+        {
+            const char* const rb = lds + oR + (k & 1) * a.rbuf;
+            const int b0 = has_scale ? fast_div(min(m0, p.M - 1), a.hw, rcp_hw) : 0;
+#pragma unroll
+            for (int half = 0; half < 2; ++half) {
+#pragma unroll
+                for (int r = 0; r < 8; ++r) {
+                    const int row = (r & 3) + 8 * (r >> 2) + 4 * (lane >> 5);
+                    stg[row * 36 + (lane & 31)] = acc[8 * half + r];
+                }
+#pragma unroll
+                for (int ps = 0; ps < 2; ++ps) {
+                    const int hrow = 8 * ps + e_row, row = 16 * half + hrow;
+                    const int m = m0 + row;
+                    f32x4 v = *reinterpret_cast<const f32x4*>(stg + hrow * 36 + 4 * e_q);
+                    v += bias4;
+                    f32x4 r4 = {0.f, 0.f, 0.f, 0.f};
+                    if (has_res) {
+                        r4 = *reinterpret_cast<const f32x4*>(rb + row * rrow + nl * 4);
+                        if (has_scale) {
+                            const int b = fast_div(min(m, p.M - 1), a.hw, rcp_hw);
+                            r4 *= *reinterpret_cast<const f32x4*>(rb + rtile + (b - b0) * (S1B3_BN * 4) + nl * 4);
+                        }
+                        if (!p.res_after_act) v += r4;
+                    }
+                    if (p.act == ACT_LEAKY) {
+                        v.x = v.x > 0.f ? v.x : 0.1f * v.x; v.y = v.y > 0.f ? v.y : 0.1f * v.y;
+                        v.z = v.z > 0.f ? v.z : 0.1f * v.z; v.w = v.w > 0.f ? v.w : 0.1f * v.w;
+                    } else if (p.act == ACT_RELU) {
+                        v.x = v.x > 0.f ? v.x : 0.f; v.y = v.y > 0.f ? v.y : 0.f;
+                        v.z = v.z > 0.f ? v.z : 0.f; v.w = v.w > 0.f ? v.w : 0.f;
+                    }
+                    if (has_res && p.res_after_act) v += r4;
+                    const unsigned off = (m < p.M && n_ok) ? (unsigned)(m * p.out_ld + n) : (OOB >> 2);
+                    if (pd.f32) {
+                        const u32x4 o = {__float_as_uint(v.x), __float_as_uint(v.y), __float_as_uint(v.z), __float_as_uint(v.w)};
+                        __builtin_amdgcn_raw_buffer_store_b128(o, rsrcO, (int)(off * 4), 0, 0);
+                    }
+                    emit_planes4(pd, v, off * 2);
+                }
+            }
+        }
+    }
+    if (st && nit > 0) st[4] = bp_clock();
+}
+
+static bool s1b3_plan(const ConvParams& p, long long M, bool has_res, S1B3Args* out, int* grid, int* lds_bytes) {
+    S1B3Args a{};
+    const int nch = p.nchunks;
+    a.MT = (int)((M + S1B3_BM - 1) / S1B3_BM);
+    a.NG = (p.CoutPad + S1B3_BN - 1) / S1B3_BN;
+    a.has_res = has_res ? 1 : 0;
+    a.hw = p.OH * p.OW;
+    a.stamp_blocks = a.MT * a.NG;
+    a.rbuf = has_res ? 32 * S1B3_BN * 4 + (p.res_scale ? 1024 : 0) : 0;
+    const int raw_b = nch * 4096, pl_b = 3 * nch * 2048, stg_b = 4 * S1B3_STG_FLOATS * 4, bias_b = S1B3_BN * 4;
+    a.off_pl = 2 * raw_b;
+    a.off_stg = a.off_pl + pl_b;
+    a.off_res = a.off_stg + stg_b;
+    a.off_bias = a.off_res + 2 * a.rbuf;
+    const int total = a.off_bias + bias_b;
+    if (total > 160 * 1024 - 192) return false;
+    const char* const bpc_env = std::getenv("BP_S1B3_BPC");
+    const int bpc = bpc_env ? std::max(1, std::atoi(bpc_env)) : ((nch <= 4 && 2 * total <= 160 * 1024 - 384) ? 2 : 1);
+    const int MT8 = (a.MT + 7) / 8;
+    const char* const ms_env = std::getenv("BP_S1B3_MS");
+    const int ms_want = ms_env && std::atoi(ms_env) > 0 ? std::atoi(ms_env) : (bpc * 256) / (8 * a.NG);
+    a.MS = std::max(1, std::min(MT8, ms_want));
+    *out = a;
+    *grid = 8 * a.NG * a.MS;
+    *lds_bytes = total;
+    return true;
+}
+
+bool conv_s1b3_eligible(const ConvParams& p, long long M) {
+    if (p.mfma_mode != PREC_BF16X3 || p.ksize != 1 || p.stride != 1 || p.pad != 0 || M < 2048) return false;
+    if (p.store_mode != ST_NHWC || p.pool_out != nullptr) return false;
+    const int nch = p.nchunks;
+    if (!(nch == 2 || nch == 4 || nch == 8)) return false;
+    if (p.w16s == nullptr || p.in == nullptr || (p.in16 != nullptr && p.wpl != nullptr)) return false;
+    if (p.Kpad != p.Cin || (p.in_ld & 3) || p.H != p.OH || p.W != p.OW) return false;
+    if (p.CoutPad < S1B3_BN || (p.Cout & 3) || (p.out_ld & 3) || p.OH * p.OW < S1B3_BM) return false;
+    if (p.res && ((p.res_ld & 3) != 0 || p.res16 != nullptr)) return false;
+    if (p.res_scale && !p.res) return false;
+    if (p.out16 != nullptr && p.out_np != 3) return false;
+    if (M * p.out_ld * 4 >= (long long)OOB || (p.res && M * p.res_ld * 4 >= (long long)OOB) || M * p.in_ld * 4 >= (long long)OOB ||
+        (long long)3 * p.CoutPad * p.Kpad * 2 >= (long long)OOB) return false;
+    S1B3Args a; int g, l;
+    if (!s1b3_plan(p, M, p.res != nullptr, &a, &g, &l)) return false;
+    const int min_tiles = nch == 8 ? 16 : 3;
+    return std::getenv("BP_S1B3_ALL") != nullptr || (a.MT + 7) / 8 >= min_tiles * a.MS;
+}
+
+template <int NCH>
+static void launch_s1b3_t(const ConvParams& p, const S1B3Args& a, int grid, int lds_bytes, hipStream_t s) {
+    if (lds_bytes > 64 * 1024) allow_big_lds(reinterpret_cast<const void*>(conv_s1b3_kernel<NCH>));
+    const dim3 block(NCH >= 8 ? 384 : 320);
+    if (g_conv_prof)
+        hipExtLaunchKernelGGL((conv_s1b3_kernel<NCH>), dim3(grid), block, lds_bytes, s, g_conv_prof->e0, g_conv_prof->e1, 0, p, a);
+    else
+        hipLaunchKernelGGL((conv_s1b3_kernel<NCH>), dim3(grid), block, lds_bytes, s, p, a);
+}
+
+void launch_conv_s1b3(const ConvParams& p, hipStream_t s) {
+    BP_CHECK(conv_s1b3_eligible(p, p.M) && p.splits == 1 && p.hy_splits == 0 && !p.xcd_home,
+             "streaming 1x1 tile (bf16x3): 1x1 / stride 1, NHWC store, fp32 activations, K in {64, 128, 256}, N >= 128, M >= 2048, one K slice");
+    S1B3Args a; int grid = 0, lds_bytes = 0;
+    BP_CHECK(s1b3_plan(p, p.M, p.res != nullptr, &a, &grid, &lds_bytes), "streaming 1x1 tile (bf16x3): no LDS plan");
+    switch (p.nchunks) {
+        case 2: launch_s1b3_t<2>(p, a, grid, lds_bytes, s); break;
+        case 4: launch_s1b3_t<4>(p, a, grid, lds_bytes, s); break;
+        default: launch_s1b3_t<8>(p, a, grid, lds_bytes, s); break;
+    }
+}
+
+}
diff --git a/betapose_amd/csrc/engine.cpp b/betapose_amd/csrc/engine.cpp
--- a/betapose_amd/csrc/engine.cpp
+++ b/betapose_amd/csrc/engine.cpp
@@ -442,7 +442,8 @@
     if (mode == PREC_BF16X3)
         for (const PlanEntry& e : plan_file_entries())
             if (e.M == (int)M && e.CoutPad == c.CoutPad && e.nchunks == c.nchunks && !conv_tile_is_pl(e.tile) &&
-                (!conv_tile_is_halo(e.tile) || conv_halo_eligible(c, e.tile))) { *tile = e.tile; *splits = e.splits; return; }
+                (!conv_tile_is_halo(e.tile) || conv_halo_eligible(c, e.tile)) &&
+                (e.tile != TILE_S1B3 || (e.splits == 1 && conv_s1b3_eligible(c, M)))) { *tile = e.tile; *splits = e.splits; return; }
     static const bool halo_off = std::getenv("BP_NO_HALO") != nullptr;
 #ifdef BP_EXPERIMENTAL
     for (const PlanEntry* e = (mode == PREC_F16 ? kPlanF16 : kPlanB3); e->M != 0; ++e)
@@ -481,6 +482,7 @@
     if (tile == TILE_64x64 || tile == TILE_128x64) return !on_planes;
     if (tile == TILE_S1) return conv_s1_eligible(c, M);
     if (tile == TILE_P3) return conv_p3_eligible(c, M);
+    if (tile == TILE_S1B3) return conv_s1b3_eligible(c, M);
     if (conv_tile_is_pl(tile)) return c.mfma_mode != PREC_F32 && conv_pl_eligible(c) && (!conv_tile_is_plh(tile) || conv_plh_eligible(c));
     if (tile == TILE_64x64_BD || tile == TILE_BD_K2) return c.mfma_mode == PREC_BF16X3 && conv_h16_eligible(c) && c.w16s != nullptr && !on_planes;
     if (conv_tile_is_halo(tile)) return c.mfma_mode == PREC_BF16X3 && c.in16 == nullptr && conv_halo_eligible(c, tile);
@@ -510,6 +512,7 @@
     if (mode != PREC_F32) {
         choose_h16(c, M, mode, sk_max, &t, &s, lone);
         if (t == TILE_S1 && op.pool_out) t = TILE_PL64;
+        if (t == TILE_S1B3 && op.pool_out) t = TILE_64x64_BD;
         static const bool s1_off = std::getenv("BP_NO_S1") != nullptr;
         if (!s1_off && mode == PREC_F16 && s == 1 && conv_tile_is_pl(t) && !op.pool_out && conv_s1_eligible(c, M)) t = TILE_S1;
         static const bool p3_off = std::getenv("BP_NO_P3") != nullptr;
@@ -517,14 +520,16 @@
         static const int p3_k1 = std::getenv("BP_P3_K1") ? std::atoi(std::getenv("BP_P3_K1")) : 1;
         if (!p3_off && p3_k1 && mode == PREC_F16 && s == 1 && c.ksize == 1 && conv_tile_is_pl(t) && !op.pool_out && conv_p3_eligible(c, M) &&
             (p3_k1 == 2 || c.Cin >= 512)) t = TILE_P3;
-        if (force_tile >= 0 && !((force_tile == TILE_S1 || force_tile == TILE_P3) && op.pool_out) && tile_runs(force_tile, c, M)) t = force_tile;
+        static const bool s1b3_off = std::getenv("BP_NO_S1B3") != nullptr;
+        if (!s1b3_off && mode == PREC_BF16X3 && s == 1 && t == TILE_64x64_BD && !op.pool_out && conv_s1b3_eligible(c, M)) t = TILE_S1B3;
+        if (force_tile >= 0 && !((force_tile == TILE_S1 || force_tile == TILE_P3 || force_tile == TILE_S1B3) && op.pool_out) && tile_runs(force_tile, c, M)) t = force_tile;
         if (!(sk_target == 512 && sk_min_chunks == 4 && sk_max == 8)) {
             const long long blocks = ((M + conv_tile_bm(t) - 1) / conv_tile_bm(t)) *
                                      ((c.CoutPad + conv_tile_bn(t) - 1) / conv_tile_bn(t));
             s = 1;
             while (blocks * s < sk_target && c.nchunks / (s + 1) >= sk_min_chunks && s < sk_max) ++s;
         }
-        if (t == TILE_S1 || t == TILE_P3) s = 1;
+        if (t == TILE_S1 || t == TILE_P3 || t == TILE_S1B3) s = 1;
     } else if (stem3_wanted(c, force_tile)) {
         t = TILE_STEM3;
     } else if (stem7_wanted(c, force_tile)) {
diff --git a/betapose_amd/ops.py b/betapose_amd/ops.py
--- a/betapose_amd/ops.py
+++ b/betapose_amd/ops.py
@@ -11,7 +11,7 @@
 STORE = {"nhwc": 0, "up2": 1, "pixshuf": 2, "nchw": 3}
 _F16, _B3 = 256, 512
 TILE = {"auto": -1, "64x64": 0, "128x64": 1, "stem3": 20, "stem7": 28, "64x64_f16": _F16, "128x64_f16": _F16 + 1, "64x64_b3": _B3, "bd_b3": _B3 + 12,
-        "bd_f16": _F16 + 12, "halo64_b3": _B3 + 21, "halo128_b3": _B3 + 22, "halo64k2_b3": _B3 + 23, "bdk2_b3": _B3 + 24}
+        "bd_f16": _F16 + 12, "halo64_b3": _B3 + 21, "halo128_b3": _B3 + 22, "halo64k2_b3": _B3 + 23, "bdk2_b3": _B3 + 24, "s1b3_b3": _B3 + 29}
 for _n, _i in (("w1x1", 2), ("w1x2", 3), ("w2x1", 5), ("w2x2", 6), ("pl64", 13), ("pl128", 14), ("pl128x64", 15), ("pl256x128", 16), ("pl128s", 17), ("pl64k2", 18), ("pl64bd", 19), ("plh128", 25), ("s1", 26), ("p3", 27)):
     TILE[_n + "_f16"] = _F16 + _i
     TILE[_n + "_b3"] = _B3 + _i
@@ -21,7 +21,7 @@
 
 def conv2d_nhwc(x, weight, bias=None, stride: int = 1, pad: int = 0, act: str = "linear", store: str = "nhwc",
                 res=None, res_after_act: bool = False, tile: str = "auto", splits: int = 0, iters: int = 0,
-                planes: bool = False):
+                planes: bool = False, res_scale=None):
     import torch
     _lib.require_gpu()
     w = np.ascontiguousarray(weight.detach().cpu().numpy() if hasattr(weight, "detach") else weight, dtype=np.float32)
@@ -45,9 +45,12 @@
     if planes:
         assert store != "nchw", "NCHW outputs (the heat-maps) have no operand planes"
         pl = torch.zeros((1 if TILE[tile] < _B3 else 3,) + tuple(out.shape), device=x.device, dtype=torch.int16)
-    _lib.check(_lib.lib().bp_conv2d_planes(x.data_ptr(), N, H, W, Cin, w.ctypes.data, b.ctypes.data if b is not None else None,
+    if res_scale is not None:
+        assert res is not None and tuple(res_scale.shape) == (N, Cout) and res_scale.dtype == torch.float32
+    _lib.check(_lib.lib().bp_conv2d_scaled(x.data_ptr(), N, H, W, Cin, w.ctypes.data, b.ctypes.data if b is not None else None,
                                            Cout, k, stride, pad, ACT[act], STORE[store],
-                                           res.contiguous().data_ptr() if res is not None else None, int(res_after_act),
+                                           res.contiguous().data_ptr() if res is not None else None,
+                                           res_scale.contiguous().data_ptr() if res_scale is not None else None, int(res_after_act),
                                            TILE[tile], int(splits), out.data_ptr(), pl.data_ptr() if planes else None,
                                            int(iters), C.byref(ms), _lib.current_stream()))
     ret = (out,) + ((pl,) if planes else ()) + ((ms.value,) if iters > 0 else ())
diff --git a/include/betapose_hip.h b/include/betapose_hip.h
--- a/include/betapose_hip.h
+++ b/include/betapose_hip.h
@@ -126,6 +126,11 @@
 int bp_conv2d_planes(const float* d_in, int N, int H, int W, int Cin, const float* h_w, const float* h_bias, int Cout, int k,
                      int stride, int pad, int act, int store_mode, const float* d_res, int res_after_act, int tile, int splits,
                      float* d_out, unsigned short* d_out_planes, int iters, float* ms_per_iter, void* stream);
+int bp_conv2d_scaled(const float* d_in, int N, int H, int W, int Cin, const float* h_w, const float* h_bias, int Cout, int k,
+                     int stride, int pad, int act, int store_mode, const float* d_res, const float* d_res_scale, int res_after_act,
+                     int tile, int splits, float* d_out, unsigned short* d_out_planes, int iters, float* ms_per_iter, void* stream);
+int bp_conv_tile_eligible(int tile, int precision, int N, int H, int W, int Cin, int Cout, int k, int stride, int pad, int store_mode,
+                          int pooled);
 
 int bp_pipeline_create(bp_yolo* y, bp_kpd* k, int frame_h, int frame_w, int batch, float conf, int num_classes,
                        uint8_t* d_frames, float* d_results, float* d_hm, bp_pipeline** out);
```

Measured after the change: 1022 (median of 3 runs). Within noise of the previous version (+0.1%).
